# sayands/sgaligner

Measured on AMD Instinct MI355X. Metric: subscan-pairs/sec (fwd+bwd) + node-match Hits@1 vs reference, higher is better.
Workload: dtype f32 (fp32 operands and fp32 accumulation throughout; the anchors x negatives loss sweeps multiply them as three exact bf16 planes, six bf16 MFMAs per product...

## Files before the change

include/sgaligner_hip.h:

```cpp
#ifndef SGALIGNER_HIP_H
#define SGALIGNER_HIP_H
#include <stddef.h>
#include <stdint.h>
#ifdef __cplusplus
extern "C" {
#endif

int sga_version(void);
const char* sga_last_error(void);
int sga_device_cus(void);

int sga_pointnet_fwd(const float* x, const float* w1, const float* b1, const float* w2, const float* b2,
                     const float* w3, const float* b3, float* y, int32_t* argmax, int T, int P, int C3,
                     void* stream);
size_t sga_pointnet_fwd_ws_bytes(int T, int C3);
int sga_pointnet_fwd_ws(const float* x, const float* w1, const float* b1, const float* w2, const float* b2,
                        const float* w3, const float* b3, float* y, int32_t* argmax, int T, int P, int C3,
                        void* workspace, size_t ws_bytes, int mode, void* stream);
size_t sga_pointnet_fwd_bn_ws_bytes(int T, int C3);
int sga_pointnet_fwd_bn(const float* x, const float* w1, const float* b1, const float* w2, const float* b2,
                        const float* w3, const float* b3, float* y, int32_t* argmax, int T, int P, int C3,
                        void* workspace, size_t ws_bytes, void* bn_workspace, size_t bn_ws_bytes, double* bn_sums, int mode, void* stream);
int sga_pointnet_bwd(const float* x, const int32_t* argmax, const float* y, const float* gy, const float* w1,
                     const float* b1, const float* w2, const float* b2, const float* w3, float* gw1, float* gb1,
                     float* gw2, float* gb2, float* gw3, float* gb3, int T, int P, int C3, int mode, void* stream);

int sga_gemm(int transA, int transB, int M, int N, int K, const void* A, long lda, int a_is_f64, const float* B,
             long ldb, float* C, long ldc, const float* bias, int accumulate, void* stream);
int sga_colsum(const float* X, long ld, int M, int N, float* out, int accumulate, void* stream);
int sga_gemm_bnstats(int M, int N, int K, const float* A, long lda, const float* B, long ldb, float* C, long ldc, const float* bias,
                     double* sums, void* stream);
int sga_cast_f64_f32(const double* in, float* out, size_t n, void* stream);

int sga_fusion_fwd(const float* const* embs, int M, const float* weight, float* joint, int T, int D, void* stream);
size_t sga_fusion_bwd_workspace_bytes(int M);
int sga_fusion_bwd(const float* const* embs, int M, const float* weight, const float* gjoint, float* const* gembs,
                   float* gweight, int T, int D, void* workspace, size_t workspace_bytes, void* stream);

int sga_gat_complete_flags(const int64_t* edges, const int32_t* node_off, const int32_t* edge_off, int G, uint8_t* flags, void* stream);
int sga_gat_attn_fwd(const float* H, const float* att_src, const float* att_dst, const float* bias,
                     const int64_t* edges, const int32_t* node_off, const int32_t* edge_off, int G, int nmax,
                     float* out, int32_t* status, const uint8_t* complete, void* stream);
int sga_gat_attn_bwd(const float* H, const float* dO, const float* att_src, const float* att_dst, const int64_t* edges,
                     const int32_t* node_off, const int32_t* edge_off, int G, int nmax, float* dH, float* d_att_src,
                     float* d_att_dst, const uint8_t* complete, void* stream);
int sga_elu_fwd(const float* x, float* y, size_t n, void* stream);
int sga_elu_bwd(const float* x, const float* gy, float* gx, size_t n, void* stream);

int sga_loss_gather(const float* E, int T, int D, const int32_t* idx, int R, float* Z, int Dp, float* nrm, void* stream);
int sga_loss_scatter(const float* dZ, const float* Z, const float* nrm, const int32_t* idx, int R, int D, int Dp,
                     float* dE, void* stream);
int sga_loss_slots(void);
int sga_loss_neg_sums(const float* Z, int Dp, int A, int J1, int J2, float tau0, float tau1, double* sums8, void* stream);
int sga_loss_neg_grad(const float* Z, int Dp, int A, int J1, int J2, float tau0, float tau1, const double* gs8,
                      float* dZ, void* stream);
int sga_loss_neg_sums_shard(const float* Z, int Dp, int A, int J1, int J2, float tau0, float tau1, double* sums8, int a_lo, int a_hi,
                            void* stream);
int sga_loss_neg_grad_shard(const float* Z, int Dp, int A, int J1, int J2, float tau0, float tau1, const double* gs8,
                            float* dZ, int a_lo, int a_hi, void* stream);
int sga_loss_anchor_fwd(const float* const* Z, const int* Dp, int NT, int A, const double* sums, float alpha,
                        float tau_icl, float tau_ial, double* out, int a_lo, int a_hi, void* stream);
int sga_loss_anchor_bwd(const float* const* Z, const int* Dp, int NT, int A, const double* sums, float alpha,
                        float tau_icl, float tau_ial, const float* coef, float* const* M1, double* gs, int a_lo, int a_hi,
                        void* stream);

size_t sga_loss_anchor_f16_ws_bytes(int NT, int A, int ns);
int sga_loss_anchor_fwd_f16(const float* const* Z, const void* const* Zh, const int* Dp, int NT, int A, const double* sums,
                            float alpha, float tau_icl, float tau_ial, double* out, int a_lo, int a_hi, void* ws, size_t ws_bytes,
                            void* stream);
int sga_loss_anchor_bwd_f16(const float* const* Z, const void* const* Zh, const int* Dp, int NT, int A, const double* sums,
                            float alpha, float tau_icl, float tau_ial, const float* coef, float* const* M1,
                            double* gs, int a_lo, int a_hi, void* ws, size_t ws_bytes, void* stream);

int sga_loss_stash_grad(const float* M1, const float* Z, int A, int Dp, float* dZ, int a_lo, int a_hi, void* stream);
int sga_loss_multi_sums(const float* const* Z, int M, int D, const float* beta, int A, int J1, int J2, float tau0, float tau1,
                        double* sums, int a_lo, int a_hi, void* stream);
int sga_loss_multi_grad(const float* const* Z, int M, int D, const float* beta, int A, int J1, int J2, float tau0, float tau1,
                        const double* gs, float* const* dZ, double* gamma, int a_lo, int a_hi, void* stream);
size_t sga_loss_centre_bytes(void);
int sga_loss_centre_tables(const float* Z, int A, int J1, int J2, float* Zc, void* stat_ws, void* stream);
int sga_loss_multi_sums_centred(const float* const* Zc, int M, const float* beta, int A, int J1, int J2, float tau0, float tau1,
                                double* sums, int a_lo, int a_hi, void* stream);
int sga_loss_multi_grad_centred(const float* const* Zc, int M, const float* beta, int A, int J1, int J2, float tau0, float tau1,
                                const double* gs, float* const* dZ, double* gamma, int a_lo, int a_hi, void* stream);
int sga_loss_scatter_tangent_stat(const float* dZ, const float* Z, const float* nrm, const int32_t* idx, int R, int D,
                                  const void* stat_ws, float* dE, void* stream);
int sga_loss_anchor_multi_fwd(const float* const* Z, int M, const float* beta, int A, const double* sums, float alpha,
                              float tau_icl, float tau_ial, double* out, int a_lo, int a_hi, void* stream);
int sga_loss_anchor_multi_bwd(const float* const* Z, int M, const float* beta, int A, const double* sums, float alpha,
                              float tau_icl, float tau_ial, const float* coef, float* const* M1, double* gs, double* gamma,
                              int a_lo, int a_hi, double* out_terms, void* stream);
int sga_loss_anchor_multi_bwd_sym(const float* const* Z, int M, const float* beta, int A, const double* sums, float alpha,
                                  float tau_icl, float tau_ial, const float* coef, float* const* M1, float* const* M2, double* gs,
                                  double* gamma, int a_lo, int a_hi, double* out_terms, void* stream);
int sga_loss_stash_grad_sym(const float* M1, const float* M2, const float* Z, int A, int Dp, float* dZ, int a_lo, int a_hi,
                            void* stream);
int sga_loss_anchor_multi_bwd_symx(const float* const* Z, int M, const float* beta, int A, const double* sums, float alpha,
                                   float tau_icl, float tau_ial, const float* coef, float* const* M1, float* const* M2,
                                   double* gs, double* gamma, int a_lo, int a_hi, int j_lo, int j_hi, int mir, double* out_terms, void* stream);
int sga_loss_stash_grad_symx(const float* M1, const float* M2, const float* Z, int A, int Dp, float* dZ, int a_lo, int a_hi,
                             int j_lo, int j_hi, int mir, void* stream);

int sga_loss_build_joint(const float* const* Z, int M, const float* beta, int rows, float* ZJ, void* stream);
int sga_loss_fold_joint(const float* const* Z, int M, const float* beta, const float* dZJ, int rows, float* const* dZ,
                        double* gamma2, void* stream);
int sga_loss_check_norms(const float* nrm, int n, float* poison, void* stream);

size_t sga_loss_split3_bytes(int A, int J1, int J2);
int sga_loss_split3_tables(const float* Z, int A, int J1, int J2, void* Zb, float* Zc, void* stream);
int sga_loss_multi_sums_bf16x6(const void* const* Zb, int M, const float* beta, int A, int J1, int J2, float tau0, float tau1,
                               double* sums, int a_lo, int a_hi, int lite, void* stream);
int sga_loss_multi_grad_bf16x6(const void* const* Zb, int M, const float* beta, int A, int J1, int J2, float tau0, float tau1,
                               const double* gs, float* const* dZ, double* gamma, int a_lo, int a_hi, void* stream);
int sga_loss_scatter_tangent(const float* dZ, const float* Z, const float* nrm, const int32_t* idx, int A, int J1, int J2, int D,
                             const void* Zb, float* dE, void* stream);
int sga_loss_stash_grad_symx_bf16x6(const float* M1, const float* M2, const void* Zb, int A, int J1, int J2, float* dZ,
                                    int a_lo, int a_hi, int j_lo, int j_hi, int mir, void* stream);

int sga_group_loss_fwd(const float* const* Z, int M, const float* beta, int A, int J1, const int32_t* groups, int G,
                       const int64_t* s_off, int64_t s_total, float alpha, float tau_icl, float tau_ial, float* S,
                       double* sums, double* out, int use_valu, void* stream);
int sga_group_loss_bwd(const float* const* Z, int M, const float* beta, int A, int J1, const int32_t* groups, int G,
                       const int64_t* s_off, int64_t s_total, float alpha, float tau_icl, float tau_ial, float* S,
                       const double* sums, const float* coef, float* const* dZ, double* gamma, int use_valu, void* stream);

size_t sga_simrank_workspace_bytes(int T);
size_t sga_simrank_workspace_bytes_f16(int T, int D);
int sga_simrank(const float* E, int T, int D, const int32_t* pair_off, const int32_t* blk_pair, const int32_t* blk_row, int n_blocks, int B,
                int max_pair_objects, const int32_t* q_idx, const int32_t* q_tgt, int Q, int K, int32_t* rank,
                int32_t* topk_idx, float* topk_sim, int f16, void* workspace, size_t workspace_bytes, void* stream);
int sga_pair_metrics(const int32_t* rank, const int32_t* topk_idx, const float* topk_sim, int K, const int32_t* q_tgt,
                     const int32_t* pair_off, const int32_t* pair_q_off, int B, float* out, void* stream);

int sga_gemm_ex(int transA, int transB, int M, int N, int K, const float* A, long lda, const float* B, long ldb,
                float* C, long ldc, const float* bias, int act, const float* resid, long ldr, void* stream);
int sga_pct_attention(const float* Q, long ldq, const float* V, long ldv, int T, int N, float* stats, float* Xs,
                      long ldx, void* stream);
int sga_pct_attention_bwd(const float* Q, long ldq, const float* V, long ldv, const float* dXs, long ldd, int T, int N,
                          const float* stats, float* work, float* dQ, long ldo, float* dV, long ldw, void* stream);
int sga_segment_max(const float* Y, long ldy, int T, int N, int C, float* G, int32_t* argmax, void* stream);
int sga_segment_max_bwd(const float* dG, const int32_t* argmax, int T, int N, int C, float* dY, long ldd, void* stream);
int sga_pct_head_prep(const float* dG, const float* G, const float* gamma, const float* beta, const float* fin, int T, int C, long R,
                      int training, float slope, float* coef, float* ab, void* stream);
int sga_pct_head_dw(const float* WG, const float* W, const float* ab, const float* cs, const float* coef, const int32_t* amax,
                    const float* cat, long ldc, int T, int N, int C, int K, float* dW, float* Wb, float* a0, void* stream);
int sga_pct_head_scatter(const float* coef, const int32_t* amax, const float* W, int T, int N, int C, int K, float* dcat, long ldd,
                         void* stream);
int sga_segment_max_affine(const float* Y, long ldy, int T, int N, int C, const float* scale, const float* shift, float slope, float* G,
                           int32_t* argmax, void* stream);

int sga_bn_stats(const float* X, long ldx, int R, int C, double* sums, void* stream);
int sga_bn_finalize(const double* sums, int R, int C, const float* gamma, const float* beta, float* running_mean, float* running_var,
                    long long* num_batches_tracked, float momentum, float eps, int training, float* out, void* stream);
int sga_bn_bwd_finalize(const double* sums, int R, int C, float* out, void* stream);
int sga_bn_apply(const float* X, long ldx, int R, int C, const float* scale, const float* shift, int act,
                 const float* resid, long ldr, float* Y, long ldy, void* stream);
int sga_bn_bwd_stats(const float* X, long ldx, const float* dY, long ldd, int R, int C, const float* scale,
                     const float* shift, const float* mean, const float* rstd, int act, double* sums, void* stream);
int sga_bn_bwd_apply(const float* X, long ldx, const float* dY, long ldd, int R, int C, const float* scale,
                     const float* shift, const float* mean, const float* rstd, const float* mean_g,
                     const float* mean_gx, int act, float* dX, long ldo, void* stream);

size_t sga_fps_scratch_floats(int total_points);
int sga_fps(const float* pts, const int32_t* offsets, int n_obj, const int32_t* start, int npoint,
            const int32_t* work_small, int n_small, const int32_t* work_mid, int n_mid,
            const int32_t* work_large, int n_large, int32_t* out_idx, float* scratch, void* stream);

int sga_hull_candidates(const float* pts, const int32_t* offsets, int n_obj, unsigned char* keep, int32_t* n_planes, void* stream);
int sga_hull_max_candidates(void);
int sga_hull_vertices(const double* pts, const int32_t* offsets, int n_obj, unsigned char* is_vertex, int32_t* status, void* stream);

size_t sga_loss_neg_grad_wide_floats(int A, int J1, int J2);
int sga_loss_neg_grad_wide(const float* Z, int Dp, int A, int J1, int J2, float tau0, float tau1, const double* gs8, float* dZ,
                           float* stash, size_t stash_floats, void* stream);

long sga_wide16_ldt(int A, int J1, int J2);
int sga_wide16_prepare(const float* Z, int Dp, int A, int J1, int J2, void* Zh, void* ZhT, void* stream);
int sga_loss_neg_sums_f16(const void* Zh, int Dp, int A, int J1, int J2, float tau0, float tau1, double* sums8, int a_lo, int a_hi, void* stream);
size_t sga_loss_neg_grad_f16_bytes(int A, int J1, int J2);
int sga_loss_neg_grad_f16(const void* Zh, const void* ZhT, int Dp, int A, int J1, int J2, float tau0, float tau1, const double* gs8,
                          float* dZ, void* stash, size_t stash_bytes, int a_lo, int a_hi, void* stream);
size_t sga_loss_stash_grad_f16_bytes(int A, int ns);
int sga_loss_stash_grad_f16(const float* M1, const void* ZhT, int Dp, int A, int J1, int J2, float* dZ, int a_lo, int a_hi,
                            void* ws, size_t ws_bytes, void* stream);

int sga_loss_head_fwd(const void* sums, int sums_f64, const float* lv_ial, const float* lv_icl, int M, double inv_a2,
                      double z_ial, double alpha, double zoom, double* out, void* stream);
int sga_loss_head_bwd(const double* gout, const void* sums, int sums_f64, const float* lv_ial, const float* lv_icl, int M,
                      double inv_a2, double z_ial, double alpha, double zoom, void* dsums, float* dlv_ial, float* dlv_icl,
                      void* stream);

#ifdef __cplusplus
}
#endif
#endif
```

sgaligner_amd/_lib.py:

```python
from __future__ import annotations

import ctypes
import os
from ctypes import c_char_p, c_double, c_float, c_int, c_int64, c_long, c_size_t, c_void_p

_HERE = os.path.dirname(os.path.abspath(__file__))
LIB_PATH = os.environ.get('SGA_LIB_PATH') or os.path.join(_HERE, 'csrc', 'libsga_hip.so')
_lib = None

P = c_void_p
I = c_int
F = c_float

SIGNATURES = {
    'sga_version': (I, []),
    'sga_last_error': (c_char_p, []),
    'sga_device_cus': (I, []),
    'sga_pointnet_fwd': (I, [P, P, P, P, P, P, P, P, P, I, I, I, P]),
    'sga_pointnet_fwd_ws_bytes': (c_size_t, [I, I]),
    'sga_loss_neg_grad_wide_floats': (c_size_t, [I, I, I]),
    'sga_loss_neg_grad_wide': (I, [P, I, I, I, I, c_float, c_float, P, P, P, c_size_t, P]),
    'sga_wide16_ldt': (c_long, [I, I, I]),
    'sga_wide16_prepare': (I, [P, I, I, I, I, P, P, P]),
    'sga_loss_neg_sums_f16': (I, [P, I, I, I, I, c_float, c_float, P, I, I, P]),
    'sga_loss_neg_grad_f16_bytes': (c_size_t, [I, I, I]),
    'sga_loss_neg_grad_f16': (I, [P, P, I, I, I, I, c_float, c_float, P, P, P, c_size_t, I, I, P]),
    'sga_loss_head_fwd': (I, [P, I, P, P, I, c_double, c_double, c_double, c_double, P, P]),
    'sga_loss_head_bwd': (I, [P, P, I, P, P, I, c_double, c_double, c_double, c_double, P, P, P, P]),
    'sga_pointnet_fwd_ws': (I, [P, P, P, P, P, P, P, P, P, I, I, I, P, c_size_t, I, P]),
    'sga_pointnet_fwd_bn_ws_bytes': (c_size_t, [I, I]),
    'sga_pointnet_fwd_bn': (I, [P, P, P, P, P, P, P, P, P, I, I, I, P, c_size_t, P, c_size_t, P, I, P]),
    'sga_pointnet_bwd': (I, [P] * 15 + [I, I, I, I, P]),
    'sga_gat_complete_flags': (I, [P, P, P, I, P, P]),
    'sga_gat_attn_fwd': (I, [P, P, P, P, P, P, P, I, I, P, P, P, P]),
    'sga_gat_attn_bwd': (I, [P, P, P, P, P, P, P, I, I, P, P, P, P, P]),
    'sga_elu_fwd': (I, [P, P, c_size_t, P]),
    'sga_elu_bwd': (I, [P, P, P, c_size_t, P]),
    'sga_simrank_workspace_bytes': (c_size_t, [I]),
    'sga_simrank_workspace_bytes_f16': (c_size_t, [I, I]),
    'sga_simrank': (I, [P, I, I, P, P, P, I, I, I, P, P, I, I, P, P, P, I, P, c_size_t, P]),
    'sga_pair_metrics': (I, [P, P, P, I, P, P, P, I, P, P]),
    'sga_gemm_ex': (I, [I, I, I, I, I, P, c_long, P, c_long, P, c_long, P, I, P, c_long, P]),
    'sga_pct_attention': (I, [P, c_long, P, c_long, I, I, P, P, c_long, P]),
    'sga_pct_attention_bwd': (I, [P, c_long, P, c_long, P, c_long, I, I, P, P, P, c_long, P, c_long, P]),
    'sga_segment_max': (I, [P, c_long, I, I, I, P, P, P]),
    'sga_segment_max_bwd': (I, [P, P, I, I, I, P, c_long, P]),
    'sga_pct_head_prep': (I, [P, P, P, P, P, I, I, c_long, I, c_float, P, P, P]),
    'sga_pct_head_dw': (I, [P, P, P, P, P, P, P, c_long, I, I, I, I, P, P, P, P]),
    'sga_pct_head_scatter': (I, [P, P, P, I, I, I, I, P, c_long, P]),
    'sga_segment_max_affine': (I, [P, c_long, I, I, I, P, P, c_float, P, P, P]),
    'sga_bn_stats': (I, [P, c_long, I, I, P, P]),
    'sga_bn_finalize': (I, [P, I, I, P, P, P, P, P, c_float, c_float, I, P, P]),
    'sga_bn_bwd_finalize': (I, [P, I, I, P, P]),
    'sga_bn_apply': (I, [P, c_long, I, I, P, P, I, P, c_long, P, c_long, P]),
    'sga_bn_bwd_stats': (I, [P, c_long, P, c_long, I, I, P, P, P, P, I, P, P]),
    'sga_bn_bwd_apply': (I, [P, c_long, P, c_long, I, I, P, P, P, P, P, P, I, P, c_long, P]),
    'sga_fps_scratch_floats': (c_size_t, [I]),
    'sga_fps': (I, [P, P, I, P, I, P, I, P, I, P, I, P, P, P]),
    'sga_hull_candidates': (I, [P, P, I, P, P, P]),
    'sga_hull_max_candidates': (I, []),
    'sga_hull_vertices': (I, [P, P, I, P, P, P]),
    'sga_gemm': (I, [I, I, I, I, I, P, c_long, I, P, c_long, P, c_long, P, I, P]),
    'sga_colsum': (I, [P, c_long, I, I, P, I, P]),
    'sga_gemm_bnstats': (I, [I, I, I, P, c_long, P, c_long, P, c_long, P, P, P]),
    'sga_cast_f64_f32': (I, [P, P, c_size_t, P]),
    'sga_loss_gather': (I, [P, I, I, P, I, P, I, P, P]),
    'sga_loss_scatter': (I, [P, P, P, P, I, I, I, P, P]),
    'sga_loss_neg_sums': (I, [P, I, I, I, I, F, F, P, P]),
    'sga_loss_neg_grad': (I, [P, I, I, I, I, F, F, P, P, P]),
    'sga_loss_neg_sums_shard': (I, [P, I, I, I, I, F, F, P, I, I, P]),
    'sga_loss_neg_grad_shard': (I, [P, I, I, I, I, F, F, P, P, I, I, P]),
    'sga_loss_anchor_fwd': (I, [P, P, I, I, P, F, F, F, P, I, I, P]),
    'sga_loss_anchor_bwd': (I, [P, P, I, I, P, F, F, F, P, P, P, I, I, P]),
    'sga_loss_anchor_f16_ws_bytes': (c_size_t, [I, I, I]),
    'sga_loss_anchor_fwd_f16': (I, [P, P, P, I, I, P, F, F, F, P, I, I, P, c_size_t, P]),
    'sga_loss_anchor_bwd_f16': (I, [P, P, P, I, I, P, F, F, F, P, P, P, I, I, P, c_size_t, P]),
    'sga_loss_stash_grad_f16_bytes': (c_size_t, [I, I]),
    'sga_loss_stash_grad_f16': (I, [P, P, I, I, I, I, P, I, I, P, c_size_t, P]),
    'sga_loss_multi_sums': (I, [P, I, I, P, I, I, I, F, F, P, I, I, P]),
    'sga_loss_multi_grad': (I, [P, I, I, P, I, I, I, F, F, P, P, P, I, I, P]),
    'sga_loss_centre_bytes': (c_size_t, []),
    'sga_loss_centre_tables': (I, [P, I, I, I, P, P, P]),
    'sga_loss_multi_sums_centred': (I, [P, I, P, I, I, I, F, F, P, I, I, P]),
    'sga_loss_multi_grad_centred': (I, [P, I, P, I, I, I, F, F, P, P, P, I, I, P]),
    'sga_loss_scatter_tangent_stat': (I, [P, P, P, P, I, I, P, P, P]),
    'sga_loss_build_joint': (I, [P, I, P, I, P, P]),
    'sga_loss_fold_joint': (I, [P, I, P, P, I, P, P, P]),
    'sga_loss_check_norms': (I, [P, I, P, P]),
    'sga_loss_slots': (I, []),
    'sga_loss_anchor_multi_fwd': (I, [P, I, P, I, P, F, F, F, P, I, I, P]),
    'sga_loss_anchor_multi_bwd': (I, [P, I, P, I, P, F, F, F, P, P, P, P, I, I, P, P]),
    'sga_loss_stash_grad': (I, [P, P, I, I, P, I, I, P]),
    'sga_loss_anchor_multi_bwd_sym': (I, [P, I, P, I, P, F, F, F, P, P, P, P, P, I, I, P, P]),
    'sga_loss_stash_grad_sym': (I, [P, P, P, I, I, P, I, I, P]),
    'sga_loss_anchor_multi_bwd_symx': (I, [P, I, P, I, P, F, F, F, P, P, P, P, P, I, I, I, I, I, P, P]),
    'sga_loss_stash_grad_symx': (I, [P, P, P, I, I, P, I, I, I, I, I, P]),
    'sga_loss_split3_bytes': (c_size_t, [I, I, I]),
    'sga_loss_split3_tables': (I, [P, I, I, I, P, P, P]),
    'sga_loss_scatter_tangent': (I, [P, P, P, P, I, I, I, I, P, P, P]),
    'sga_loss_stash_grad_symx_bf16x6': (I, [P, P, P, I, I, I, P, I, I, I, I, I, P]),
    'sga_loss_multi_sums_bf16x6': (I, [P, I, P, I, I, I, F, F, P, I, I, I, P]),
    'sga_loss_multi_grad_bf16x6': (I, [P, I, P, I, I, I, F, F, P, P, P, I, I, P]),
    'sga_group_loss_fwd': (I, [P, I, P, I, I, P, I, P, c_int64, F, F, F, P, P, P, I, P]),
    'sga_group_loss_bwd': (I, [P, I, P, I, I, P, I, P, c_int64, F, F, F, P, P, P, P, P, I, P]),
    'sga_fusion_fwd': (I, [P, I, P, P, I, I, P]),
    'sga_fusion_bwd_workspace_bytes': (c_size_t, [I]),
    'sga_fusion_bwd': (I, [P, I, P, P, P, P, I, I, P, c_size_t, P]),
}


class SgaLibraryError(RuntimeError):
    pass


def lib():
    global _lib
    if _lib is None:
        if not os.path.exists(LIB_PATH):
            raise SgaLibraryError(
                f'HIP library not built: {LIB_PATH} is missing. Run `python -c "import __graft_entry__ as g; g.build()"` '
                f'(or `python -m sgaligner_amd._build`). sgaligner_amd has no CPU fallback.')
        import torch
        try:
            l = ctypes.CDLL(LIB_PATH)
        except OSError as e:
            raise SgaLibraryError(f'cannot load {LIB_PATH}: {e}') from e
        for name, (res, args) in SIGNATURES.items():
            try:
                fn = getattr(l, name)
            except AttributeError as e:
                raise SgaLibraryError(f'{LIB_PATH} does not export {name}; rebuild the library') from e
            fn.restype = res
            fn.argtypes = args
        _lib = l
    return _lib


def check(rc: int, what: str):
    if rc != 0:
        msg = lib().sga_last_error()
        raise RuntimeError(f'{what} failed (code {rc}): {msg.decode() if msg else "?"}')
```

sgaligner_amd/csrc/contrastive.hip:

```cpp
#include "mfma_tiles.h"
#include <type_traits>

#include "loss_math.h"
#include "wide16_api.h"

extern "C" int sga_gemm(int transA, int transB, int M, int N, int K, const void* A, long lda, int a_is_f64, const float* B,
                        long ldb, float* C, long ldc, const float* bias, int accumulate, void* stream);

namespace {

constexpr int CT_THREADS = 256;
constexpr int CT_MAXT = 9;
__global__ void gather_normalize_kernel(const float* __restrict__ E, int D, const int* __restrict__ idx, int R,
                                        float* __restrict__ Z, int Dp, float* __restrict__ nrm) {
    const int lane = threadIdx.x & 63, wpb = blockDim.x >> 6;
    for (int r = blockIdx.x * wpb + (threadIdx.x >> 6); r < R; r += gridDim.x * wpb) {
        const float* x = E + (size_t)idx[r] * D;
        float ss = 0.f;
        for (int d = lane; d < D; d += 64) { const float v = x[d]; ss += v * v; }
        ss = wave_sum(ss);
        const float n = sqrtf(ss);
        const float inv = 1.f / fmaxf(n, 1e-12f);
        float* z = Z + (size_t)r * Dp;
        for (int d = lane; d < Dp; d += 64) z[d] = d < D ? x[d] * inv : 0.f;
        if (lane == 0) nrm[r] = n;
    }
}

__global__ void scatter_normalize_bwd_kernel(const float* __restrict__ dZ, const float* __restrict__ Z,
                                             const float* __restrict__ nrm, const int* __restrict__ idx, int R, int D,
                                             int Dp, float* __restrict__ dE) {
    const int lane = threadIdx.x & 63, wpb = blockDim.x >> 6;
    for (int r = blockIdx.x * wpb + (threadIdx.x >> 6); r < R; r += gridDim.x * wpb) {
        const float* g = dZ + (size_t)r * Dp;
        const float* z = Z + (size_t)r * Dp;
        float dot = 0.f;
        for (int d = lane; d < D; d += 64) dot += g[d] * z[d];
        dot = wave_sum(dot);
        const float n = nrm[r];
        const bool clamped = n < 1e-12f;
        const float inv = 1.f / fmaxf(n, 1e-12f);
        if (clamped) dot = 0.f;
        float* o = dE + (size_t)idx[r] * D;
        for (int d = lane; d < D; d += 64) atomicAdd(o + d, (g[d] - z[d] * dot) * inv);
    }
}

struct SweepSeg { int row0, n, fam; };
struct SweepGroup { int own0, nown, blk0, nseg; SweepSeg seg[2]; int nsplit; };
struct SweepArgs {
    const float* Z; int Dp; int ngroups; SweepGroup grp[4];
    float k0, k1;
    float it0, it1;
    double* sums;
    const double* gs;
    float* dZ;
    int col0;
};

template <int NJT, int NCT, bool GRAD>
__global__ __launch_bounds__(CT_THREADS) void sweep_kernel(SweepArgs a) {
    constexpr int OT = NJT * 32;
    constexpr int GW = NCT * 32;
    extern __shared__ __attribute__((aligned(16))) float lds[];
    float* own_s = lds;
    float* oth_s = lds + 128 * SGA_LDS_STRIDE;

    const int tid = threadIdx.x, lane = tid & 63, wave = tid >> 6, h = lane >> 5;
    int g = 0;
#pragma unroll
    for (int i = 1; i < 4; ++i) if (i < a.ngroups && (int)blockIdx.x >= a.grp[i].blk0) g = i;
    const SweepGroup& grp = a.grp[g];
    const int own0 = grp.own0 + ((int)blockIdx.x - grp.blk0) * 128;
    const int own_end = grp.own0 + grp.nown;
    const int my_i = own0 + wave * 32 + (lane & 31);

    f32x16 gacc[GRAD ? NCT : 1];
    if (GRAD) zero_acc<GRAD ? NCT : 1>(gacc);
    double dsum[2][2] = {{0.0, 0.0}, {0.0, 0.0}};

#pragma unroll
    for (int sg = 0; sg < 2; ++sg) {
        if (sg >= grp.nseg) break;
        const SweepSeg seg = grp.seg[sg];
        float c0 = 0.f, c1 = 0.f;
        if (GRAD) { c0 = (float)(a.gs[seg.fam * 2 + 0] * (double)a.it0); c1 = (float)(a.gs[seg.fam * 2 + 1] * (double)a.it1); }
        const int ntile = (seg.n + OT - 1) / OT;
        for (int jt = blockIdx.y; jt < ntile; jt += gridDim.y) {
            const int j0 = seg.row0 + jt * OT, j_end = seg.row0 + seg.n;
            f32x16 sacc[NJT];
            zero_acc<NJT>(sacc);
            for (int k0 = 0; k0 < a.Dp; k0 += SGA_KC) {
                __syncthreads();
                lds_load_rows<128, CT_THREADS>(own_s, a.Z, a.Dp, own0, own_end, k0, a.Dp, tid);
                lds_load_rows<OT, CT_THREADS>(oth_s, a.Z, a.Dp, j0, j_end, k0, a.Dp, tid);
                __syncthreads();
                mfma_chunk<NJT>(sacc, oth_s, own_s + (wave * 32 + (lane & 31)) * SGA_LDS_STRIDE, lane);
            }
            if (!GRAD) {
                float p0 = 0.f, p1 = 0.f;
                const bool iv = my_i < own_end;
#pragma unroll
                for (int t = 0; t < NJT; ++t)
#pragma unroll
                    for (int r = 0; r < 16; ++r) {
                        const float okf = (iv && (j0 + t * 32 + mfma32_row(r, h) < j_end)) ? 1.f : 0.f;
                        p0 = fmaf(okf, fexp2(sacc[t][r] * a.k0), p0);
                        p1 = fmaf(okf, fexp2(sacc[t][r] * a.k1), p1);
                    }
                dsum[sg][0] += (double)p0;
                dsum[sg][1] += (double)p1;
            } else {
#pragma unroll
                for (int t = 0; t < NJT; ++t)
#pragma unroll
                    for (int r = 0; r < 16; ++r)
                        sacc[t][r] = c0 * fexp2(sacc[t][r] * a.k0) + c1 * fexp2(sacc[t][r] * a.k1);
                __syncthreads();
                for (int e = tid; e < OT * (GW / 4); e += CT_THREADS) {
                    const int r = e / (GW / 4), c = (e % (GW / 4)) * 4;
                    const int gr = j0 + r, gc = a.col0 + c;
                    f32x4 v = {0.f, 0.f, 0.f, 0.f};
                    if (gr < j_end && gc < a.Dp) v = *reinterpret_cast<const f32x4*>(a.Z + (size_t)gr * a.Dp + gc);
                    *reinterpret_cast<f32x4*>(lds + r * GW + c) = v;
                }
                __syncthreads();
#pragma unroll
                for (int t = 0; t < NJT; ++t)
#pragma unroll
                    for (int s = 0; s < 16; ++s) {
                        const float av = sacc[t][s];
                        const float* brow = lds + (t * 32 + mfma32_row(s, h)) * GW + (lane & 31);
#pragma unroll
                        for (int ct = 0; ct < NCT; ++ct)
                            gacc[ct] = __builtin_amdgcn_mfma_f32_32x32x2f32(av, brow[ct * 32], gacc[ct], 0, 0, 0);
                    }
            }
        }
    }
    if (!GRAD) {
#pragma unroll
        for (int sg = 0; sg < 2; ++sg)
#pragma unroll
            for (int tt = 0; tt < 2; ++tt) {
                const double v = wave_sum_d(dsum[sg][tt]);
                if (lane == 0 && sg < grp.nseg && v != 0.0) atomicAdd(a.sums + 8 + my_slot() * 8 + grp.seg[sg].fam * 2 + tt, v);
            }
    } else {
#pragma unroll
        for (int ct = 0; ct < NCT; ++ct) {
            const int d = a.col0 + ct * 32 + (lane & 31);
            if (d < a.Dp) {
#pragma unroll
                for (int r = 0; r < 16; ++r) {
                    const int i = own0 + wave * 32 + mfma32_row(r, h);
                    if (i < own_end) atomicAdd(a.dZ + (size_t)i * a.Dp + d, gacc[ct][r]);
                }
            }
        }
    }
}

struct CoefArgs {
    const float* Z; int Dp; SweepGroup grp[2];
    float k0, k1, it0, it1;
    const double* gs;
    float* stash[2];
    int ld, n1;
};

template <int NJT>
__global__ __launch_bounds__(CT_THREADS) void sweep_coef_kernel(CoefArgs a) {
    constexpr int OT = NJT * 32;
    __shared__ __attribute__((aligned(16))) float own_s[128 * SGA_LDS_STRIDE];
    __shared__ __attribute__((aligned(16))) float oth_s[OT * SGA_LDS_STRIDE];
    const int tid = threadIdx.x, lane = tid & 63, wave = tid >> 6, h = lane >> 5;
    const int g = ((int)blockIdx.x >= a.grp[1].blk0 && a.grp[1].nown > 0) ? 1 : 0;
    const SweepGroup& grp = a.grp[g];
    const int own0 = grp.own0 + ((int)blockIdx.x - grp.blk0) * 128;
    const int own_end = grp.own0 + grp.nown;
    const int my_i = own0 + wave * 32 + (lane & 31);
    float* __restrict__ st = a.stash[g];
#pragma unroll
    for (int sg = 0; sg < 2; ++sg) {
        const SweepSeg seg = grp.seg[sg];
        const float c0 = (float)(a.gs[seg.fam * 2 + 0] * (double)a.it0), c1 = (float)(a.gs[seg.fam * 2 + 1] * (double)a.it1);
        const int ntile = (seg.n + OT - 1) / OT;
        for (int jt = blockIdx.y; jt < ntile; jt += gridDim.y) {
            const int j0 = seg.row0 + jt * OT, j_end = seg.row0 + seg.n;
            f32x16 sacc[NJT];
            zero_acc<NJT>(sacc);
            for (int k0 = 0; k0 < a.Dp; k0 += SGA_KC) {
                __syncthreads();
                lds_load_rows<128, CT_THREADS>(own_s, a.Z, a.Dp, own0, own_end, k0, a.Dp, tid);
                lds_load_rows<OT, CT_THREADS>(oth_s, a.Z, a.Dp, j0, j_end, k0, a.Dp, tid);
                __syncthreads();
                mfma_chunk<NJT>(sacc, oth_s, own_s + (wave * 32 + (lane & 31)) * SGA_LDS_STRIDE, lane);
            }
            if (my_i < own_end) {
#pragma unroll
                for (int t = 0; t < NJT; ++t)
#pragma unroll
                    for (int r = 0; r < 16; ++r) {
                        const int j = j0 + t * 32 + mfma32_row(r, h);
                        if (j < j_end) st[(size_t)(j - a.n1) * a.ld + (my_i - grp.own0)] = c0 * fexp2(sacc[t][r] * a.k0) + c1 * fexp2(sacc[t][r] * a.k1);
                    }
            }
        }
    }
}

template <int NQ, bool GRAD>
__global__ __launch_bounds__(CT_THREADS) void sweep_fast_kernel(SweepArgs a) {
    constexpr int DP = NQ * 8;
    constexpr int STR = DP + 4;
    constexpr int NJT = 4, OT = 128, NCT = 4;
    extern __shared__ __attribute__((aligned(16))) float lds[];

    const int tid = threadIdx.x, lane = tid & 63, wave = tid >> 6, h = lane >> 5;
    int g = 0;
#pragma unroll
    for (int i = 1; i < 4; ++i) if (i < a.ngroups && (int)blockIdx.x >= a.grp[i].blk0) g = i;
    const SweepGroup& grp = a.grp[g];
    const int own0 = grp.own0 + ((int)blockIdx.x - grp.blk0) * 128;
    const int own_end = grp.own0 + grp.nown;
    const int my_i = own0 + wave * 32 + (lane & 31);

    f32x4 own[NQ];
    {
        const float* src = a.Z + (size_t)(my_i < own_end ? my_i : own0) * DP + 4 * h;
        const float msk = my_i < own_end ? 1.f : 0.f;
#pragma unroll
        for (int q = 0; q < NQ; ++q) {
            f32x4 v = *reinterpret_cast<const f32x4*>(src + 8 * q);
            own[q] = v * msk;
        }
    }
    f32x16 gacc[GRAD ? NCT : 1];
    if (GRAD) zero_acc<GRAD ? NCT : 1>(gacc);
    double dsum[2][2] = {{0.0, 0.0}, {0.0, 0.0}};

#pragma unroll
    for (int sg = 0; sg < 2; ++sg) {
        if (sg >= grp.nseg) break;
        const SweepSeg seg = grp.seg[sg];
        float c0 = 0.f, c1 = 0.f;
        if (GRAD) { c0 = (float)(a.gs[seg.fam * 2 + 0] * (double)a.it0); c1 = (float)(a.gs[seg.fam * 2 + 1] * (double)a.it1); }
        const int ntile = (seg.n + OT - 1) / OT;
        for (int jt = blockIdx.y; jt < ntile; jt += gridDim.y) {
            const int j0 = seg.row0 + jt * OT, j_end = seg.row0 + seg.n;
            __syncthreads();
            for (int e = tid; e < OT * (DP / 4); e += CT_THREADS) {
                const int r = e / (DP / 4), c = (e % (DP / 4)) * 4;
                f32x4 v = {0.f, 0.f, 0.f, 0.f};
                if (j0 + r < j_end) v = *reinterpret_cast<const f32x4*>(a.Z + (size_t)(j0 + r) * DP + c);
                *reinterpret_cast<f32x4*>(lds + r * STR + c) = v;
            }
            __syncthreads();
            f32x16 sacc[NJT];
            zero_acc<NJT>(sacc);
            const float* ap = lds + (lane & 31) * STR + 4 * h;
#pragma unroll
            for (int q = 0; q < NQ; ++q) {
#pragma unroll
                for (int t = 0; t < NJT; ++t) {
                    const f32x4 av = *reinterpret_cast<const f32x4*>(ap + t * 32 * STR + 8 * q);
#pragma unroll
                    for (int r = 0; r < 4; ++r) sacc[t] = __builtin_amdgcn_mfma_f32_32x32x2f32(av[r], own[q][r], sacc[t], 0, 0, 0);
                }
            }
            if (!GRAD) {
                float p0 = 0.f, p1 = 0.f;
                const bool iv = my_i < own_end;
#pragma unroll
                for (int t = 0; t < NJT; ++t)
#pragma unroll
                    for (int r = 0; r < 16; ++r) {
                        const float okf = (iv && (j0 + t * 32 + mfma32_row(r, h) < j_end)) ? 1.f : 0.f;
                        p0 = fmaf(okf, fexp2(sacc[t][r] * a.k0), p0);
                        p1 = fmaf(okf, fexp2(sacc[t][r] * a.k1), p1);
                    }
                dsum[sg][0] += (double)p0;
                dsum[sg][1] += (double)p1;
            } else {
#pragma unroll
                for (int t = 0; t < NJT; ++t)
#pragma unroll
                    for (int r = 0; r < 16; ++r)
                        sacc[t][r] = c0 * fexp2(sacc[t][r] * a.k0) + c1 * fexp2(sacc[t][r] * a.k1);
#pragma unroll
                for (int t = 0; t < NJT; ++t)
#pragma unroll
                    for (int s = 0; s < 16; ++s) {
                        const float av = sacc[t][s];
                        const float* brow = lds + (t * 32 + mfma32_row(s, h)) * STR + (lane & 31);
#pragma unroll
                        for (int ct = 0; ct < NCT; ++ct)
                            gacc[ct] = __builtin_amdgcn_mfma_f32_32x32x2f32(av, brow[ct * 32], gacc[ct], 0, 0, 0);
                    }
            }
        }
    }
    if (!GRAD) {
#pragma unroll
        for (int sg = 0; sg < 2; ++sg)
#pragma unroll
// ... 645 lines not shown
                acc[m] = fmaf(gj, a.Z[m][(size_t)r * 104 + d], acc[m]);
                a.dZ[m][(size_t)r * 104 + d] += sb * gj;
            }
        }
#pragma unroll
    for (int m = 0; m < 4; ++m) {
        const float v = wave_sum(acc[m]);
        if (lane == 0 && m < a.M && v != 0.f) atomicAdd(gamma2 + m, (double)v);
    }
}

__global__ void check_norms_kernel(const float* __restrict__ nrm, int n, float* __restrict__ poison) {
    for (int i = blockIdx.x * blockDim.x + threadIdx.x; i < n; i += gridDim.x * blockDim.x)
        if (!(nrm[i] >= 1e-12f)) *poison = __builtin_nanf("");
}

typedef _Float16 ak_f16x8 __attribute__((ext_vector_type(8)));
template <int NROWS, int NTHREADS>
__device__ __forceinline__ void lds_load_rows_h(float* __restrict__ tile, const _Float16* __restrict__ g, int ld, int row0, int nrows, int k0,
                                                int ncols, int tid) {
    unsigned char* t8 = reinterpret_cast<unsigned char*>(tile);
#pragma unroll
    for (int e = tid; e < NROWS * 8; e += NTHREADS) {
        const int r = e >> 3, c = (e & 7) * 8;
        ak_f16x8 v = {0, 0, 0, 0, 0, 0, 0, 0};
        const int gr = row0 + r, gc = k0 + c;
        if (gr < nrows && gc < ncols) v = *reinterpret_cast<const ak_f16x8*>(g + (size_t)gr * ld + gc);
        *reinterpret_cast<ak_f16x8*>(t8 + r * 144 + c * 2) = v;
    }
}
template <int NT>
__device__ __forceinline__ void mfma_chunk_h(f32x16 (&acc)[NT], const float* __restrict__ a_tile, const float* __restrict__ b_row, int lane) {
    const unsigned char* ap = reinterpret_cast<const unsigned char*>(a_tile) + (lane & 31) * 144 + (lane >> 5) * 16;
    const unsigned char* bp = reinterpret_cast<const unsigned char*>(b_row) + (lane >> 5) * 16;
#pragma unroll
    for (int q = 0; q < 4; ++q) {
        const ak_f16x8 b = *reinterpret_cast<const ak_f16x8*>(bp + 32 * q);
#pragma unroll
        for (int t = 0; t < NT; ++t) {
            const ak_f16x8 av = *reinterpret_cast<const ak_f16x8*>(ap + t * 32 * 144 + 32 * q);
            acc[t] = __builtin_amdgcn_mfma_f32_32x32x16_f16(av, b, acc[t], 0, 0, 0);
        }
    }
}

struct AnchorArgs {
    int NT, A, i_lo, i_hi;
    const float* Z[CT_MAXT]; int Dp[CT_MAXT];
    const _Float16* Zh[CT_MAXT];
    const double* sums;
    float alpha, kc, ki, itc, iti;
    double* out;
    const float* coef;
    float* M1[CT_MAXT];
    double* gs;
    const float* SP[CT_MAXT];
    const float* SQ[CT_MAXT];
    long ldp;
};

template <bool BWD, bool PRE = false>
__global__ __launch_bounds__(CT_THREADS) void anchor_kernel(AnchorArgs a) {
    constexpr int NJT = PRE ? 1 : 2, OT = 32 * NJT;
    constexpr int LR = PRE ? 1 : 128, LO = PRE ? 1 : OT;
    __shared__ __attribute__((aligned(16))) float own1[LR * SGA_LDS_STRIDE];
    __shared__ __attribute__((aligned(16))) float own2[LR * SGA_LDS_STRIDE];
    __shared__ __attribute__((aligned(16))) float oth1[LO * SGA_LDS_STRIDE];
    __shared__ __attribute__((aligned(16))) float oth2[LO * SGA_LDS_STRIDE];
    __shared__ float inv_s[CT_MAXT * 8];

    const int tid = threadIdx.x, lane = tid & 63, wave = tid >> 6, h = lane >> 5;
    const int A = a.A, NT = a.NT, M = NT > 1 ? NT - 1 : 0;
    double* const out_s = BWD ? nullptr : a.out + (NT + 2 * M) * (1 + my_slot());
    double* const gs_s = BWD ? a.gs + NT * 8 * (1 + my_slot()) : nullptr;
    for (int e = tid; e < NT * 8; e += CT_THREADS) inv_s[e] = (float)(1.0 / (a.sums[e] + 1e-9));
    const int i0 = a.i_lo + blockIdx.x * 128, j0 = blockIdx.y * OT;
    const int my_i = i0 + wave * 32 + (lane & 31);
    const bool iv = my_i < a.i_hi;
    const int ns = a.i_hi - a.i_lo;

    f32x16 xJ[NJT], gJ[NJT];
    zero_acc<NJT>(xJ);
    zero_acc<NJT>(gJ);

    for (int it = 0; it < NT; ++it) {
        const int k = (NT > 1) ? (it == 0 ? NT - 1 : it - 1) : 0;
        const bool is_joint = NT > 1 && it == 0;
        const float* Z = a.Z[k];
        const int Dp = a.Dp[k];
        f32x16 P[NJT], Q[NJT];
        zero_acc<NJT>(P);
        zero_acc<NJT>(Q);
        const _Float16* Zh = a.Zh[k];
        if constexpr (PRE) {
            __syncthreads();
            const float* sp = a.SP[k] + (iv ? my_i - a.i_lo : 0);
            const float* sq = a.SQ[k] + (iv ? my_i - a.i_lo : 0);
#pragma unroll
            for (int t = 0; t < NJT; ++t)
#pragma unroll
                for (int r = 0; r < 16; ++r) {
                    const int j = min(j0 + t * 32 + mfma32_row(r, h), A - 1);
                    P[t][r] = sp[(size_t)j * a.ldp];
                    Q[t][r] = sq[(size_t)j * a.ldp];
                }
        } else
        if (Zh) {
            for (int k0 = 0; k0 < Dp; k0 += 64) {
                __syncthreads();
                lds_load_rows_h<128, CT_THREADS>(own1, Zh, Dp, i0, A, k0, Dp, tid);
                lds_load_rows_h<128, CT_THREADS>(own2, Zh, Dp, A + i0, 2 * A, k0, Dp, tid);
                lds_load_rows_h<OT, CT_THREADS>(oth1, Zh, Dp, A + j0, 2 * A, k0, Dp, tid);
                lds_load_rows_h<OT, CT_THREADS>(oth2, Zh, Dp, j0, A, k0, Dp, tid);
                __syncthreads();
                const int ro = (wave * 32 + (lane & 31)) * SGA_LDS_STRIDE;
                mfma_chunk_h<NJT>(P, oth1, own1 + ro, lane);
                mfma_chunk_h<NJT>(Q, oth2, own2 + ro, lane);
            }
        } else
        for (int k0 = 0; k0 < Dp; k0 += SGA_KC) {
            __syncthreads();
            lds_load_rows<128, CT_THREADS>(own1, Z, Dp, i0, A, k0, Dp, tid);
            lds_load_rows<128, CT_THREADS>(own2, Z, Dp, A + i0, 2 * A, k0, Dp, tid);
            lds_load_rows<OT, CT_THREADS>(oth1, Z, Dp, A + j0, 2 * A, k0, Dp, tid);
            lds_load_rows<OT, CT_THREADS>(oth2, Z, Dp, j0, A, k0, Dp, tid);
            __syncthreads();
            const int ro = (wave * 32 + (lane & 31)) * SGA_LDS_STRIDE;
            mfma_chunk<NJT>(P, oth1, own1 + ro, lane);
            mfma_chunk<NJT>(Q, oth2, own2 + ro, lane);
        }
        if (is_joint) {
#pragma unroll
            for (int t = 0; t < NJT; ++t) xJ[t] = P[t];
        }
        const float* is = inv_s + k * 8;
        const float a11c = is[0], a12c = is[2], a22c = is[4], a21c = is[6];
        const float a11i = is[1], a12i = is[3], a22i = is[5], a21i = is[7];
        const float* js = inv_s + (NT - 1) * 8;
        const float j11 = js[1], j12 = js[3], j22 = js[5], j21 = js[7];

        if (!BWD) {
            float icl = 0.f, la = 0.f, lb = 0.f;
#pragma unroll
            for (int t = 0; t < NJT; ++t)
#pragma unroll
                for (int r = 0; r < 16; ++r) {
                    const bool ok = iv && (j0 + t * 32 + mfma32_row(r, h) < A);
                    const float x = P[t][r], y = Q[t][r];
                    const float qa = g_val(fexp2(x * a.kc), a11c, a12c);
                    const float qb = g_val(fexp2(y * a.kc), a22c, a21c);
                    const float term = -flog(a.alpha * qa + (1.f - a.alpha) * qb);
                    icl += ok ? term : 0.f;
                    if (M > 0 && !is_joint) {
                        const float dm = fexp2(x * a.ki), dj = fexp2(xJ[t][r] * a.ki);
                        const float qoa = g_val(dm, a11i, a12i), qma = g_val(dj, j11, j12);
                        const float qob = g_val(dm, a22i, a21i), qmb = g_val(dj, j22, j21);
                        const float ta = __expf(qoa) * (qoa - flog(qma));
                        const float tb = __expf(qob) * (qob - flog(qmb));
                        la += ok ? ta : 0.f;
                        lb += ok ? tb : 0.f;
                    }
                    __builtin_amdgcn_sched_barrier(0);
                }
            icl = wave_sum(icl);
            if (lane == 0) atomicAdd(out_s + k, (double)icl);
            if (M > 0 && !is_joint) {
                la = wave_sum(la);
                lb = wave_sum(lb);
                if (lane == 0) { atomicAdd(out_s + NT + k, (double)la); atomicAdd(out_s + NT + M + k, (double)lb); }
            }
        } else {
            const float c = a.coef[k];
            const float ca = (M > 0 && !is_joint) ? a.coef[NT + k] : 0.f;
            const float cb = (M > 0 && !is_joint) ? a.coef[NT + M + k] : 0.f;
            float gs_c[4] = {0.f, 0.f, 0.f, 0.f};
            float gs_i[4] = {0.f, 0.f, 0.f, 0.f};
            float gs_j[4] = {0.f, 0.f, 0.f, 0.f};
#pragma unroll
            for (int t = 0; t < NJT; ++t)
#pragma unroll
                for (int r = 0; r < 16; ++r) {
                    const bool ok = iv && (j0 + t * 32 + mfma32_row(r, h) < A);
                    const float x = P[t][r], y = Q[t][r];
                    const float dx = fexp2(x * a.kc), dy = fexp2(y * a.kc);
                    const GV Ax = g_full(dx, a11c, a12c), Bx = g_full(dx, a22c, a21c);
                    const float qAy = g_val(dy, a11c, a12c), qBy = g_val(dy, a22c, a21c);
                    const float z_ij = a.alpha * Ax.q + (1.f - a.alpha) * qBy;
                    const float z_ji = a.alpha * qAy + (1.f - a.alpha) * Bx.q;
                    const float wA = ok ? -c * a.alpha * frcp(z_ij) : 0.f;
                    const float wB = ok ? -c * (1.f - a.alpha) * frcp(z_ji) : 0.f;
                    float gx = (wA * Ax.dd + wB * Bx.dd) * dx * a.itc;
                    gs_c[0] += wA * Ax.dsa; gs_c[1] += wA * Ax.dsb; gs_c[2] += wB * Bx.dsa; gs_c[3] += wB * Bx.dsb;
                    if (M > 0 && !is_joint) {
                        const float dm = fexp2(x * a.ki), dj = fexp2(xJ[t][r] * a.ki);
                        const GV OA = g_full(dm, a11i, a12i), OB = g_full(dm, a22i, a21i);
                        const GV MA = g_full(dj, j11, j12), MB = g_full(dj, j22, j21);
                        const float eA = ok ? __expf(OA.q) : 0.f, eB = ok ? __expf(OB.q) : 0.f;
                        const float tA = ca * eA * (OA.q - flog(MA.q) + 1.f), uA = -ca * eA * frcp(MA.q);
                        const float tB = cb * eB * (OB.q - flog(MB.q) + 1.f), uB = -cb * eB * frcp(MB.q);
                        gx += (tA * OA.dd + tB * OB.dd) * dm * a.iti;
                        gJ[t][r] += (uA * MA.dd + uB * MB.dd) * dj * a.iti;
                        gs_i[0] += tA * OA.dsa; gs_i[1] += tA * OA.dsb; gs_i[2] += tB * OB.dsa; gs_i[3] += tB * OB.dsb;
                        gs_j[0] += uA * MA.dsa; gs_j[1] += uA * MA.dsb; gs_j[2] += uB * MB.dsa; gs_j[3] += uB * MB.dsb;
                    }
                    P[t][r] = gx;
                    __builtin_amdgcn_sched_barrier(0);
                }
#pragma unroll
            for (int f = 0; f < 4; ++f) {
                const float vc = wave_sum(gs_c[f]);
                if (lane == 0 && vc != 0.f) atomicAdd(gs_s + k * 8 + f * 2 + 0, (double)vc);
                if (M > 0 && !is_joint) {
                    const float vi = wave_sum(gs_i[f]), vj = wave_sum(gs_j[f]);
                    if (lane == 0 && vi != 0.f) atomicAdd(gs_s + k * 8 + f * 2 + 1, (double)vi);
                    if (lane == 0 && vj != 0.f) atomicAdd(gs_s + (NT - 1) * 8 + f * 2 + 1, (double)vj);
                }
            }
            if (is_joint) {
#pragma unroll
                for (int t = 0; t < NJT; ++t) gJ[t] = P[t];
            } else if (iv) {
                float* m1 = a.M1[k];
#pragma unroll
                for (int t = 0; t < NJT; ++t)
#pragma unroll
                    for (int r = 0; r < 16; ++r) {
                        const int j = j0 + t * 32 + mfma32_row(r, h);
                        if (j < A) m1[(size_t)j * ns + (my_i - a.i_lo)] = P[t][r];
                    }
            }
        }
    }
    if (BWD && NT > 1 && iv) {
        float* m1 = a.M1[NT - 1];
#pragma unroll
        for (int t = 0; t < NJT; ++t)
#pragma unroll
            for (int r = 0; r < 16; ++r) {
                const int j = j0 + t * 32 + mfma32_row(r, h);
                if (j < A) m1[(size_t)j * ns + (my_i - a.i_lo)] = gJ[t][r];
            }
    }
}

template <int NCT, bool TRANS>
__global__ __launch_bounds__(256) void stash_gemm_kernel(const float* __restrict__ M1, const float* __restrict__ X,
                                                         float* __restrict__ out, int MR, int KR, int ldm, int ld, int Dp, int k_per_split) {
    const int lane = threadIdx.x & 63, wave = threadIdx.x >> 6, h = lane >> 5, l31 = lane & 31;
    const int m0 = (blockIdx.x * 4 + wave) * 32;
    if (m0 >= MR) return;
    const int kbeg = blockIdx.y * k_per_split, kend = min(KR, kbeg + k_per_split);
    const int m = min(m0 + l31, MR - 1);
    f32x16 acc[NCT];
    zero_acc<NCT>(acc);
    int ncol[NCT];
#pragma unroll
    for (int ct = 0; ct < NCT; ++ct) ncol[ct] = min(ct * 32 + l31, Dp - 1);
    for (int k0 = kbeg; k0 < kend; k0 += 8) {
        float av[4];
        float kmask[4];
#pragma unroll
        for (int r = 0; r < 4; ++r) {
            const int k = k0 + 4 * h + r;
            kmask[r] = k < kend ? 1.f : 0.f;
            const int kc = min(k, KR - 1);
            av[r] = (TRANS ? M1[(size_t)kc * ldm + m] : M1[(size_t)m * ldm + kc]) * kmask[r];
        }
#pragma unroll
        for (int r = 0; r < 4; ++r) {
            const int kc = min(k0 + 4 * h + r, KR - 1);
            const float* xr = X + (size_t)kc * ld;
#pragma unroll
            for (int ct = 0; ct < NCT; ++ct) acc[ct] = __builtin_amdgcn_mfma_f32_32x32x2f32(av[r], xr[ncol[ct]], acc[ct], 0, 0, 0);
        }
    }
#pragma unroll
    for (int ct = 0; ct < NCT; ++ct) {
        const int d = ct * 32 + l31;
        if (d < Dp) {
#pragma unroll
            for (int r = 0; r < 16; ++r) {
                const int row = m0 + mfma32_row(r, h);
                if (row < MR) atomicAdd(out + (size_t)row * ld + d, acc[ct][r]);
            }
        }
    }
}

struct AnchorMultiArgs {
    int M, A, i_lo, i_hi, nsplit;
    const float* Z[4];
    const float* beta;
    const double* sums;
    const float* inv;
    float alpha, kc, ki, itc, iti;
    double* out;
    const float* coef;
    float* M1[4];
    double* gs;
    double* gamma;
    int j_lo;
    float* M2[4];
    int j_hi, mir;
};

template <int M, bool BWD>
__global__ __launch_bounds__(CT_THREADS, M <= 3 ? 2 : 1) void anchor_multi_kernel(AnchorMultiArgs a) {
    constexpr int DP = 104, NQ = 13, NT = M + 1;
    extern __shared__ __attribute__((aligned(16))) float lds[];
    float* inv_s = lds + M * 2 * 32 * DP;
    const int tid = threadIdx.x, lane = tid & 63, wave = tid >> 6, h = lane >> 5, l31 = lane & 31;
    const int A = a.A, ns = a.i_hi - a.i_lo;
    const int ib = blockIdx.x / a.nsplit, split = blockIdx.x % a.nsplit;
    const int i0 = a.i_lo + ib * 32;
    const int my_i = i0 + l31;
    const bool iv = my_i < a.i_hi;

    for (int e = tid; e < M * 2 * 32 * (DP / 4); e += CT_THREADS) {
        const int c = (e % (DP / 4)) * 4, r = (e / (DP / 4)) % 32, side = (e / (DP / 4) / 32) % 2, m = e / (DP / 4) / 64;
        const int row = min(i0 + r, a.i_hi - 1) + side * A;
        *reinterpret_cast<f32x4*>(lds + ((m * 2 + side) * 32 + r) * DP + c) = *reinterpret_cast<const f32x4*>(a.Z[m] + (size_t)row * DP + c);
    }
    for (int e = tid; e < NT * 8; e += CT_THREADS) inv_s[e] = (float)(1.0 / (a.sums[e] + 1e-9));
    __syncthreads();
    float beta[M];
#pragma unroll
    for (int m = 0; m < M; ++m) beta[m] = a.beta[m];

    double acc_d[NT + 2 * M];
#pragma unroll
    for (int e = 0; e < NT + 2 * M; ++e) acc_d[e] = 0.0;

    const int ntile = (A + 31) / 32;
    for (int jt = split * 4 + wave; jt < ntile; jt += a.nsplit * 4) {
        const int j0 = jt * 32;
        float acc_out[NT + 2 * M];
#pragma unroll
        for (int e = 0; e < NT + 2 * M; ++e) acc_out[e] = 0.f;
        const int jrow = min(j0 + l31, A - 1);
        f32x16 P[M], Q[M];
        zero_acc<M>(P);
        zero_acc<M>(Q);
#pragma unroll
        for (int m = 0; m < M; ++m) {
            const float* gp = a.Z[m] + (size_t)(A + jrow) * DP + 4 * h;
            const float* gq = a.Z[m] + (size_t)jrow * DP + 4 * h;
            const float* bp = lds + ((m * 2 + 0) * 32 + l31) * DP + 4 * h;
            const float* bq = lds + ((m * 2 + 1) * 32 + l31) * DP + 4 * h;
            f32x4 apA = *reinterpret_cast<const f32x4*>(gp), aqA = *reinterpret_cast<const f32x4*>(gq), apB = apA, aqB = aqA;
#pragma unroll
            for (int q = 0; q < NQ; ++q) {
                if (q + 1 < NQ) {
                    if (q & 1) { apA = *reinterpret_cast<const f32x4*>(gp + 8 * (q + 1)); aqA = *reinterpret_cast<const f32x4*>(gq + 8 * (q + 1)); }
                    else { apB = *reinterpret_cast<const f32x4*>(gp + 8 * (q + 1)); aqB = *reinterpret_cast<const f32x4*>(gq + 8 * (q + 1)); }
                }
                const f32x4 b1 = *reinterpret_cast<const f32x4*>(bp + 8 * q);
                const f32x4 b2 = *reinterpret_cast<const f32x4*>(bq + 8 * q);
#pragma unroll
                for (int r = 0; r < 4; ++r) {
                    P[m] = __builtin_amdgcn_mfma_f32_32x32x2f32((q & 1) ? apB[r] : apA[r], b1[r], P[m], 0, 0, 0);
                    Q[m] = __builtin_amdgcn_mfma_f32_32x32x2f32((q & 1) ? aqB[r] : aqA[r], b2[r], Q[m], 0, 0, 0);
                }
                __builtin_amdgcn_sched_barrier(0);
            }
        }
        float xs[M][16], ys[M][16];
#pragma unroll
        for (int m = 0; m < M; ++m)
#pragma unroll
            for (int r = 0; r < 16; ++r) { xs[m][r] = P[m][r]; ys[m][r] = Q[m][r]; }
        const float* js = inv_s + M * 8;
#pragma unroll
        for (int r = 0; r < 16; ++r) {
            const int j = j0 + mfma32_row(r, h);
            const bool ok = iv && j < A;
            float xj = 0.f, yj = 0.f;
#pragma unroll
            for (int m = 0; m < M; ++m) { xj = fmaf(beta[m], xs[m][r], xj); yj = fmaf(beta[m], ys[m][r], yj); }
            {
                const float dji = fexp2(xj * a.ki);
                const float qma = g_val(dji, js[1], js[3]), qmb = g_val(dji, js[5], js[7]);
                const float lqma = flog(qma), lqmb = flog(qmb);
#pragma unroll
                for (int k = 0; k < NT; ++k) {
                    const float x = k < M ? xs[k < M ? k : 0][r] : xj, y = k < M ? ys[k < M ? k : 0][r] : yj;
                    const float* is = inv_s + k * 8;
                    const float qa = g_val(fexp2(x * a.kc), is[0], is[2]);
                    const float qb = g_val(fexp2(y * a.kc), is[4], is[6]);
                    const float term = -flog(a.alpha * qa + (1.f - a.alpha) * qb);
                    acc_out[k] += ok ? term : 0.f;
                    if (k < M) {
                        const float dm = fexp2(x * a.ki);
                        const float qoa = g_val(dm, is[1], is[3]), qob = g_val(dm, is[5], is[7]);
                        const float ta = __expf(qoa) * (qoa - lqma), tb = __expf(qob) * (qob - lqmb);
                        acc_out[NT + (k < M ? k : 0)] += ok ? ta : 0.f;
                        acc_out[NT + M + (k < M ? k : 0)] += ok ? tb : 0.f;
                    }
                }
            }
#pragma unroll
            for (int e = 0; e < NT + 2 * M; ++e) asm volatile("" : "+v"(acc_out[e]));
            __builtin_amdgcn_sched_barrier(0);
        }
#pragma unroll
        for (int e = 0; e < NT + 2 * M; ++e) acc_d[e] += (double)acc_out[e];
    }
    const int slot = my_slot();
#pragma unroll
    for (int e = 0; e < NT + 2 * M; ++e) {
        const double v = wave_sum_d(acc_d[e]);
        if (lane == 0 && v != 0.0) atomicAdd(a.out + (NT + 2 * M) * (1 + slot) + e, v);
    }
}

__global__ void inv_sums_kernel(const double* __restrict__ sums, float* __restrict__ inv, int n) {
    const int i = blockIdx.x * blockDim.x + threadIdx.x;
    if (i < n) inv[i] = (float)(1.0 / (sums[i] + 1e-9));
}

template <int M, bool TERMS = false, int RB = (M <= 3 ? 32 : 16), bool SYM = false>
__global__ __launch_bounds__(CT_THREADS, 2) void anchor_multi_bwd16_kernel(AnchorMultiArgs a) {
    static_assert(!SYM || TERMS, "symmetric mode: one-pass build");
    constexpr int DP = 104, NT = M + 1, NSUB = RB / 16, TW = 4 / NSUB;
    extern __shared__ __attribute__((aligned(16))) float lds[];
    const float* __restrict__ inv_s = a.inv;
    auto CF = [&](int e) { return a.coef[e]; };
    const int tid = threadIdx.x, lane = tid & 63, wave = tid >> 6, g = lane >> 4, l15 = lane & 15;
    const int A = a.A, ns = a.i_hi - a.i_lo;
    const int JH = SYM ? a.j_hi : A;
    const int ib = blockIdx.x / a.nsplit, split = blockIdx.x % a.nsplit;
    const int i0 = a.i_lo + ib * RB;
    const int ih = wave % NSUB, tw = wave / NSUB;
    const int my_i = i0 + ih * 16 + l15;
    const bool iv = my_i < a.i_hi;

    for (int e = tid; e < M * 2 * RB * (DP / 4); e += CT_THREADS) {
        const int c = (e % (DP / 4)) * 4, r = (e / (DP / 4)) % RB, side = (e / (DP / 4) / RB) % 2, m = e / (DP / 4) / (2 * RB);
        const int row = min(i0 + r, a.i_hi - 1) + side * A;
        *reinterpret_cast<f32x4*>(lds + ((m * 2 + side) * RB + r) * DP + c) = *reinterpret_cast<const f32x4*>(a.Z[m] + (size_t)row * DP + c);
    }
    __syncthreads();
    float beta[M];
#pragma unroll
    for (int m = 0; m < M; ++m) beta[m] = a.beta[m];

    float acc_gs[NT][8], acc_gam[M];
#pragma unroll
    for (int k = 0; k < NT; ++k)
#pragma unroll
        for (int e = 0; e < 8; ++e) acc_gs[k][e] = 0.f;
#pragma unroll
    for (int m = 0; m < M; ++m) acc_gam[m] = 0.f;
    float acc_out[TERMS ? NT + 2 * M : 1];
#pragma unroll
    for (int e = 0; e < (TERMS ? NT + 2 * M : 1); ++e) acc_out[e] = 0.f;
    int tiles_done = 0;
    const int slot = my_slot();
    auto flush = [&]() {
        if (TERMS) {
#pragma unroll
            for (int e = 0; e < NT + 2 * M; ++e) {
                const float v = wave_sum(acc_out[TERMS ? e : 0]);
                if (lane == 0 && v != 0.f) atomicAdd(a.out + (NT + 2 * M) * (1 + slot) + e, (double)v);
                acc_out[TERMS ? e : 0] = 0.f;
            }
        }
#pragma unroll
        for (int k = 0; k < NT; ++k)
#pragma unroll
            for (int e = 0; e < 8; ++e) {
                const float iv2 = inv_s[k * 8 + e];
                const float v = -iv2 * iv2 * wave_sum(acc_gs[k][e]);
                if (lane == 0 && v != 0.f) atomicAdd(a.gs + NT * 8 * (1 + slot) + k * 8 + e, (double)v);
                acc_gs[k][e] = 0.f;
            }
#pragma unroll
        for (int m = 0; m < M; ++m) {
            const float v = wave_sum(acc_gam[m]);
            if (lane == 0 && v != 0.f) atomicAdd(a.gamma + M * (1 + slot) + m, (double)v);
            acc_gam[m] = 0.f;
        }
    };
    const float* js = inv_s + M * 8;

    const int ntile = (JH + 15) / 16;
#pragma unroll 1
    for (int jt = (a.j_lo >> 4) + split * TW + tw; jt < ntile; jt += a.nsplit * TW) {
        const int j0 = jt * 16;
        const int jrow = min(j0 + l15, A - 1);
        int lofs = 0;
        asm volatile("" : "+v"(lofs));
        f32x4 P[M], Q[M];
        struct JOps { f32x4 p[6], q[6]; float pt[2], qt[2]; };
        auto jload = [&](int m, JOps& o) {
            const float* gp = a.Z[m] + (size_t)(A + jrow) * DP;
            const float* gq = a.Z[m] + (size_t)jrow * DP;
#pragma unroll
            for (int q = 0; q < 6; ++q) {
                o.p[q] = *reinterpret_cast<const f32x4*>(gp + 16 * q + 4 * g);
                o.q[q] = *reinterpret_cast<const f32x4*>(gq + 16 * q + 4 * g);
            }
#pragma unroll
            for (int t = 0; t < 2; ++t) { o.pt[t] = gp[96 + 4 * t + g]; o.qt[t] = gq[96 + 4 * t + g]; }
        };
        constexpr bool JDB = true;
        JOps jb[JDB ? 2 : 1];
        jload(0, jb[0]);
#pragma unroll
        for (int m = 0; m < M; ++m) {
            if (JDB) { if (m + 1 < M) jload(m + 1, jb[JDB ? (m + 1) & 1 : 0]); }
            else if (m > 0) jload(m, jb[0]);
            __builtin_amdgcn_sched_barrier(0);
            P[m] = f32x4{0.f, 0.f, 0.f, 0.f};
            Q[m] = P[m];
            const JOps& o = jb[JDB ? m & 1 : 0];
            const float* bp = lds + lofs + ((m * 2 + 0) * RB + ih * 16 + l15) * DP;
            const float* bq = lds + lofs + ((m * 2 + 1) * RB + ih * 16 + l15) * DP;
#pragma unroll
            for (int q = 0; q < 6; ++q) {
                const f32x4 b1 = *reinterpret_cast<const f32x4*>(bp + 16 * q + 4 * g);
                const f32x4 b2 = *reinterpret_cast<const f32x4*>(bq + 16 * q + 4 * g);
#pragma unroll
                for (int r = 0; r < 4; ++r) {
                    P[m] = __builtin_amdgcn_mfma_f32_16x16x4f32(o.p[q][r], b1[r], P[m], 0, 0, 0);
                    Q[m] = __builtin_amdgcn_mfma_f32_16x16x4f32(o.q[q][r], b2[r], Q[m], 0, 0, 0);
                }
            }
#pragma unroll
            for (int t = 0; t < 2; ++t) {
                const int kk = 96 + 4 * t + g;
                P[m] = __builtin_amdgcn_mfma_f32_16x16x4f32(o.pt[t], bp[kk], P[m], 0, 0, 0);
                Q[m] = __builtin_amdgcn_mfma_f32_16x16x4f32(o.qt[t], bq[kk], Q[m], 0, 0, 0);
            }
            __builtin_amdgcn_sched_barrier(0);
        }
        const float cJ = CF(M);
        auto epilogue = [&](auto masked_c) {
        constexpr bool MASKED = decltype(masked_c)::value;
#pragma unroll
        for (int r = 0; r < 4; ++r) {
            const int j = j0 + 4 * g + r;
            const bool ok = !MASKED || (iv && (j < JH));
            const float okf = (!MASKED || ok) ? 1.f : 0.f;
            float xj = 0.f, yj = 0.f;
#pragma unroll
            for (int m = 0; m < M; ++m) { xj = fmaf(beta[m], P[m][r], xj); yj = fmaf(beta[m], Q[m][r], yj); }
            float gJ, EA = 0.f, EB = 0.f;
            {
                const float dx = fexp2(xj * a.kc), dy = fexp2(yj * a.kc);
                const GP Ax = g_parts(dx, js[0], js[2]), Bx = g_parts(dx, js[4], js[6]);
                const float qAy = g_val(dy, js[0], js[2]), qBy = g_val(dy, js[4], js[6]);
                const float denA = a.alpha * Ax.q + (1.f - a.alpha) * qBy;
                const float wA = okf * (-cJ * a.alpha) * frcp(denA) * dx;
                const float wB = okf * (-cJ * (1.f - a.alpha)) * frcp(a.alpha * qAy + (1.f - a.alpha) * Bx.q) * dx;
                if (TERMS) acc_out[TERMS ? M : 0] = fmaf(okf, -flog(denA), acc_out[TERMS ? M : 0]);
                gJ = fmaf(wA, Ax.dd, wB * Bx.dd) * a.itc;
                acc_gs[M][0] = fmaf(wA, Ax.p, acc_gs[M][0]); acc_gs[M][2] = fmaf(wA, Ax.r, acc_gs[M][2]);
                acc_gs[M][4] = fmaf(wB, Bx.p, acc_gs[M][4]); acc_gs[M][6] = fmaf(wB, Bx.r, acc_gs[M][6]);
            }
            const float dji = fexp2(xj * a.ki);
            const GP MA = g_parts(dji, js[1], js[3]), MB = g_parts(dji, js[5], js[7]);
            const float lqma = flog(MA.q), lqmb = flog(MB.q);
            float gx[M];
#pragma unroll
            for (int m = 0; m < M; ++m) {
                const float* is = inv_s + m * 8;
                const float c = CF(m), ca = CF(NT + m), cb = CF(NT + M + m);
                const float x = P[m][r], y = Q[m][r];
                const float dx = fexp2(x * a.kc), dy = fexp2(y * a.kc);
                const GP Ax = g_parts(dx, is[0], is[2]), Bx = g_parts(dx, is[4], is[6]);
                const float qAy = g_val(dy, is[0], is[2]), qBy = g_val(dy, is[4], is[6]);
                const float denA = a.alpha * Ax.q + (1.f - a.alpha) * qBy;
                const float wA = okf * (-c * a.alpha) * frcp(denA) * dx;
                const float wB = okf * (-c * (1.f - a.alpha)) * frcp(a.alpha * qAy + (1.f - a.alpha) * Bx.q) * dx;
                if (TERMS) acc_out[TERMS ? m : 0] = fmaf(okf, -flog(denA), acc_out[TERMS ? m : 0]);
                float gxm = fmaf(wA, Ax.dd, wB * Bx.dd) * a.itc;
                acc_gs[m][0] = fmaf(wA, Ax.p, acc_gs[m][0]); acc_gs[m][2] = fmaf(wA, Ax.r, acc_gs[m][2]);
                acc_gs[m][4] = fmaf(wB, Bx.p, acc_gs[m][4]); acc_gs[m][6] = fmaf(wB, Bx.r, acc_gs[m][6]);
                const float dm = fexp2(x * a.ki);
                const GP OA = g_parts(dm, is[1], is[3]), OB = g_parts(dm, is[5], is[7]);
                const float xA = okf * __expf(OA.q), xB = okf * __expf(OB.q);
                const float eA = ca * xA, eB = cb * xB;
                if (TERMS) {
                    acc_out[TERMS ? NT + m : 0] = fmaf(xA, OA.q - lqma, acc_out[TERMS ? NT + m : 0]);
                    acc_out[TERMS ? NT + M + m : 0] = fmaf(xB, OB.q - lqmb, acc_out[TERMS ? NT + M + m : 0]);
                }
                const float tA = eA * (OA.q - lqma + 1.f) * dm, tB = eB * (OB.q - lqmb + 1.f) * dm;
                gxm = fmaf(fmaf(tA, OA.dd, tB * OB.dd), a.iti, gxm);
                acc_gs[m][1] = fmaf(tA, OA.p, acc_gs[m][1]); acc_gs[m][3] = fmaf(tA, OA.r, acc_gs[m][3]);
                acc_gs[m][5] = fmaf(tB, OB.p, acc_gs[m][5]); acc_gs[m][7] = fmaf(tB, OB.r, acc_gs[m][7]);
                EA += eA; EB += eB;
                gx[m] = gxm;
            }
            {
                const float uA = -EA * frcp(MA.q) * dji, uB = -EB * frcp(MB.q) * dji;
                gJ = fmaf(fmaf(uA, MA.dd, uB * MB.dd), a.iti, gJ);
                acc_gs[M][1] = fmaf(uA, MA.p, acc_gs[M][1]); acc_gs[M][3] = fmaf(uA, MA.r, acc_gs[M][3]);
                acc_gs[M][5] = fmaf(uB, MB.p, acc_gs[M][5]); acc_gs[M][7] = fmaf(uB, MB.r, acc_gs[M][7]);
            }
#pragma unroll
            for (int m = 0; m < M; ++m) {
                acc_gam[m] = fmaf(gJ, P[m][r], acc_gam[m]);
#ifdef SGA_DBG_AA_NOSTORE
                acc_gam[m] += fmaf(beta[m], gJ, gx[m]);
#else
                if (ok) a.M1[m][(size_t)(j - a.j_lo) * ns + (my_i - a.i_lo)] = fmaf(beta[m], gJ, gx[m]);
#endif
            }
#pragma unroll
            for (int k = 0; k < NT; ++k)
#pragma unroll
                for (int e = 0; e < 8; ++e) asm volatile("" : "+v"(acc_gs[k][e]));
#pragma unroll
            for (int m = 0; m < M; ++m) asm volatile("" : "+v"(acc_gam[m]));
            if (TERMS) {
#pragma unroll
                for (int e = 0; e < NT + 2 * M; ++e) asm volatile("" : "+v"(acc_out[TERMS ? e : 0]));
            }
            __builtin_amdgcn_sched_barrier(0);
        }
        };
        auto epilogue_sym = [&](auto) {
#pragma unroll
        for (int r = 0; r < 4; ++r) {
            const int j = j0 + 4 * g + r;
            const bool ok = iv && (j < JH);
            const float okf = ok ? 1.f : 0.f;
            float xj = 0.f, yj = 0.f;
#pragma unroll
            for (int m = 0; m < M; ++m) { xj = fmaf(beta[m], P[m][r], xj); yj = fmaf(beta[m], Q[m][r], yj); }
            float gci[NT][2];
#pragma unroll
            for (int k = 0; k < NT; ++k) {
                const float* is = inv_s + k * 8;
                const float x = k < M ? P[k < M ? k : 0][r] : xj, y = k < M ? Q[k < M ? k : 0][r] : yj;
                const float c = CF(k);
                const float dx = fexp2(x * a.kc), dy = fexp2(y * a.kc);
                const GP Ax = g_parts(dx, is[0], is[2]), Bx = g_parts(dx, is[4], is[6]);
                const GP Ay = g_parts(dy, is[0], is[2]), By = g_parts(dy, is[4], is[6]);
                const float den1 = a.alpha * Ax.q + (1.f - a.alpha) * By.q;
                const float den2 = a.alpha * Ay.q + (1.f - a.alpha) * Bx.q;
                const float r1 = okf * -c * frcp(den1), r2 = okf * -c * frcp(den2);
                const float wAx = a.alpha * r1 * dx, wBx = (1.f - a.alpha) * r2 * dx;
                const float wAy = a.alpha * r2 * dy, wBy = (1.f - a.alpha) * r1 * dy;
                acc_out[TERMS ? k : 0] = fmaf(okf, -(flog(den1) + flog(den2)), acc_out[TERMS ? k : 0]);
                gci[k][0] = fmaf(wAx, Ax.dd, wBx * Bx.dd) * a.itc;
                gci[k][1] = fmaf(wAy, Ay.dd, wBy * By.dd) * a.itc;
                acc_gs[k][0] = fmaf(wAx, Ax.p, fmaf(wAy, Ay.p, acc_gs[k][0])); acc_gs[k][2] = fmaf(wAx, Ax.r, fmaf(wAy, Ay.r, acc_gs[k][2]));
                acc_gs[k][4] = fmaf(wBx, Bx.p, fmaf(wBy, By.p, acc_gs[k][4])); acc_gs[k][6] = fmaf(wBx, Bx.r, fmaf(wBy, By.r, acc_gs[k][6]));
#pragma unroll
                for (int e = 0; e < 8; e += 2) asm volatile("" : "+v"(acc_gs[k][e]));
                asm volatile("" : "+v"(acc_out[TERMS ? k : 0]));
                __builtin_amdgcn_sched_barrier(0);
            }
#pragma unroll
            for (int dir = 0; dir < 2; ++dir) {
                const float vj = dir ? yj : xj;
                const float dji = fexp2(vj * a.ki);
                const GP MA = g_parts(dji, js[1], js[3]), MB = g_parts(dji, js[5], js[7]);
                const float lqma = flog(MA.q), lqmb = flog(MB.q);
                float gx[M], EA = 0.f, EB = 0.f;
#pragma unroll
                for (int m = 0; m < M; ++m) {
                    const float* is = inv_s + m * 8;
                    const float ca = CF(NT + m), cb = CF(NT + M + m);
                    const float v = dir ? Q[m][r] : P[m][r];
                    const float dm = fexp2(v * a.ki);
                    const GP OA = g_parts(dm, is[1], is[3]), OB = g_parts(dm, is[5], is[7]);
                    const float xA = okf * __expf(OA.q), xB = okf * __expf(OB.q);
                    const float eA = ca * xA, eB = cb * xB;
                    acc_out[TERMS ? NT + m : 0] = fmaf(xA, OA.q - lqma, acc_out[TERMS ? NT + m : 0]);
                    acc_out[TERMS ? NT + M + m : 0] = fmaf(xB, OB.q - lqmb, acc_out[TERMS ? NT + M + m : 0]);
                    const float tA = eA * (OA.q - lqma + 1.f) * dm, tB = eB * (OB.q - lqmb + 1.f) * dm;
                    gx[m] = fmaf(fmaf(tA, OA.dd, tB * OB.dd), a.iti, gci[m][dir]);
                    acc_gs[m][1] = fmaf(tA, OA.p, acc_gs[m][1]); acc_gs[m][3] = fmaf(tA, OA.r, acc_gs[m][3]);
                    acc_gs[m][5] = fmaf(tB, OB.p, acc_gs[m][5]); acc_gs[m][7] = fmaf(tB, OB.r, acc_gs[m][7]);
                    EA += eA; EB += eB;
                }
                const float uA = -EA * frcp(MA.q) * dji, uB = -EB * frcp(MB.q) * dji;
                const float gJ = fmaf(fmaf(uA, MA.dd, uB * MB.dd), a.iti, gci[M][dir]);
                acc_gs[M][1] = fmaf(uA, MA.p, acc_gs[M][1]); acc_gs[M][3] = fmaf(uA, MA.r, acc_gs[M][3]);
                acc_gs[M][5] = fmaf(uB, MB.p, acc_gs[M][5]); acc_gs[M][7] = fmaf(uB, MB.r, acc_gs[M][7]);
                float* const* dst = dir ? a.M2 : a.M1;
                const size_t off = (size_t)(j - (dir ? a.mir : a.j_lo)) * ns + (my_i - a.i_lo);
#pragma unroll
                for (int m = 0; m < M; ++m) {
                    acc_gam[m] = fmaf(gJ, dir ? Q[m][r] : P[m][r], acc_gam[m]);
                    if (ok) dst[m][off] = fmaf(beta[m], gJ, gx[m]);
                }
#pragma unroll
                for (int k = 0; k < NT; ++k)
#pragma unroll
                    for (int e = 1; e < 8; e += 2) asm volatile("" : "+v"(acc_gs[k][e]));
#pragma unroll
                for (int m = 0; m < M; ++m) asm volatile("" : "+v"(acc_gam[m]));
#pragma unroll
                for (int e = NT; e < NT + 2 * M; ++e) asm volatile("" : "+v"(acc_out[TERMS ? e : 0]));
                __builtin_amdgcn_sched_barrier(0);
            }
        }
        };
#ifdef SGA_DBG_AA_NOEPI
#pragma unroll
        for (int m = 0; m < M; ++m)
#pragma unroll
            for (int r = 0; r < 4; ++r) acc_gam[m] += P[m][r] * Q[m][r];
#else
        if constexpr (SYM) {
            if (j0 >= a.mir) epilogue_sym(0); else epilogue(std::true_type{});
        } else {
            if (j0 + 16 <= A && i0 + RB <= a.i_hi) epilogue(std::false_type{}); else epilogue(std::true_type{});
        }
#endif
        if ((++tiles_done & (SYM ? 15 : 31)) == 0) flush();
    }
    flush();
}

int rows_grid(int R) {
    int g = (R + 3) / 4;
    const int cap = sga_num_cus() * 8;
    return g > cap ? cap : (g < 1 ? 1 : g);
}

}

extern "C" int sga_loss_gather(const float* E, int T, int D, const int32_t* idx, int R, float* Z, int Dp, float* nrm,
                               void* stream) {
    (void)T;
    SGA_CHECK_ARG(D >= 1 && Dp >= D && Dp % 8 == 0 && R >= 0, "sga_loss_gather: bad argument (Dp must be a multiple of 8 >= D)");
    if (R == 0) return SGA_OK;
    SGA_CHECK_ARG(E && idx && Z && nrm, "sga_loss_gather: null pointer");
    hipLaunchKernelGGL(gather_normalize_kernel, dim3(rows_grid(R)), dim3(256), 0, static_cast<hipStream_t>(stream), E, D, idx, R, Z, Dp, nrm);
    SGA_CHECK_LAUNCH("sga_loss_gather");
    return SGA_OK;
}

extern "C" int sga_loss_scatter(const float* dZ, const float* Z, const float* nrm, const int32_t* idx, int R, int D,
                                int Dp, float* dE, void* stream) {
    SGA_CHECK_ARG(D >= 1 && Dp >= D && R >= 0, "sga_loss_scatter: bad argument");
    if (R == 0) return SGA_OK;
    SGA_CHECK_ARG(dZ && Z && nrm && idx && dE, "sga_loss_scatter: null pointer");
    hipLaunchKernelGGL(scatter_normalize_bwd_kernel, dim3(rows_grid(R)), dim3(256), 0, static_cast<hipStream_t>(stream), dZ, Z, nrm, idx, R, D, Dp, dE);
    SGA_CHECK_LAUNCH("sga_loss_scatter");
    return SGA_OK;
}

static void fill_groups(SweepArgs& a, int A, int J1, int J2, bool grad, int a_lo, int a_hi) {
    const int x1 = 0, x2 = A, n1 = 2 * A, n2 = 2 * A + J1, ns = a_hi - a_lo;
    int blk = 0, g = 0;
    auto add = [&](int own0, int nown, SweepSeg s0, SweepSeg s1) {
        if (nown <= 0) return;
        SweepGroup& G = a.grp[g++];
        G.own0 = own0; G.nown = nown; G.blk0 = blk; G.nseg = 2; G.seg[0] = s0; G.seg[1] = s1; G.nsplit = 1;
        blk += (nown + 127) / 128;
    };
    add(x1 + a_lo, ns, SweepSeg{n1, J1, 0}, SweepSeg{n2, J2, 1});
    add(x2 + a_lo, ns, SweepSeg{n2, J2, 2}, SweepSeg{n1, J1, 3});
    if (grad) {
        add(n1, J1, SweepSeg{x1 + a_lo, ns, 0}, SweepSeg{x2 + a_lo, ns, 3});
        add(n2, J2, SweepSeg{x1 + a_lo, ns, 1}, SweepSeg{x2 + a_lo, ns, 2});
    }
    a.ngroups = g;
}

static int total_blocks(const SweepArgs& a) {
    int n = 0;
    for (int g = 0; g < a.ngroups; ++g) n += (a.grp[g].nown + 127) / 128;
    return n;
}

extern "C" int sga_loss_neg_sums(const float* Z, int Dp, int A, int J1, int J2, float tau0, float tau1, double* sums8,
                                 void* stream) {
    return sga_loss_neg_sums_shard(Z, Dp, A, J1, J2, tau0, tau1, sums8, 0, A, stream);
}

extern "C" int sga_loss_neg_sums_shard(const float* Z, int Dp, int A, int J1, int J2, float tau0, float tau1, double* sums8,
                                       int a_lo, int a_hi, void* stream) {
    SGA_CHECK_ARG(Z && sums8 && Dp % 8 == 0 && A >= 0 && J1 >= 0 && J2 >= 0 && tau0 > 0 && tau1 > 0, "sga_loss_neg_sums: bad argument");
    SGA_CHECK_ARG(a_lo >= 0 && a_lo <= a_hi && a_hi <= A, "sga_loss_neg_sums: anchor shard [%d,%d) outside [0,%d]", a_lo, a_hi, A);
    hipStream_t s = static_cast<hipStream_t>(stream);
    if (int rc = zero_slots(sums8, 8, s, "sga_loss_neg_sums")) return rc;
    if (A == 0 || a_hi == a_lo || (J1 == 0 && J2 == 0)) return SGA_OK;
    SweepArgs a{};
    a.Z = Z; a.Dp = Dp; a.k0 = LOG2E / tau0; a.k1 = LOG2E / tau1; a.it0 = 1.f / tau0; a.it1 = 1.f / tau1;
    a.sums = sums8; a.gs = nullptr; a.dZ = nullptr; a.col0 = 0;
    fill_groups(a, A, J1, J2, false, a_lo, a_hi);
    const int nblk = total_blocks(a);
    const int jt = ((J1 > J2 ? J1 : J2) + 127) / 128;
    int gy = (8 * sga_num_cus() + nblk - 1) / nblk;
    if (gy > jt) gy = jt;
    if (gy < 1) gy = 1;
    if (Dp == 104) launch_sweep_fast<13, false>(a, nblk, gy, s);
    else if (Dp == 128) launch_sweep_fast<16, false>(a, nblk, gy, s);
    else launch_sweep<4, 1, false>(a, nblk, gy, s);
    fold_slots(sums8, 8, s);
    SGA_CHECK_LAUNCH("sga_loss_neg_sums");
    return SGA_OK;
}

extern "C" int sga_loss_neg_grad(const float* Z, int Dp, int A, int J1, int J2, float tau0, float tau1,
                                 const double* gs8, float* dZ, void* stream) {
    return sga_loss_neg_grad_shard(Z, Dp, A, J1, J2, tau0, tau1, gs8, dZ, 0, A, stream);
}

extern "C" int sga_loss_neg_grad_shard(const float* Z, int Dp, int A, int J1, int J2, float tau0, float tau1,
                                       const double* gs8, float* dZ, int a_lo, int a_hi, void* stream) {
    SGA_CHECK_ARG(Z && gs8 && dZ && Dp % 8 == 0 && A >= 0 && J1 >= 0 && J2 >= 0, "sga_loss_neg_grad: bad argument");
    SGA_CHECK_ARG(a_lo >= 0 && a_lo <= a_hi && a_hi <= A, "sga_loss_neg_grad: anchor shard [%d,%d) outside [0,%d]", a_lo, a_hi, A);
    hipStream_t s = static_cast<hipStream_t>(stream);
    if (A == 0 || a_hi == a_lo || (J1 == 0 && J2 == 0)) return SGA_OK;
    SweepArgs a{};
    a.Z = Z; a.Dp = Dp; a.k0 = LOG2E / tau0; a.k1 = LOG2E / tau1; a.it0 = 1.f / tau0; a.it1 = 1.f / tau1;
    a.sums = nullptr; a.gs = gs8; a.dZ = dZ;
    fill_groups(a, A, J1, J2, true, a_lo, a_hi);
    const int nblk = total_blocks(a);
    int mx = A > J1 ? A : J1;
    if (J2 > mx) mx = J2;
    int gy = (6 * sga_num_cus() + nblk - 1) / nblk;
    if (Dp <= 128) {
        const int jt = (mx + 127) / 128;
        if (gy > jt) gy = jt;
        if (gy < 1) gy = 1;
        a.col0 = 0;
        if (Dp == 104) launch_sweep_fast<13, true>(a, nblk, gy, s);
        else if (Dp == 128) launch_sweep_fast<16, true>(a, nblk, gy, s);
        else launch_sweep<4, 4, true>(a, nblk, gy, s);
    } else {
        const int jt = (mx + 63) / 64;
        if (gy > jt) gy = jt;
        if (gy < 1) gy = 1;
        for (int col0 = 0; col0 < Dp; col0 += 320) {
            a.col0 = col0;
            launch_sweep<2, 10, true>(a, nblk, gy, s);
        }
    }
    SGA_CHECK_LAUNCH("sga_loss_neg_grad");
    return SGA_OK;
}

extern "C" size_t sga_loss_neg_grad_wide_floats(int A, int J1, int J2) {
    return (size_t)2 * (size_t)(J1 + J2) * (size_t)((A + 31) / 32 * 32);
}

extern "C" int sga_loss_neg_grad_wide(const float* Z, int Dp, int A, int J1, int J2, float tau0, float tau1, const double* gs8,
                                      float* dZ, float* stash, size_t stash_floats, void* stream) {
    SGA_CHECK_ARG(Z && gs8 && dZ && stash && Dp % 8 == 0 && A >= 0 && J1 >= 0 && J2 >= 0, "sga_loss_neg_grad_wide: bad argument");
    hipStream_t s = static_cast<hipStream_t>(stream);
    const int J = J1 + J2;
    if (A == 0 || J == 0) return SGA_OK;
    size_t rows = stash_floats / ((size_t)2 * J);
    if (rows >= (size_t)A) rows = A; else rows = rows / 32 * 32;
    SGA_CHECK_ARG(rows >= 32 || rows == (size_t)A, "sga_loss_neg_grad_wide: workspace holds fewer than 32 anchor rows (%zu floats for J = %d)", stash_floats, J);
    const int n1 = 2 * A, n2 = 2 * A + J1;
    for (int lo = 0; lo < A; lo += (int)rows) {
        const int hi = lo + (int)rows < A ? lo + (int)rows : A, ns = hi - lo;
        CoefArgs a{};
        a.Z = Z; a.Dp = Dp; a.k0 = LOG2E / tau0; a.k1 = LOG2E / tau1; a.it0 = 1.f / tau0; a.it1 = 1.f / tau1; a.gs = gs8;
        a.ld = ns; a.n1 = n1;
        a.stash[0] = stash; a.stash[1] = stash + (size_t)J * ns;
        const int nb = (ns + 127) / 128;
        a.grp[0] = SweepGroup{lo, ns, 0, 2, {SweepSeg{n1, J1, 0}, SweepSeg{n2, J2, 1}}, 1};
        a.grp[1] = SweepGroup{A + lo, ns, nb, 2, {SweepSeg{n2, J2, 2}, SweepSeg{n1, J1, 3}}, 1};
        const int mx = J1 > J2 ? J1 : J2;
        int gy = (6 * sga_num_cus() + 2 * nb - 1) / (2 * nb);
        const int jt = (mx + 63) / 64;
        if (gy > jt) gy = jt;
        if (gy < 1) gy = 1;
        hipLaunchKernelGGL(sweep_coef_kernel<2>, dim3(2 * nb, gy), dim3(CT_THREADS), 0, s, a);
        SGA_CHECK_LAUNCH("sga_loss_neg_grad_wide");
        for (int g = 0; g < 2; ++g) {
            const float* C = a.stash[g];
            const size_t own_row = (size_t)(g == 0 ? lo : A + lo);
            int rc = sga_gemm(1, 0, ns, Dp, J, C, ns, 0, Z + (size_t)n1 * Dp, Dp, dZ + own_row * Dp, Dp, nullptr, 1, stream);
            if (rc) return rc;
            rc = sga_gemm(0, 0, J, Dp, ns, C, ns, 0, Z + own_row * Dp, Dp, dZ + (size_t)n1 * Dp, Dp, nullptr, 1, stream);
            if (rc) return rc;
        }
    }
    return SGA_OK;
}

static int fill_anchor(AnchorArgs& a, const float* const* Z, const int* Dp, int NT, int A, const double* sums,
                       float alpha, float tau_icl, float tau_ial, int a_lo, int a_hi) {
    if (NT < 1 || NT > CT_MAXT) { sga_set_error("sga_loss_anchor: NT=%d outside [1,%d]", NT, CT_MAXT); return SGA_ERR_ARG; }
    if (a_lo < 0 || a_hi > A || a_lo > a_hi) { sga_set_error("sga_loss_anchor: anchor shard [%d,%d) outside [0,%d]", a_lo, a_hi, A); return SGA_ERR_ARG; }
    a.NT = NT; a.A = A; a.sums = sums; a.alpha = alpha; a.i_lo = a_lo; a.i_hi = a_hi;
    a.kc = LOG2E / tau_icl; a.ki = LOG2E / tau_ial; a.itc = 1.f / tau_icl; a.iti = 1.f / tau_ial;
    for (int k = 0; k < NT; ++k) {
        if (!Z[k] || Dp[k] % 8) { sga_set_error("sga_loss_anchor: table %d null or Dp %% 8 != 0", k); return SGA_ERR_ARG; }
        a.Z[k] = Z[k]; a.Dp[k] = Dp[k];
    }
    return SGA_OK;
}

extern "C" int sga_loss_anchor_fwd(const float* const* Z, const int* Dp, int NT, int A, const double* sums,
                                   float alpha, float tau_icl, float tau_ial, double* out, int a_lo, int a_hi, void* stream) {
    return sga_loss_anchor_fwd_f16(Z, nullptr, Dp, NT, A, sums, alpha, tau_icl, tau_ial, out, a_lo, a_hi, nullptr, 0, stream);
}

static size_t anchor_ws_ldp(int ns) { return (size_t)(ns + 3) / 4 * 4; }
extern "C" size_t sga_loss_anchor_f16_ws_bytes(int NT, int A, int ns) {
    if (NT < 1 || A < 1 || ns < 1) return 256;
    return (size_t)NT * 2 * A * anchor_ws_ldp(ns) * sizeof(float) + 256;
}
static int anchor_pre_blocks(AnchorArgs& a, const void* const* Zh, void* ws, size_t ws_bytes, hipStream_t s, bool& pre) {
    pre = false;
    if (!ws) return SGA_OK;
    const int ns = a.i_hi - a.i_lo, A = a.A;
    if (ws_bytes < sga_loss_anchor_f16_ws_bytes(a.NT, A, ns)) {
        sga_set_error("sga_loss_anchor (f16): workspace of %zu bytes, %zu needed", ws_bytes, sga_loss_anchor_f16_ws_bytes(a.NT, A, ns));
        return SGA_ERR_WORKSPACE;
    }
    const size_t ldp = anchor_ws_ldp(ns);
    float* w = static_cast<float*>(ws);
    SgaW16Store e[8];
    int n = 0;
    for (int k = 0; k < a.NT; ++k) {
        const _Float16* zh = Zh ? static_cast<const _Float16*>(Zh[k]) : nullptr;
        const long dp = a.Dp[k];
        float* sp = w + (size_t)(2 * k) * A * ldp;
        float* sq = w + (size_t)(2 * k + 1) * A * ldp;
        a.SP[k] = sp; a.SQ[k] = sq;
        if (zh) {
            e[n++] = SgaW16Store{zh + (size_t)A * dp, dp, A, zh + (size_t)a.i_lo * dp, dp, ns, (int)dp, sp, (long)ldp};
            e[n++] = SgaW16Store{zh, dp, A, zh + (size_t)(A + a.i_lo) * dp, dp, ns, (int)dp, sq, (long)ldp};
        } else {
            const float* z = a.Z[k];
            if (int rc = sga_gemm(0, 1, A, ns, (int)dp, z + (size_t)A * dp, dp, 0, z + (size_t)a.i_lo * dp, dp, sp, (long)ldp, nullptr, 0, s)) return rc;
            if (int rc = sga_gemm(0, 1, A, ns, (int)dp, z, dp, 0, z + (size_t)(A + a.i_lo) * dp, dp, sq, (long)ldp, nullptr, 0, s)) return rc;
        }
        if (n == 8 || (k == a.NT - 1 && n > 0)) {
            if (int rc = sga_wide16_store_batch(e, n, s)) return rc;
            n = 0;
        }
    }
    a.ldp = (long)ldp;
    pre = true;
    return SGA_OK;
}

extern "C" int sga_loss_anchor_fwd_f16(const float* const* Z, const void* const* Zh, const int* Dp, int NT, int A, const double* sums,
                                       float alpha, float tau_icl, float tau_ial, double* out, int a_lo, int a_hi, void* ws, size_t ws_bytes,
                                       void* stream) {
    SGA_CHECK_ARG(Z && Dp && sums && out && A >= 0, "sga_loss_anchor_fwd: bad argument");
    hipStream_t s = static_cast<hipStream_t>(stream);
    const int M = NT > 1 ? NT - 1 : 0;
    if (int rc0 = zero_slots(out, NT + 2 * M, s, "sga_loss_anchor_fwd")) return rc0;
    if (A == 0 || a_hi <= a_lo) return SGA_OK;
    AnchorArgs a{};
    int rc = fill_anchor(a, Z, Dp, NT, A, sums, alpha, tau_icl, tau_ial, a_lo, a_hi);
    if (rc) return rc;
    a.out = out;
    for (int k = 0; k < NT; ++k) a.Zh[k] = Zh ? static_cast<const _Float16*>(Zh[k]) : nullptr;
    bool pre = false;
    if (int rcp = anchor_pre_blocks(a, Zh, ws, ws_bytes, s, pre)) return rcp;
    if (pre) hipLaunchKernelGGL((anchor_kernel<false, true>), dim3((a_hi - a_lo + 127) / 128, (A + 31) / 32), dim3(CT_THREADS), 0, s, a);
    else hipLaunchKernelGGL(anchor_kernel<false>, dim3((a_hi - a_lo + 127) / 128, (A + 63) / 64), dim3(CT_THREADS), 0, s, a);
    fold_slots(out, NT + 2 * M, s);
    SGA_CHECK_LAUNCH("sga_loss_anchor_fwd");
    return SGA_OK;
}

extern "C" int sga_loss_anchor_bwd(const float* const* Z, const int* Dp, int NT, int A, const double* sums,
                                   float alpha, float tau_icl, float tau_ial, const float* coef, float* const* M1,
                                   double* gs, int a_lo, int a_hi, void* stream) {
    return sga_loss_anchor_bwd_f16(Z, nullptr, Dp, NT, A, sums, alpha, tau_icl, tau_ial, coef, M1, gs, a_lo, a_hi, nullptr, 0, stream);
}

extern "C" int sga_loss_anchor_bwd_f16(const float* const* Z, const void* const* Zh, const int* Dp, int NT, int A, const double* sums,
                                       float alpha, float tau_icl, float tau_ial, const float* coef, float* const* M1,
                                       double* gs, int a_lo, int a_hi, void* ws, size_t ws_bytes, void* stream) {
    SGA_CHECK_ARG(Z && Dp && sums && coef && M1 && gs && A >= 0, "sga_loss_anchor_bwd: bad argument");
    hipStream_t s = static_cast<hipStream_t>(stream);
    if (int rc0 = zero_slots(gs, NT * 8, s, "sga_loss_anchor_bwd")) return rc0;
    if (A == 0 || a_hi <= a_lo) return SGA_OK;
    AnchorArgs a{};
    int rc = fill_anchor(a, Z, Dp, NT, A, sums, alpha, tau_icl, tau_ial, a_lo, a_hi);
    if (rc) return rc;
    a.coef = coef; a.gs = gs;
    for (int k = 0; k < NT; ++k) { SGA_CHECK_ARG(M1[k], "sga_loss_anchor_bwd: null stash %d", k); a.M1[k] = M1[k]; }
    for (int k = 0; k < NT; ++k) a.Zh[k] = Zh ? static_cast<const _Float16*>(Zh[k]) : nullptr;
    bool pre = false;
    if (int rcp = anchor_pre_blocks(a, Zh, ws, ws_bytes, s, pre)) return rcp;
    if (pre) hipLaunchKernelGGL((anchor_kernel<true, true>), dim3((a_hi - a_lo + 127) / 128, (A + 31) / 32), dim3(CT_THREADS), 0, s, a);
    else hipLaunchKernelGGL(anchor_kernel<true>, dim3((a_hi - a_lo + 127) / 128, (A + 63) / 64), dim3(CT_THREADS), 0, s, a);
    fold_slots(gs, NT * 8, s);
    SGA_CHECK_LAUNCH("sga_loss_anchor_bwd");
    return SGA_OK;
}

static int fill_multi(MultiArgs& a, const float* const* Z, int M, int D, const float* beta, int A, int J1, int J2, float tau0,
                      float tau1, bool grad, int a_lo, int a_hi) {
    if (D < 1 || D > 104) { sga_set_error("sga_loss_multi: D=%d outside [1,104] (the fused sweeps take Dp = 104 tables)", D); return SGA_ERR_ARG; }
    a.ktail = D > 100 ? 2 : (D > 96 ? 1 : 0);
    if (a_lo < 0 || a_hi > A || a_lo > a_hi) { sga_set_error("sga_loss_multi: anchor shard [%d,%d) outside [0,%d]", a_lo, a_hi, A); return SGA_ERR_ARG; }
    if (M < 2 || M > 4) { sga_set_error("sga_loss_multi: M=%d outside [2,4]", M); return SGA_ERR_ARG; }
    a.M = M;
    for (int m = 0; m < M; ++m) { if (!Z[m]) { sga_set_error("sga_loss_multi: null table"); return SGA_ERR_ARG; } a.Z[m] = Z[m]; }
    a.beta = beta; a.k0 = LOG2E / tau0; a.k1 = LOG2E / tau1; a.it0 = 1.f / tau0; a.it1 = 1.f / tau1;
    SweepArgs tmp{};
    fill_groups(tmp, A, J1, J2, grad, a_lo, a_hi);
    a.ngroups = tmp.ngroups;
    for (int g = 0; g < 4; ++g) a.grp[g] = tmp.grp[g];
    return SGA_OK;
}
static int plan_multi(MultiArgs& a, int target_steps, int own_rows = 128) {
    int nwg = 0;
    for (int g = 0; g < a.ngroups; ++g) {
        SweepGroup& G = a.grp[g];
        int steps = 0;
        for (int sg = 0; sg < G.nseg; ++sg) steps += (G.seg[sg].n + 31) / 32;
        int ns = (steps + target_steps - 1) / target_steps;
        if (ns < 1) ns = 1;
        G.nsplit = ns;
        G.blk0 = nwg;
        nwg += ((((G.nown + own_rows - 1) / own_rows) * ns + 7) / 8) * 8;
    }
    return nwg;
}

static int multi_sums_impl(const float* const* Z, int M, int D, bool centred, const float* beta, int A, int J1, int J2, float tau0,
                           float tau1, double* sums, int a_lo, int a_hi, void* stream) {
    SGA_CHECK_ARG(Z && beta && sums && A >= 0 && J1 >= 0 && J2 >= 0, "sga_loss_multi_sums: bad argument");
    hipStream_t s = static_cast<hipStream_t>(stream);
    if (int rc0 = zero_slots(sums, (M + 1) * 8, s, "sga_loss_multi_sums")) return rc0;
    if (A == 0 || a_hi <= a_lo || (J1 == 0 && J2 == 0)) return SGA_OK;
    MultiArgs a{};
    int rc = fill_multi(a, Z, M, D, beta, A, J1, J2, tau0, tau1, false, a_lo, a_hi);
    if (rc) return rc;
    a.swap_tail = centred ? 1 : 0;
    a.sums = sums;
    const int nwg = plan_multi(a, 160, S16_OWN);
    if (M == 2) launch_sweep16<2, false>(a, nwg, s);
    else if (M == 3) launch_sweep16<3, false>(a, nwg, s);
    else launch_sweep16x2<false>(a, nwg, s);
    fold_slots(sums, (M + 1) * 8, s);
    SGA_CHECK_LAUNCH("sga_loss_multi_sums");
    return SGA_OK;
}
extern "C" int sga_loss_multi_sums(const float* const* Z, int M, int D, const float* beta, int A, int J1, int J2, float tau0,
                                   float tau1, double* sums, int a_lo, int a_hi, void* stream) {
    return multi_sums_impl(Z, M, D, false, beta, A, J1, J2, tau0, tau1, sums, a_lo, a_hi, stream);
}
extern "C" int sga_loss_multi_sums_centred(const float* const* Zc, int M, const float* beta, int A, int J1, int J2, float tau0,
                                           float tau1, double* sums, int a_lo, int a_hi, void* stream) {
    return multi_sums_impl(Zc, M, 102, true, beta, A, J1, J2, tau0, tau1, sums, a_lo, a_hi, stream);
}

static int multi_grad_impl(const float* const* Z, int M, int D, bool centred, const float* beta, int A, int J1, int J2, float tau0,
                           float tau1, const double* gs, float* const* dZ, double* gamma, int a_lo, int a_hi,
                           void* stream) {
    SGA_CHECK_ARG(Z && beta && gs && dZ && gamma && A >= 0 && J1 >= 0 && J2 >= 0, "sga_loss_multi_grad: bad argument");
    hipStream_t s = static_cast<hipStream_t>(stream);
    if (int rcz = zero_slots(gamma, M > 0 ? M : 1, s, "sga_loss_multi_grad")) return rcz;
    if (A == 0 || a_hi <= a_lo || (J1 == 0 && J2 == 0)) return SGA_OK;
    MultiArgs a{};
    int rc = fill_multi(a, Z, M, D, beta, A, J1, J2, tau0, tau1, true, a_lo, a_hi);
    if (rc) return rc;
    a.swap_tail = centred ? 1 : 0;
    a.gs = gs; a.gamma = gamma;
    for (int m = 0; m < M; ++m) { SGA_CHECK_ARG(dZ[m], "sga_loss_multi_grad: null dZ"); a.dZ[m] = dZ[m]; }
    const int nwg = plan_multi(a, 160, S16_OWN);
    if (M == 2) launch_sweep16<2, true>(a, nwg, s);
    else if (M == 3) launch_sweep16<3, true>(a, nwg, s);
    else launch_sweep16x2<true>(a, nwg, s);
    fold_slots(gamma, M, s);
    SGA_CHECK_LAUNCH("sga_loss_multi_grad");
    return SGA_OK;
}
extern "C" int sga_loss_multi_grad(const float* const* Z, int M, int D, const float* beta, int A, int J1, int J2, float tau0,
                                   float tau1, const double* gs, float* const* dZ, double* gamma, int a_lo, int a_hi,
                                   void* stream) {
    return multi_grad_impl(Z, M, D, false, beta, A, J1, J2, tau0, tau1, gs, dZ, gamma, a_lo, a_hi, stream);
}
extern "C" int sga_loss_multi_grad_centred(const float* const* Zc, int M, const float* beta, int A, int J1, int J2, float tau0,
                                           float tau1, const double* gs, float* const* dZ, double* gamma, int a_lo, int a_hi,
                                           void* stream) {
    return multi_grad_impl(Zc, M, 102, true, beta, A, J1, J2, tau0, tau1, gs, dZ, gamma, a_lo, a_hi, stream);
}

extern "C" int sga_loss_build_joint(const float* const* Z, int M, const float* beta, int rows, float* ZJ, void* stream) {
    SGA_CHECK_ARG(Z && beta && ZJ && M >= 2 && M <= 4 && rows >= 0, "sga_loss_build_joint: bad argument");
    if (rows == 0) return SGA_OK;
    MultiArgs a{};
    a.M = M; a.beta = beta;
    for (int m = 0; m < M; ++m) a.Z[m] = Z[m];
    hipLaunchKernelGGL(build_joint_kernel, dim3(rows_grid(rows)), dim3(256), 0, static_cast<hipStream_t>(stream), a, ZJ, rows);
    SGA_CHECK_LAUNCH("sga_loss_build_joint");
    return SGA_OK;
}

extern "C" int sga_loss_fold_joint(const float* const* Z, int M, const float* beta, const float* dZJ, int rows,
                                   float* const* dZ, double* gamma2, void* stream) {
    SGA_CHECK_ARG(Z && beta && dZJ && dZ && gamma2 && M >= 2 && M <= 4 && rows >= 0, "sga_loss_fold_joint: bad argument");
    if (rows == 0) return SGA_OK;
    MultiArgs a{};
    a.M = M; a.beta = beta;
    for (int m = 0; m < M; ++m) { a.Z[m] = Z[m]; a.dZ[m] = dZ[m]; }
    hipLaunchKernelGGL(fold_joint_kernel, dim3(rows_grid(rows)), dim3(256), 0, static_cast<hipStream_t>(stream), a, dZJ, rows, gamma2);
    SGA_CHECK_LAUNCH("sga_loss_fold_joint");
    return SGA_OK;
}

extern "C" int sga_loss_check_norms(const float* nrm, int n, float* poison, void* stream) {
    SGA_CHECK_ARG(nrm && poison && n >= 0, "sga_loss_check_norms: bad argument");
    if (n == 0) return SGA_OK;
    hipLaunchKernelGGL(check_norms_kernel, dim3(64), dim3(256), 0, static_cast<hipStream_t>(stream), nrm, n, poison);
    SGA_CHECK_LAUNCH("sga_loss_check_norms");
    return SGA_OK;
}

extern "C" int sga_loss_slots(void) { return SGA_SLOTS; }

static void launch_stash(bool trans, int nct10, const float* M1, const float* X, float* out, int MR, int KR, int ldm, int ld,
                         int w, hipStream_t s) {
    const int gx = (MR + 127) / 128;
    int splits = (6 * sga_num_cus() + gx - 1) / gx;
    int kper = ((KR + splits - 1) / splits + 7) / 8 * 8;
    if (kper < 64) kper = 64;
    splits = (KR + kper - 1) / kper;
    dim3 grid(gx, splits), blk(256);
    if (trans) {
        if (nct10) hipLaunchKernelGGL((stash_gemm_kernel<10, true>), grid, blk, 0, s, M1, X, out, MR, KR, ldm, ld, w, kper);
        else hipLaunchKernelGGL((stash_gemm_kernel<4, true>), grid, blk, 0, s, M1, X, out, MR, KR, ldm, ld, w, kper);
    } else {
        if (nct10) hipLaunchKernelGGL((stash_gemm_kernel<10, false>), grid, blk, 0, s, M1, X, out, MR, KR, ldm, ld, w, kper);
        else hipLaunchKernelGGL((stash_gemm_kernel<4, false>), grid, blk, 0, s, M1, X, out, MR, KR, ldm, ld, w, kper);
    }
}

extern "C" int sga_loss_stash_grad(const float* M1, const float* Z, int A, int Dp, float* dZ, int a_lo, int a_hi, void* stream) {
    SGA_CHECK_ARG(M1 && Z && dZ && A >= 0 && Dp >= 8 && Dp % 8 == 0 && a_lo >= 0 && a_hi <= A && a_lo <= a_hi, "sga_loss_stash_grad: bad argument");
    const int ns = a_hi - a_lo;
    if (A == 0 || ns == 0) return SGA_OK;
    hipStream_t s = static_cast<hipStream_t>(stream);
    const float* X1 = Z + (size_t)a_lo * Dp;
    const float* X2 = Z + (size_t)A * Dp;
    if (ns % 4 == 0 && Dp % 4 == 0 && reinterpret_cast<uintptr_t>(M1) % 16 == 0 && reinterpret_cast<uintptr_t>(Z) % 16 == 0 &&
        reinterpret_cast<uintptr_t>(dZ) % 16 == 0) {
        int rc = sga_gemm(1, 0, ns, Dp, A, M1, ns, 0, X2, Dp, dZ + (size_t)a_lo * Dp, Dp, nullptr, 1, stream);
        if (rc) return rc;
        return sga_gemm(0, 0, A, Dp, ns, M1, ns, 0, X1, Dp, dZ + (size_t)A * Dp, Dp, nullptr, 1, stream);
    }
    for (int c0 = 0; c0 < Dp; c0 += 320) {
        const int w = Dp - c0 < 320 ? Dp - c0 : 320;
        launch_stash(true, w > 128, M1, X2 + c0, dZ + (size_t)a_lo * Dp + c0, ns, A, ns, Dp, w, s);
        launch_stash(false, w > 128, M1, X1 + c0, dZ + (size_t)A * Dp + c0, A, ns, ns, Dp, w, s);
    }
    SGA_CHECK_LAUNCH("sga_loss_stash_grad");
    return SGA_OK;
}

static int fill_anchor_multi(AnchorMultiArgs& a, const float* const* Z, int M, const float* beta, int A, const double* sums,
                             float alpha, float tau_icl, float tau_ial, int a_lo, int a_hi) {
    if (M < 2 || M > 4) { sga_set_error("sga_loss_anchor_multi: M=%d not in {2,3,4} (use the per-table kernels)", M); return SGA_ERR_ARG; }
    if (a_lo < 0 || a_hi > A || a_lo > a_hi) { sga_set_error("sga_loss_anchor_multi: anchor shard [%d,%d) outside [0,%d]", a_lo, a_hi, A); return SGA_ERR_ARG; }
    a.M = M; a.A = A; a.i_lo = a_lo; a.i_hi = a_hi; a.beta = beta; a.sums = sums; a.alpha = alpha;
    a.kc = LOG2E / tau_icl; a.ki = LOG2E / tau_ial; a.itc = 1.f / tau_icl; a.iti = 1.f / tau_ial;
    for (int m = 0; m < M; ++m) { if (!Z[m]) { sga_set_error("sga_loss_anchor_multi: null table"); return SGA_ERR_ARG; } a.Z[m] = Z[m]; }
    const int nib = (a_hi - a_lo + 31) / 32, ntile = (A + 31) / 32;
    int ns = (4 * sga_num_cus() + nib - 1) / (nib > 0 ? nib : 1);
    if (ns > (ntile + 3) / 4) ns = (ntile + 3) / 4;
    if (ns < 1) ns = 1;
    a.nsplit = ns;
    return SGA_OK;
}

template <int M, bool BWD>
static void launch_anchor_multi(const AnchorMultiArgs& a, hipStream_t s) {
    const size_t lds = (size_t)(M * 2 * 32 * 104 + (M + 1) * 8) * sizeof(float);
    auto k = anchor_multi_kernel<M, BWD>;
    hipFuncSetAttribute(reinterpret_cast<const void*>(k), hipFuncAttributeMaxDynamicSharedMemorySize, (int)lds);
    const int nib = (a.i_hi - a.i_lo + 31) / 32;
    hipLaunchKernelGGL(k, dim3(nib * a.nsplit), dim3(CT_THREADS), lds, s, a);
}

extern "C" int sga_loss_anchor_multi_fwd(const float* const* Z, int M, const float* beta, int A, const double* sums,
                                         float alpha, float tau_icl, float tau_ial, double* out, int a_lo, int a_hi,
                                         void* stream) {
    SGA_CHECK_ARG(Z && beta && sums && out && A >= 0, "sga_loss_anchor_multi_fwd: bad argument");
    hipStream_t s = static_cast<hipStream_t>(stream);
    const int n = (M + 1) + 2 * M;
    if (int rc0 = zero_slots(out, n, s, "sga_loss_anchor_multi_fwd")) return rc0;
    if (A == 0 || a_hi <= a_lo) return SGA_OK;
    AnchorMultiArgs a{};
    int rc = fill_anchor_multi(a, Z, M, beta, A, sums, alpha, tau_icl, tau_ial, a_lo, a_hi);
    if (rc) return rc;
    a.out = out;
    if (M == 2) launch_anchor_multi<2, false>(a, s); else if (M == 3) launch_anchor_multi<3, false>(a, s); else launch_anchor_multi<4, false>(a, s);
    fold_slots(out, n, s);
    SGA_CHECK_LAUNCH("sga_loss_anchor_multi_fwd");
    return SGA_OK;
}

extern "C" int sga_loss_anchor_multi_bwd(const float* const* Z, int M, const float* beta, int A, const double* sums,
                                         float alpha, float tau_icl, float tau_ial, const float* coef, float* const* M1,
                                         double* gs, double* gamma, int a_lo, int a_hi, double* out_terms, void* stream) {
    SGA_CHECK_ARG(Z && beta && sums && coef && M1 && gs && gamma && A >= 0, "sga_loss_anchor_multi_bwd: bad argument");
    hipStream_t s = static_cast<hipStream_t>(stream);
    if (int rc0 = zero_slots(gs, (M + 1) * 8, s, "sga_loss_anchor_multi_bwd")) return rc0;
    if (int rc1 = zero_slots(gamma, M, s, "sga_loss_anchor_multi_bwd")) return rc1;
    if (out_terms) { if (int rc2 = zero_slots(out_terms, (M + 1) + 2 * M, s, "sga_loss_anchor_multi_bwd")) return rc2; }
    if (A == 0 || a_hi <= a_lo) return SGA_OK;
    AnchorMultiArgs a{};
    int rc = fill_anchor_multi(a, Z, M, beta, A, sums, alpha, tau_icl, tau_ial, a_lo, a_hi);
    if (rc) return rc;
    a.coef = coef; a.gs = gs; a.gamma = gamma;
    float* inv = reinterpret_cast<float*>(gs + (size_t)(1 + SGA_SLOTS) * (M + 1) * 8);
    hipLaunchKernelGGL(inv_sums_kernel, dim3(1), dim3(64), 0, s, sums, inv, (M + 1) * 8);
    a.inv = inv;
    for (int m = 0; m < M; ++m) { SGA_CHECK_ARG(M1[m], "sga_loss_anchor_multi_bwd: null stash"); a.M1[m] = M1[m]; }
    {
        const int RB = M <= 3 ? 32 : 16, TW = M <= 3 ? 2 : 4;
        const size_t lds = (size_t)(M * 2 * RB * 104 + (M + 1) * 8) * sizeof(float);
        const int nib = (a.i_hi - a.i_lo + RB - 1) / RB, ntile16 = (A + 15) / 16;
        int nsp = (6 * sga_num_cus() + nib - 1) / (nib > 0 ? nib : 1);
        if (nsp > (ntile16 + TW - 1) / TW) nsp = (ntile16 + TW - 1) / TW;
        if (nsp < 1) nsp = 1;
        a.nsplit = nsp;
        a.out = out_terms;
        auto go = [&](auto k) {
            hipFuncSetAttribute(reinterpret_cast<const void*>(k), hipFuncAttributeMaxDynamicSharedMemorySize, (int)lds);
            hipLaunchKernelGGL(k, dim3(nib * nsp), dim3(CT_THREADS), lds, s, a);
        };
        if (out_terms) { if (M == 2) go(anchor_multi_bwd16_kernel<2, true>); else if (M == 3) go(anchor_multi_bwd16_kernel<3, true>); else go(anchor_multi_bwd16_kernel<4, true>); }
        else { if (M == 2) go(anchor_multi_bwd16_kernel<2, false>); else if (M == 3) go(anchor_multi_bwd16_kernel<3, false>); else go(anchor_multi_bwd16_kernel<4, false>); }
    }
    if (out_terms) fold_slots(out_terms, (M + 1) + 2 * M, s);
    fold_slots(gs, (M + 1) * 8, s);
    fold_slots(gamma, M, s);
    SGA_CHECK_LAUNCH("sga_loss_anchor_multi_bwd");
    return SGA_OK;
}

static int symx_impl(const float* const* Z, int M, const float* beta, int A, const double* sums, float alpha,
                     float tau_icl, float tau_ial, const float* coef, float* const* M1, float* const* M2,
                     double* gs, double* gamma, int a_lo, int a_hi, int j_lo, int j_hi, int mir, double* out_terms,
                     void* stream);

extern "C" int sga_loss_anchor_multi_bwd_symx(const float* const* Z, int M, const float* beta, int A, const double* sums, float alpha,
                                              float tau_icl, float tau_ial, const float* coef, float* const* M1, float* const* M2,
                                              double* gs, double* gamma, int a_lo, int a_hi, int j_lo, int j_hi, int mir, double* out_terms,
                                              void* stream) {
    return symx_impl(Z, M, beta, A, sums, alpha, tau_icl, tau_ial, coef, M1, M2, gs, gamma, a_lo, a_hi, j_lo, j_hi, mir, out_terms, stream);
}

static int symx_impl(const float* const* Z, int M, const float* beta, int A, const double* sums, float alpha,
                     float tau_icl, float tau_ial, const float* coef, float* const* M1, float* const* M2,
                     double* gs, double* gamma, int a_lo, int a_hi, int j_lo, int j_hi, int mir, double* out_terms,
                     void* stream) {
    SGA_CHECK_ARG(Z && beta && sums && coef && M1 && M2 && gs && gamma && out_terms && A >= 0, "sga_loss_anchor_multi_bwd_symx: bad argument");
    SGA_CHECK_ARG(M >= 2 && M <= 4, "sga_loss_anchor_multi_bwd_symx: M=%d (2, 3 or 4)", M);
    SGA_CHECK_ARG(a_lo % 32 == 0 && (a_hi % 32 == 0 || a_hi == A), "sga_loss_anchor_multi_bwd_symx: block [%d,%d) not on 32-row boundaries", a_lo, a_hi);
    SGA_CHECK_ARG(j_lo >= 0 && j_lo % 16 == 0 && j_hi <= A && j_lo <= j_hi && (j_hi % 16 == 0 || j_hi == A) && mir >= j_lo && (mir % 16 == 0 || mir >= j_hi),
                  "sga_loss_anchor_multi_bwd_symx: columns [%d,%d) / mirror start %d not on 16-column boundaries", j_lo, j_hi, mir);
    SGA_CHECK_ARG(mir <= j_lo || (j_lo >= a_lo && (mir < j_hi ? mir : j_hi) <= a_hi), "sga_loss_anchor_multi_bwd_symx: ordered columns [%d,%d) outside the block's square [%d,%d)",
                  j_lo, mir, a_lo, a_hi);
    hipStream_t s = static_cast<hipStream_t>(stream);
    if (int rc0 = zero_slots(gs, (M + 1) * 8, s, "sga_loss_anchor_multi_bwd_symx")) return rc0;
    if (int rc1 = zero_slots(gamma, M, s, "sga_loss_anchor_multi_bwd_symx")) return rc1;
    if (int rc2 = zero_slots(out_terms, (M + 1) + 2 * M, s, "sga_loss_anchor_multi_bwd_symx")) return rc2;
    if (A == 0 || a_hi <= a_lo || j_hi <= j_lo) return SGA_OK;
    AnchorMultiArgs a{};
    int rc = fill_anchor_multi(a, Z, M, beta, A, sums, alpha, tau_icl, tau_ial, a_lo, a_hi);
    if (rc) return rc;
    a.coef = coef; a.gs = gs; a.gamma = gamma; a.out = out_terms; a.j_lo = j_lo; a.j_hi = j_hi; a.mir = mir;
    float* inv = reinterpret_cast<float*>(gs + (size_t)(1 + SGA_SLOTS) * (M + 1) * 8);
    hipLaunchKernelGGL(inv_sums_kernel, dim3(1), dim3(64), 0, s, sums, inv, (M + 1) * 8);
    a.inv = inv;
    for (int m = 0; m < M; ++m) {
        SGA_CHECK_ARG(M1[m] && (M2[m] || mir >= j_hi), "sga_loss_anchor_multi_bwd_symx: null stash");
        a.M1[m] = M1[m]; a.M2[m] = M2[m];
    }
    const int RB = M <= 3 ? 32 : 16, TW = M <= 3 ? 2 : 4;
    const size_t lds = (size_t)(M * 2 * RB * 104 + (M + 1) * 8) * sizeof(float);
    const int nib = (a_hi - a_lo + RB - 1) / RB, ntile16 = (j_hi - j_lo + 15) / 16;
    int nsp = (6 * sga_num_cus() + nib - 1) / nib;
    if (nsp > (ntile16 + TW - 1) / TW) nsp = (ntile16 + TW - 1) / TW;
    if (nsp < 1) nsp = 1;
    a.nsplit = nsp;
    auto go = [&](auto k) {
        hipFuncSetAttribute(reinterpret_cast<const void*>(k), hipFuncAttributeMaxDynamicSharedMemorySize, (int)lds);
        hipLaunchKernelGGL(k, dim3(nib * nsp), dim3(CT_THREADS), lds, s, a);
    };
    if (M == 2) go(anchor_multi_bwd16_kernel<2, true, 32, true>);
    else if (M == 3) go(anchor_multi_bwd16_kernel<3, true, 32, true>);
    else go(anchor_multi_bwd16_kernel<4, true, 16, true>);
    fold_slots(out_terms, (M + 1) + 2 * M, s);
    fold_slots(gs, (M + 1) * 8, s);
    fold_slots(gamma, M, s);
    SGA_CHECK_LAUNCH("sga_loss_anchor_multi_bwd_symx");
    return SGA_OK;
}

extern "C" int sga_loss_anchor_multi_bwd_sym(const float* const* Z, int M, const float* beta, int A, const double* sums, float alpha,
                                             float tau_icl, float tau_ial, const float* coef, float* const* M1, float* const* M2,
                                             double* gs, double* gamma, int a_lo, int a_hi, double* out_terms, void* stream) {
    return sga_loss_anchor_multi_bwd_symx(Z, M, beta, A, sums, alpha, tau_icl, tau_ial, coef, M1, M2, gs, gamma, a_lo, a_hi, a_lo, A, a_hi, out_terms, stream);
}

extern "C" int sga_loss_stash_grad_symx(const float* M1, const float* M2, const float* Z, int A, int Dp, float* dZ, int a_lo, int a_hi,
                                        int j_lo, int j_hi, int mir, void* stream) {
    SGA_CHECK_ARG(M1 && Z && dZ && A >= 0 && Dp >= 8 && Dp % 8 == 0 && a_lo >= 0 && a_hi <= A && a_lo <= a_hi && j_lo >= 0 && j_lo <= j_hi && j_hi <= A &&
                  mir >= j_lo && (M2 || mir >= j_hi), "sga_loss_stash_grad_symx: bad argument");
    const int ns = a_hi - a_lo, c1 = j_hi - j_lo, c2 = mir < j_hi ? j_hi - mir : 0;
    if (A == 0 || ns == 0 || c1 == 0) return SGA_OK;
    const float* X1 = Z;
    const float* X2 = Z + (size_t)A * Dp;
    float* d1 = dZ;
    float* d2 = dZ + (size_t)A * Dp;
    int rc = sga_gemm(1, 0, ns, Dp, c1, M1, ns, 0, X2 + (size_t)j_lo * Dp, Dp, d1 + (size_t)a_lo * Dp, Dp, nullptr, 1, stream);
    if (!rc) rc = sga_gemm(0, 0, c1, Dp, ns, M1, ns, 0, X1 + (size_t)a_lo * Dp, Dp, d2 + (size_t)j_lo * Dp, Dp, nullptr, 1, stream);
    if (!rc && c2 > 0) rc = sga_gemm(0, 0, c2, Dp, ns, M2, ns, 0, X2 + (size_t)a_lo * Dp, Dp, d1 + (size_t)mir * Dp, Dp, nullptr, 1, stream);
    if (!rc && c2 > 0) rc = sga_gemm(1, 0, ns, Dp, c2, M2, ns, 0, X1 + (size_t)mir * Dp, Dp, d2 + (size_t)a_lo * Dp, Dp, nullptr, 1, stream);
    return rc;
}

extern "C" int sga_loss_stash_grad_sym(const float* M1, const float* M2, const float* Z, int A, int Dp, float* dZ, int a_lo, int a_hi,
                                       void* stream) {
    return sga_loss_stash_grad_symx(M1, M2, Z, A, Dp, dZ, a_lo, a_hi, a_lo, A, a_hi, stream);
}
```

sgaligner_amd/csrc/sweep3.hip:

```cpp
#include <stdlib.h>
#include <type_traits>

#include "loss_math.h"

namespace {

typedef __bf16 bf16x8 __attribute__((ext_vector_type(8)));
typedef __bf16 bf16x2 __attribute__((ext_vector_type(2)));
typedef float f32x2 __attribute__((ext_vector_type(2)));
typedef unsigned int u32x4 __attribute__((ext_vector_type(4)));
typedef unsigned int u32x2 __attribute__((ext_vector_type(2)));
typedef short s16x4 __attribute__((ext_vector_type(4)));

constexpr int S3_DP = 104;
constexpr int S3_PLANE = 3 * 2 * 1024;
constexpr int S3_TAIL = 3 * S3_PLANE;
constexpr int S3_BLOCK = S3_TAIL + 2048;
constexpr int S3_NCH = S3_BLOCK / 1024;
constexpr int S3_ROWSLOTS = 3 * 12 + 4;

__device__ __forceinline__ void split3_pair(float v0, float v1, unsigned& h, unsigned& m, unsigned& l) {
    const bf16x2 H = __builtin_convertvector(f32x2{v0, v1}, bf16x2);
    const unsigned hu = __builtin_bit_cast(unsigned, H);
#ifdef S3_SPLIT_DOT2
    unsigned c0 = 0x0000BF80u, c1 = 0xBF800000u;
    asm("" : "+s"(c0), "+s"(c1));
    const bf16x2 n0 = __builtin_bit_cast(bf16x2, c0), n1 = __builtin_bit_cast(bf16x2, c1);
    const float r0 = __builtin_amdgcn_fdot2_f32_bf16(H, n0, v0, false);
    const float r1 = __builtin_amdgcn_fdot2_f32_bf16(H, n1, v1, false);
#else
    const float r0 = v0 - __builtin_bit_cast(float, hu << 16);
    const float r1 = v1 - __builtin_bit_cast(float, hu & 0xffff0000u);
#endif
    const bf16x2 Mi = __builtin_convertvector(f32x2{r0, r1}, bf16x2);
    const unsigned mu = __builtin_bit_cast(unsigned, Mi);
#ifdef S3_SPLIT_DOT2
    const float s0 = __builtin_amdgcn_fdot2_f32_bf16(Mi, n0, r0, false);
    const float s1 = __builtin_amdgcn_fdot2_f32_bf16(Mi, n1, r1, false);
#else
    const float s0 = r0 - __builtin_bit_cast(float, mu << 16);
    const float s1 = r1 - __builtin_bit_cast(float, mu & 0xffff0000u);
#endif
    const bf16x2 Lo = __builtin_convertvector(f32x2{s0, s1}, bf16x2);
    h = hu; m = mu; l = __builtin_bit_cast(unsigned, Lo);
}
__device__ __forceinline__ f32x4 mfma_b(u32x4 a, u32x4 b, f32x4 c) {
    return __builtin_amdgcn_mfma_f32_16x16x32_bf16(__builtin_bit_cast(bf16x8, a), __builtin_bit_cast(bf16x8, b), c, 0, 0, 0);
}
__device__ __forceinline__ u32x2 tr_read16(const unsigned char* p) {
    return __builtin_bit_cast(u32x2, __builtin_amdgcn_ds_read_tr16_b64_v4i16((__attribute__((address_space(3))) s16x4*)(p)));
}
__device__ __forceinline__ unsigned long long sreg64(unsigned long long v) {
    const unsigned lo = __builtin_amdgcn_readfirstlane((unsigned)v), hi = __builtin_amdgcn_readfirstlane((unsigned)(v >> 32));
    return ((unsigned long long)hi << 32) | lo;
}
template <int X, int END, int NR, bool VALU_ALL> __device__ __forceinline__ void sgb_seq() {
    if constexpr (X < END) {
        __builtin_amdgcn_sched_group_barrier(0x008, 1, 0);
        if constexpr (X < NR) __builtin_amdgcn_sched_group_barrier(0x100, 1, 0);
        if constexpr (VALU_ALL || X < 2) __builtin_amdgcn_sched_group_barrier(0x002, 2, 0);
        sgb_seq<X + 1, END, NR, VALU_ALL>();
    }
}
__host__ __device__ constexpr int s3_slot(int g, int i) { return 16 * g + (i ^ (12 * (g & 1))); }

struct TLayout { int nbA, nb1, nb2; };
__host__ __device__ inline TLayout make_tlayout(int A, int J1, int J2) { return TLayout{(A + 31) / 32, (J1 + 31) / 32, (J2 + 31) / 32}; }

constexpr int S3_STAT_BYTES = 2048;
constexpr int S3_DREAL = 100;

constexpr int S3_CS_BLOCKS = 256;
__global__ __launch_bounds__(128) void split3_colsum_kernel(const float* __restrict__ Z, int R, double* __restrict__ part) {
    const int c = threadIdx.x;
    const int per = (R + gridDim.x - 1) / gridDim.x, r0 = blockIdx.x * per, r1 = min(R, r0 + per);
    if (c >= S3_DP) return;
    double acc = 0.0;
    for (int r = r0; r < r1; ++r) acc += (double)Z[(size_t)r * S3_DP + c];
    part[(size_t)blockIdx.x * S3_DP + c] = acc;
}
__global__ __launch_bounds__(128) void split3_stats_kernel(const double* __restrict__ part, int nblocks, int R, float* __restrict__ stat) {
    __shared__ double sq[128];
    const int c = threadIdx.x;
    double cs = 0.0;
    if (c < S3_DP) for (int b = 0; b < nblocks; ++b) cs += part[(size_t)b * S3_DP + c];
    float zb = (c < S3_DREAL && R > 0) ? (float)(cs / (double)R) : 0.f;
    sq[c] = (double)zb * (double)zb;
    __syncthreads();
    __shared__ double tot;
    if (c == 0) {
        double t = 0.0;
        for (int i = 0; i < 128; ++i) t += sq[i];
        tot = t;
    }
    __syncthreads();
    const bool centre = tot >= 0.25;
    if (!centre) zb = 0.f;
    if (c < S3_DP) stat[c] = zb;
    if (c == 0) { stat[S3_DP] = centre ? (float)(0.5 * tot) : 0.f; stat[S3_DP + 1] = centre ? 1.f : 0.f; }
}

__global__ __launch_bounds__(256) void split3_tables_kernel(const float* __restrict__ Z, int A, int J1, int J2, unsigned char* __restrict__ Zb,
                                                            const float* __restrict__ stat, float* __restrict__ Zc) {
    __shared__ float tile[32 * S3_DP];
    __shared__ float zbar[S3_DP];
    const TLayout L = make_tlayout(A, J1, J2);
    int b = blockIdx.x, old0, len;
    if (b < L.nbA) { old0 = 0; len = A; }
    else if (b < 2 * L.nbA) { b -= L.nbA; old0 = A; len = A; }
    else if (b < 2 * L.nbA + L.nb1) { b -= 2 * L.nbA; old0 = 2 * A; len = J1; }
    else { b -= 2 * L.nbA + L.nb1; old0 = 2 * A + J1; len = J2; }
    const int nvalid = min(32, len - 32 * b);
    const float* src = Z + (size_t)(old0 + 32 * b) * S3_DP;
    if (threadIdx.x < S3_DP) zbar[threadIdx.x] = stat[threadIdx.x];
    __syncthreads();
    for (int e = threadIdx.x; e < 32 * S3_DP; e += 256) {
        const int r = e / S3_DP, c = e - r * S3_DP;
        tile[e] = (r < nvalid && c < S3_DREAL) ? src[e] - zbar[c] : 0.f;
        if (Zc && old0 < 2 * A && r < nvalid) Zc[(size_t)(old0 + 32 * b) * S3_DP + e] = c == S3_DREAL + 1 ? 1.f : tile[e];
    }
    __syncthreads();
    if (threadIdx.x < 32) {
        const int r = threadIdx.x;
        if (r < nvalid) {
            double a = 0.0;
            for (int c = 0; c < S3_DREAL; ++c) a += (double)zbar[c] * (double)tile[r * S3_DP + c];
            tile[r * S3_DP + S3_DREAL] = (float)(a + (double)stat[S3_DP]);
            tile[r * S3_DP + S3_DREAL + 1] = 1.f;
        }
    }
    __syncthreads();
    unsigned* out = reinterpret_cast<unsigned*>(Zb + (size_t)blockIdx.x * S3_BLOCK);
    for (int e = threadIdx.x; e < 3 * 2 * 64 * 4; e += 256) {
        const int p = e & 3, st = (e >> 2) & 63, jh = (e >> 8) & 1, q = e >> 9;
        const int g = st >> 4, i = (st & 15) ^ (12 * (g & 1));
        const int row = 8 * (i >> 2) + 4 * jh + (i & 3), col = 32 * q + 8 * g + 2 * p;
        unsigned h, m, l;
        split3_pair(tile[row * S3_DP + col], tile[row * S3_DP + col + 1], h, m, l);
        out[e] = h; out[S3_PLANE / 4 + e] = m; out[2 * S3_PLANE / 4 + e] = l;
    }
    for (int e = threadIdx.x; e < 2 * 64 * 4; e += 256) {
        const int p = e & 3, st = (e >> 2) & 63, jh = (e >> 8) & 1;
        const int g = st >> 4, i = (st & 15) ^ (12 * (g & 1));
        const int row = 8 * (i >> 2) + 4 * jh + (i & 3), col = 96 + 2 * p;
        unsigned h, m, l;
        split3_pair(tile[row * S3_DP + col], tile[row * S3_DP + col + 1], h, m, l);
        out[S3_TAIL / 4 + e] = g < 2 ? h : (g == 2 ? m : l);
    }
}


__global__ __launch_bounds__(256) void centre_tables_kernel(const float* __restrict__ Z, int R, const float* __restrict__ stat, float* __restrict__ Zc) {
    const int lane = threadIdx.x & 63, wpb = blockDim.x >> 6;
    for (int r = blockIdx.x * wpb + (threadIdx.x >> 6); r < R; r += gridDim.x * wpb) {
        const float* z = Z + (size_t)r * S3_DP;
        float* o = Zc + (size_t)r * S3_DP;
        double acc = 0.0;
        float v[2];
#pragma unroll
        for (int t = 0; t < 2; ++t) {
            const int d = lane + 64 * t;
            const float zb = d < S3_DREAL ? stat[d] : 0.f;
            v[t] = d < S3_DREAL ? z[d] - zb : 0.f;
            acc += (double)zb * (double)v[t];
        }
        acc = wave_sum_d(acc);
        o[lane] = v[0];
        const int d1 = lane + 64;
        if (d1 < S3_DP) o[d1] = d1 < S3_DREAL ? v[1] : (d1 == S3_DREAL ? (float)(acc + (double)stat[S3_DP]) : (d1 == S3_DREAL + 1 ? 1.f : 0.f));
    }
}

#ifdef S3_DBG_TIMING
__device__ unsigned long long g_s3_dbg[16];
#define S3_T(i) { const unsigned long long t_ = __builtin_readcyclecounter(); tacc[i] += t_ - tprev; tprev = t_; }
#else
#define S3_T(i)
#endif
struct TSeg { int blk0, jt_lo, jt_hi, old0, lo, hi, fam; };
struct TGroup { int own0, nown, own_old0, own_blk0, blk0, nsplit, nseg; TSeg seg[2]; };
struct TArgs {
    int M; const unsigned char* Zb[4]; int perm[4]; int ngroups; TGroup grp[4];
    float k0, k1, it0, it1, ka;
    const float* beta;
    double* sums;
    const double* gs;
    float* dZ[4];
    double* gamma;
};

template <int M, bool GRAD, int WV, int MG = M, bool GAM = true, bool LITE = false, bool FOLD = false>
__global__ __launch_bounds__(WV * 64, WV == 8 ? 2 : 1) void sweep3_kernel(TArgs a) {
    static_assert(!LITE || !GRAD, "LITE: the forward sums only");
    static_assert(!FOLD || (GRAD && WV == 4), "FOLD: the one-wave-per-SIMD gradient sweep only");
    constexpr int NCT = 7;
    constexpr int WAVES = WV, THREADS = WAVES * 64;
    constexpr int OWN = WV * 16;
    constexpr int NCH = LITE ? S3_NCH - S3_PLANE / 1024 : S3_NCH;
    constexpr int KMAX = (NCH + WAVES - 1) / WAVES;
    constexpr int BUF = M * S3_BLOCK;
    constexpr bool PIPE = WV == 4;
#ifndef S3_OWN_IN_S
#define S3_OWN_IN_S 1
#endif
    constexpr bool OWN_IN_S = GRAD && PIPE && S3_OWN_IN_S;
#ifndef S3_SPREAD
#define S3_SPREAD 1
#endif
    constexpr bool SPREAD = OWN_IN_S && S3_SPREAD && !FOLD;
    extern __shared__ __attribute__((aligned(16))) unsigned char lds3[];

    const int tid = threadIdx.x, lane = tid & 63, wave = tid >> 6, g4 = lane >> 4, l15 = lane & 15;
    int g = 0;
#pragma unroll
    for (int i = 1; i < 4; ++i) if (i < a.ngroups && (int)blockIdx.x >= a.grp[i].blk0) g = i;
    const TGroup& grp = a.grp[g];
    const int wg_in_grp = (int)blockIdx.x - grp.blk0;
    const int nsplit = grp.nsplit, n_ob = (grp.nown + OWN - 1) / OWN, n_units = n_ob * nsplit;
    const int unit = (wg_in_grp & 7) * ((n_units + 7) >> 3) + (wg_in_grp >> 3);
    if ((wg_in_grp >> 3) >= ((n_units + 7) >> 3) || unit >= n_units) return;
    const int split = unit / n_ob;
    const int own0 = grp.own0 + (unit - split * n_ob) * OWN;
    const int own_end = grp.own0 + grp.nown;
    const int wrow0 = own0 + wave * 16;
#ifdef S3_DBG_TIMING
    unsigned long long tacc[8] = {0, 0, 0, 0, 0, 0, 0, 0}, tprev = __builtin_readcyclecounter();
#endif

    u32x4 opl[M][3][3], otl[M][2];
    float beta[M];
    const bool iv = wrow0 + l15 < own_end;
    {
        const int my_i = wrow0 + l15;
        const int rel = (iv ? my_i : own0) - grp.own_old0;
        const int o = rel & 31, oi = 4 * (o >> 3) + (o & 3), ojh = (o >> 2) & 1;
        const size_t off = (size_t)(grp.own_blk0 + (rel >> 5)) * S3_BLOCK;
#pragma unroll
        for (int m = 0; m < M; ++m) {
            const unsigned char* base = a.Zb[m] + off;
#pragma unroll
            for (int p = 0; p < 3; ++p)
#pragma unroll
                for (int q = 0; q < 3; ++q) {
                    const int so = ((q * 2 + ojh) * 64 + s3_slot(g4, oi)) * 16;
                    opl[m][p][q] = iv ? *reinterpret_cast<const u32x4*>(base + p * S3_PLANE + so) : u32x4{0, 0, 0, 0};
                }
            u32x4 th = iv ? *reinterpret_cast<const u32x4*>(base + S3_TAIL + (ojh * 64 + s3_slot(0, oi)) * 16) : u32x4{0, 0, 0, 0};
            u32x4 tm = iv ? *reinterpret_cast<const u32x4*>(base + S3_TAIL + (ojh * 64 + s3_slot(2, oi)) * 16) : u32x4{0, 0, 0, 0};
            u32x4 tl = iv ? *reinterpret_cast<const u32x4*>(base + S3_TAIL + (ojh * 64 + s3_slot(3, oi)) * 16) : u32x4{0, 0, 0, 0};
            const float ksc = a.k1;
            auto rescale = [&](u32x4& ph, u32x4& pm, u32x4& pl) {
#pragma unroll
                for (int d = 0; d < 4; ++d) {
                    const float x0 = (__builtin_bit_cast(float, ph[d] << 16) + __builtin_bit_cast(float, pm[d] << 16)) + __builtin_bit_cast(float, pl[d] << 16);
                    const float x1 = (__builtin_bit_cast(float, ph[d] & 0xffff0000u) + __builtin_bit_cast(float, pm[d] & 0xffff0000u)) + __builtin_bit_cast(float, pl[d] & 0xffff0000u);
                    unsigned nh, nm, nl;
                    split3_pair(x0 * ksc, x1 * ksc, nh, nm, nl);
                    ph[d] = nh; pm[d] = nm; pl[d] = nl;
                }
            };
#pragma unroll
            for (int q = 0; q < 3; ++q) rescale(opl[m][0][q], opl[m][1][q], opl[m][2][q]);
            rescale(th, tm, tl);
            otl[m][0] = g4 == 1 ? tm : th;
            otl[m][1] = g4 == 0 ? tl : (g4 == 2 ? tm : u32x4{0, 0, 0, 0});
#pragma unroll
            for (int t = 0; t < 2; ++t)
                otl[m][t][2] = (otl[m][t][2] >> 16) | (otl[m][t][2] << 16);
        }
    }
#pragma unroll
    for (int m = 0; m < M; ++m) beta[m] = a.beta[a.perm[m]];

    constexpr int NSM = GRAD ? (FOLD ? 1 : MG) : 1;
    f32x4 gacc[GRAD ? MG : 1][NCT], gsm[NSM][NCT];
#pragma unroll
    for (int m = 0; m < (GRAD ? MG : 1); ++m)
#pragma unroll
        for (int ct = 0; ct < NCT; ++ct) gacc[m][ct] = f32x4{0.f, 0.f, 0.f, 0.f};
#pragma unroll
    for (int m = 0; m < NSM; ++m)
#pragma unroll
        for (int ct = 0; ct < NCT; ++ct) gsm[m][ct] = f32x4{0.f, 0.f, 0.f, 0.f};
    float gam[M];
#pragma unroll
    for (int m = 0; m < M; ++m) gam[m] = 0.f;

    const int wave_u = __builtin_amdgcn_readfirstlane(wave);
    unsigned l16 = threadIdx.x;
    asm volatile("" : "+v"(l16));
    l16 = (l16 & 63u) * 16u;
    unsigned long long tb[M];
    auto set_tile = [&](int blk) {
#pragma unroll
        for (int m = 0; m < M; ++m) tb[m] = sreg64(reinterpret_cast<unsigned long long>(a.Zb[m]) + (unsigned long long)blk * S3_BLOCK);
    };
    auto issue_slots = [&](unsigned char* buf, int f_lo, int f_hi) {
#ifdef S3_DBG_NODMA
        return;
#endif
#pragma unroll
        for (int f = f_lo; f < f_hi; ++f) {
            if (f >= M * KMAX) break;
            const int m = f / KMAX, k = f % KMAX;
            const int rot = (wave_u + m) & (WAVES - 1);
            int c = rot + k * WAVES;
            if ((k + 1) * WAVES > NCH) c = c >= NCH ? c - WAVES : c;
            if (LITE) c = c >= 2 * (S3_PLANE / 1024) ? c + S3_PLANE / 1024 : c;
            __builtin_amdgcn_global_load_lds((const __attribute__((address_space(1))) void*)(reinterpret_cast<const unsigned char*>(tb[m] + (unsigned)(c * 1024)) + l16),
                                             (__attribute__((address_space(3))) void*)(buf + m * S3_BLOCK + c * 1024), 16, 0, 0);
        }
    };
    auto issue = [&](int blk, unsigned char* buf) { set_tile(blk); issue_slots(buf, 0, M * KMAX); };

    const int aoff = s3_slot(g4, l15) * 16;
    const int tr_io = 4 * g4 + (l15 >> 2), tr_cs = l15 & 3;
    const int tr_main = s3_slot(tr_cs >> 1, tr_io) * 16 + (tr_cs & 1) * 8;
    const int tr_tail = S3_TAIL + tr_io * 16 + (tr_cs & 1) * 8;
    const int tr_tail_l = S3_TAIL + (48 + (tr_io ^ 12)) * 16 + (tr_cs & 1) * 8;

#pragma unroll 1
    for (int sg = 0; sg < 2; ++sg) {
        if (sg >= grp.nseg) break;
        const TSeg seg = grp.seg[sg];
        float c0[M + 1], c1[M + 1];
#pragma unroll
        for (int m = 0; m <= M; ++m) {
            const int mo = m < M ? a.perm[m] : M;
            c0[m] = GRAD ? (float)(a.gs[mo * 8 + seg.fam * 2 + 0] * (double)a.it0) : 0.f;
            c1[m] = GRAD ? (float)(a.gs[mo * 8 + seg.fam * 2 + 1] * (double)a.it1) : 0.f;
        }
        const float ka = a.ka;
        double dsum[M + 1][2];
#pragma unroll
        for (int m = 0; m <= M; ++m) { dsum[m][0] = 0.0; dsum[m][1] = 0.0; }
        float pl0[LITE ? M + 1 : 1], pl1[LITE ? M + 1 : 1];
#pragma unroll
        for (int m = 0; m < (LITE ? M + 1 : 1); ++m) { pl0[m] = 0.f; pl1[m] = 0.f; }

        __syncthreads();
        if (seg.jt_lo + split < seg.jt_hi) issue(seg.blk0 + seg.jt_lo + split, lds3);
        int it = 0;
#pragma unroll 1
        for (int jt = seg.jt_lo + split; jt < seg.jt_hi; jt += nsplit, ++it) {
            unsigned char* buf = lds3 + (it & 1) * BUF;
            const int j0 = seg.old0 + 32 * jt;
            S3_T(5)
            __syncthreads();
            S3_T(0)
            const int next_blk = seg.blk0 + (jt + nsplit < seg.jt_hi ? jt + nsplit : jt);
            unsigned char* next_buf = lds3 + ((it + 1) & 1) * BUF;
            set_tile(next_blk);
            S3_T(1)
            if (GRAD) {
                const int vlo = max(seg.lo - j0, 0), vhi = min(seg.hi - j0, 32);
                if (vlo > 0 || vhi < 32) {
                    for (int x = tid; x < M * 32 * S3_ROWSLOTS; x += THREADS) {
                        const int pc = x % S3_ROWSLOTS, w = (x / S3_ROWSLOTS) % 32, m = x / (S3_ROWSLOTS * 32);
                        if (w >= vlo && w < vhi) continue;
                        const int wjh = (w >> 2) & 1, wi = 4 * (w >> 3) + (w & 3);
                        unsigned char* base = buf + m * S3_BLOCK;
                        if (pc < 36) {
                            const int pl = pc / 12, q = (pc % 12) >> 2, gq = pc & 3;
                            *reinterpret_cast<u32x4*>(base + pl * S3_PLANE + ((q * 2 + wjh) * 64 + s3_slot(gq, wi)) * 16) = u32x4{0, 0, 0, 0};
                        } else {
                            const int gq = pc - 36;
                            *reinterpret_cast<u32x4*>(base + S3_TAIL + (wjh * 64 + s3_slot(gq, wi)) * 16) = u32x4{0, 0, 0, 0};
// ... 768 lines not shown
```

sgaligner_amd/loss_ops.py:

```python
from __future__ import annotations

import ctypes as _ct

import numpy as _np
import torch

from . import _lib
from . import ops as _o
from .ops import (_SmallCache, _ev_start, _ev_stop, _fingerprint, _h2d, _p, _ptr_array, _req, _stream, get_mfma_mode, DEFERRED_CHECKS, IndexSets,
                  _POINTNET_MODE, _stash_bytes, cast_f32, colsum, gemm)

def _anchor_chunks(a_lo, a_hi, A, n_tables):
    ns = a_hi - a_lo
    if ns <= 0 or A <= 0:
        return []
    rows = max(32, (_stash_bytes() // (4 * A * max(1, n_tables))) // 32 * 32)
    return [(c, min(c + rows, a_hi)) for c in range(a_lo, a_hi, rows)]


def _sym_chunks(A, n_tables):
    return [(lo, hi) for lo, hi, _, _, _ in _sym_jobs([0, A], 0, n_tables)]


def _sym_jobs(cuts, rank, n_tables):
# ... 180 lines not shown
                if _o.KERNEL_EVENTS is not None:
                    ev16 = (torch.cuda.Event(enable_timing=True), torch.cuda.Event(enable_timing=True))
                    ev16[0].record()
                _lib.check(L.sga_loss_neg_grad_f16(_p(zhs[k]), _p(zts[k]), dp, A, s.J1, s.J2, TAU_ICL, TAU_IAL, gs[k].data_ptr(), _p(dz),
                                                   _p(stash), have, a_lo, a_hi, st), 'sga_loss_neg_grad_f16')
                if ev16 is not None:
                    ev16[1].record()
                    _o.KERNEL_EVENTS.setdefault('wide16_grad', []).append(ev16 + ((A, s.J1, s.J2, dp),))
                del stash
            elif dp > 128 and _o.WIDE_STASH and a_lo == 0 and a_hi == A:
                need = int(L.sga_loss_neg_grad_wide_floats(A, s.J1, s.J2))
                have = max(min(need, _stash_bytes() // 4), 2 * (s.J1 + s.J2) * min(A, 32))
                stash = torch.empty((have,), device=dev, dtype=torch.float32)
                _lib.check(L.sga_loss_neg_grad_wide(_p(z), dp, A, s.J1, s.J2, TAU_ICL, TAU_IAL, gs[k].data_ptr(), _p(dz), _p(stash), have, st),
                           'sga_loss_neg_grad_wide')
                del stash
            else:
                _lib.check(L.sga_loss_neg_grad_shard(_p(z), dp, A, s.J1, s.J2, TAU_ICL, TAU_IAL, gs[k].data_ptr(), _p(dz), a_lo, a_hi, st),
                           'sga_loss_neg_grad')
            if ev is not None:
                ev[1].record()
                _o.KERNEL_EVENTS.setdefault('sweep_kernel<4,4,grad>', []).append(ev + ((A, s.J1, s.J2, dp),))
            t, d = ctx.shapes[k]
            de = torch.zeros((t, d), device=dev, dtype=torch.float32)
            _lib.check(L.sga_loss_scatter(_p(dz), _p(z), _p(nrms[k]), _p(s.idx), s.R, d, dp, _p(de), st), 'sga_loss_scatter')
            grads.append(de)
            dzs[k] = None
        return (None, None, None, None, *grads)


def contrastive_terms(tables, data_dict, alpha=ALPHA, shard=None, reduce=None):
    s = IndexSets.of(data_dict, tables[0].device, int(tables[0].shape[0]))
    return ContrastiveTermsFn.apply(s, alpha, shard, reduce, *tables), s


class LossHeadFn(torch.autograd.Function):

    @staticmethod
    def forward(ctx, sums, lv_ial, lv_icl, n_anchors, z_ial, alpha_ial, zoom):
        M = int(lv_ial.numel())
        if sums.dtype not in (torch.float32, torch.float64) or sums.numel() != 3 * M + 1 or lv_icl.numel() != M:
            raise RuntimeError('sgaligner_amd: LossHeadFn takes the 3M+1 loss terms (float32/float64) and two [M] log_vars vectors')
        sums = sums.contiguous()
        la, lc = _req(lv_ial.detach(), 'log_vars (ial)'), _req(lv_icl.detach(), 'log_vars (icl)')
        out = torch.empty((4,), device=sums.device, dtype=torch.float64)
        inv_aa = 1.0 / float(n_anchors * n_anchors) if n_anchors else float('nan')
        ctx.consts = (M, inv_aa, float(z_ial), float(alpha_ial), float(zoom))
        ctx.f64 = int(sums.dtype == torch.float64)
        _lib.check(_lib.lib().sga_loss_head_fwd(_p(sums), ctx.f64, _p(la), _p(lc), *ctx.consts, _p(out), _stream()), 'sga_loss_head_fwd')
        ctx.save_for_backward(sums, la, lc)
        return out

    @staticmethod
    def coef_hint(lv_ial, lv_icl, n_anchors, z_ial, alpha_ial, zoom):
        M = int(lv_ial.numel())
        la, lc = _req(lv_ial.detach(), 'log_vars (ial)'), _req(lv_icl.detach(), 'log_vars (icl)')
        dev = la.device
        key = (str(dev), M)
        cst = LossHeadFn._hint_const.get(key)
        if cst is None:
            cst = LossHeadFn._hint_const[key] = (torch.tensor([1.0, 0.0, 0.0, 0.0], device=dev, dtype=torch.float64),
                                                 torch.zeros((3 * M + 1,), device=dev, dtype=torch.float32))
        inv_aa = 1.0 / float(n_anchors * n_anchors) if n_anchors else float('nan')
        d = torch.empty((3 * M + 1,), device=dev, dtype=torch.float32)
        junk = torch.empty((2, M), device=dev, dtype=torch.float32)
        _lib.check(_lib.lib().sga_loss_head_bwd(_p(cst[0]), _p(cst[1]), 0, _p(la), _p(lc), M, inv_aa, float(z_ial), float(alpha_ial), float(zoom),
                                                _p(d), _p(junk[0]), _p(junk[1]), _stream()), 'sga_loss_head_bwd')
        return d

    _hint_const = {}

    @staticmethod
    def backward(ctx, gout):
        sums, la, lc = ctx.saved_tensors
        M = ctx.consts[0]
        gout = gout.to(torch.float64).contiguous()
        dsums = torch.empty_like(sums)
        dla, dlc = torch.empty_like(la), torch.empty_like(lc)
        _lib.check(_lib.lib().sga_loss_head_bwd(_p(gout), _p(sums), ctx.f64, _p(la), _p(lc), *ctx.consts, _p(dsums), _p(dla), _p(dlc),
                                                _stream()), 'sga_loss_head_bwd')
        return dsums, dla, dlc, None, None, None, None


class LossGroups:

    def __init__(self, data_dict, b, device):
        ca = _np.asarray(data_dict['e1i_count']).reshape(-1).astype(_np.int64)
        c1 = _np.asarray(data_dict['e1j_count']).reshape(-1).astype(_np.int64)
        c2 = _np.asarray(data_dict['e2j_count']).reshape(-1).astype(_np.int64)
        if not (len(ca) == len(c1) == len(c2)):
            raise RuntimeError('sgaligner_amd: e1i_count / e1j_count / e2j_count disagree')
        if int(b) < 1:
            raise RuntimeError(f'sgaligner_amd: loss_group must be a positive number of pairs (got {b})')
        B = len(ca)
        cuts = list(range(0, B, int(b))) + [B]
        oa, o1, o2 = (_np.concatenate([[0], _np.cumsum(c)]) for c in (ca, c1, c2))
        g = _np.zeros((len(cuts) - 1, 8), dtype=_np.int32)
        for k, (lo, hi) in enumerate(zip(cuts[:-1], cuts[1:])):
            g[k, :6] = (oa[lo], oa[hi] - oa[lo], o1[lo], o1[hi] - o1[lo], o2[lo], o2[hi] - o2[lo])
        size = 2 * g[:, 1].astype(_np.int64) * (g[:, 1].astype(_np.int64) + g[:, 3] + g[:, 5])
        soff = _np.concatenate([[0], _np.cumsum(size)]).astype(_np.int64)
        self.G, self.b = int(g.shape[0]), int(b)
        self.host = g
        self.s_total = int(soff[-1])
        self.groups = torch.from_numpy(g).to(device)
        self.soff = torch.from_numpy(soff).to(device)
        self.na = torch.from_numpy(g[:, 1].astype(_np.float32)).to(device)
        self.totals = (int(oa[-1]), int(o1[-1]), int(o2[-1]))

    _cache = _SmallCache()

    @staticmethod
    def of(data_dict, b, device):
        device = torch.device(device)
        key = _fingerprint([_np.asarray(data_dict[k]) for k in ('e1i_count', 'e1j_count', 'e2j_count')], (str(device), int(b)))
        return LossGroups._cache.get(key, lambda: LossGroups(data_dict, b, device))


class GroupedContrastiveFn(torch.autograd.Function):

    @staticmethod
    def forward(ctx, index_sets, groups, alpha, beta, *tables):
        L = _lib.lib()
        M = len(tables)
        nt = M + 1 if M > 1 else 1
        no = nt + (2 * M if M > 1 else 0)
        tables = [_req(t.contiguous(), f'table[{i}]') for i, t in enumerate(tables)]
        dev = tables[0].device
        s, gr = index_sets, groups
        if (s.A, s.J1, s.J2) != gr.totals:
            raise RuntimeError('sgaligner_amd: per-pair counts (e1i_count/e1j_count/e2j_count) do not add up to the index sets')
        st = _stream()
        dp = 104
        T = tables[0].shape[0]
        zs, nrms = [], []
        poison = torch.zeros((1,), device=dev, dtype=torch.float32)
        for e in tables:
            d = e.shape[1]
            if d > dp:
                raise RuntimeError('sgaligner_amd: loss_group needs emb_dim <= 104')
            z = torch.empty((max(s.R, 1), dp), device=dev, dtype=torch.float32)
            nrm = torch.empty((max(s.R, 1),), device=dev, dtype=torch.float32)
            _lib.check(L.sga_loss_gather(_p(e), T, d, _p(s.idx), s.R, _p(z), dp, _p(nrm), st), 'sga_loss_gather')
            _lib.check(L.sga_loss_check_norms(_p(nrm), s.R, _p(poison), st), 'sga_loss_check_norms')
            zs.append(z); nrms.append(nrm)
        if beta is not None:
            beta = _req(beta.contiguous(), 'beta')
        S = torch.empty((M * max(gr.s_total, 1),), device=dev, dtype=torch.float32)
        sums = torch.empty((max(gr.G, 1), nt, 8), device=dev, dtype=torch.float64)
        out = torch.zeros((max(gr.G, 1), no), device=dev, dtype=torch.float64)
        _lib.check(L.sga_group_loss_fwd(_ptr_array(zs), M, _p(beta), s.A, s.J1, _p(gr.groups), gr.G, _p(gr.soff), gr.s_total,
                                        float(alpha), TAU_ICL, TAU_IAL, _p(S), _p(sums), _p(out), int(_o.GROUP_LOSS_VALU), st), 'sga_group_loss_fwd')
        ctx.s, ctx.gr, ctx.alpha, ctx.M = s, gr, float(alpha), M
        ctx.shapes = [tuple(t.shape) for t in tables]
        ctx.has_beta = beta is not None
        ctx.save_for_backward(S, sums, *( [beta] if beta is not None else []), *zs, *nrms)
        return out[:gr.G].float() + poison

    @staticmethod
    def backward(ctx, gout):
        L = _lib.lib()
        s, gr, M = ctx.s, ctx.gr, ctx.M
        saved = list(ctx.saved_tensors)
        S, sums = saved[0], saved[1]
        beta = saved[2] if ctx.has_beta else None
        rest = saved[3:] if ctx.has_beta else saved[2:]
        zs, nrms = rest[:M], rest[M:]
        dev = S.device
        st = _stream()
        dp = 104
        coef = gout.contiguous().float()
        C = S.clone()
        dzs = [torch.zeros((max(s.R, 1), dp), device=dev, dtype=torch.float32) for _ in range(M)]
        gamma = torch.zeros((max(gr.G, 1), M), device=dev, dtype=torch.float64)
        _lib.check(L.sga_group_loss_bwd(_ptr_array(zs), M, _p(beta), s.A, s.J1, _p(gr.groups), gr.G, _p(gr.soff), gr.s_total,
                                        ctx.alpha, TAU_ICL, TAU_IAL, _p(C), _p(sums), _p(coef), _ptr_array(dzs), _p(gamma), int(_o.GROUP_LOSS_VALU), st),
                   'sga_group_loss_bwd')
        grads = []
        for k in range(M):
            t, d = ctx.shapes[k]
            de = torch.zeros((t, d), device=dev, dtype=torch.float32)
            _lib.check(L.sga_loss_scatter(_p(dzs[k]), _p(zs[k]), _p(nrms[k]), _p(s.idx), s.R, d, dp, _p(de), st), 'sga_loss_scatter')
            grads.append(de)
        gbeta = gamma[:gr.G].sum(0).float() if ctx.has_beta else None
        return (None, None, None, gbeta, *grads)


def grouped_contrastive_terms(tables, fusion_weight, data_dict, b, alpha=ALPHA):
    dev = tables[0].device
    s = IndexSets.of(data_dict, dev, int(tables[0].shape[0]))
    gr = LossGroups.of(data_dict, b, dev)
    beta = None
    if len(tables) > 1:
        w = torch.softmax(fusion_weight.reshape(-1), dim=0)
        beta = (w * w) / (w * w).sum()
    return GroupedContrastiveFn.apply(s, gr, alpha, beta, *tables), gr


def group_data_dicts(data_dict, b):
    ca, c1, c2 = (_np.asarray(data_dict[k]).reshape(-1) for k in ('e1i_count', 'e1j_count', 'e2j_count'))
    oa, o1, o2 = (_np.concatenate([[0], _np.cumsum(c)]) for c in (ca, c1, c2))
    B = len(ca)
    out = []
    for lo in range(0, B, int(b)):
        hi = min(B, lo + int(b))
        out.append({'e1i': _np.asarray(data_dict['e1i'])[oa[lo]:oa[hi]], 'e2i': _np.asarray(data_dict['e2i'])[oa[lo]:oa[hi]],
                    'e1j': _np.asarray(data_dict['e1j'])[o1[lo]:o1[hi]], 'e2j': _np.asarray(data_dict['e2j'])[o2[lo]:o2[hi]]})
    return out


def _sums_lite(ns, J1, J2):
    if _o.BF16X6_SUMS_LITE is not None:
        return bool(_o.BF16X6_SUMS_LITE)
    return ns * min(J1, J2) >= _o.BF16X6_SUMS_LITE_MIN_TERMS


def _allreduce_sum(t, group_reduce):
    if group_reduce is not None:
        group_reduce(t)
    return t


class FusedContrastiveFn(torch.autograd.Function):

    @staticmethod
    def forward(ctx, index_sets, alpha, shard, reduce, coef_hint, beta, *tables):
        L = _lib.lib()
        M = len(tables)
        nt = M + 1
        tables = [_req(t.contiguous(), f'table[{i}]') for i, t in enumerate(tables)]
        beta = _req(beta.contiguous(), 'beta')
        dev = tables[0].device
        s = index_sets
        a_lo, a_hi = (0, s.A) if shard is None else (int(shard[0]), int(shard[1]))
        T = tables[0].shape[0]
        st = _stream()
        dp = 104
        zs, nrms = [], []
        poison = torch.zeros((1,), device=dev, dtype=torch.float32)
        for k, e in enumerate(tables):
            d = e.shape[1]
            if d > dp:
                raise RuntimeError('sgaligner_amd: the fused loss path needs emb_dim <= 104')
            z = torch.empty((s.R + 32, dp), device=dev, dtype=torch.float32)
            z[s.R:].zero_()
            nrm = torch.empty((s.R,), device=dev, dtype=torch.float32)
            _lib.check(L.sga_loss_gather(_p(e), T, d, _p(s.idx), s.R, _p(z), dp, _p(nrm), st), 'sga_loss_gather')
            _lib.check(L.sga_loss_check_norms(_p(nrm), s.R, _p(poison), st), 'sga_loss_check_norms')
            zs.append(z); nrms.append(nrm)
        zarr = _ptr_array(zs)
        slots = 1 + L.sga_loss_slots()
        sums = torch.empty((slots, nt, 8), device=dev, dtype=torch.float64)
        dmax = max(e.shape[1] for e in tables)
        zbs, zcs = [], []
        split3 = centred32 = False
        if M in (2, 3, 4) and dmax <= 100 and _o.FUSED_ANCHOR_BWD and get_mfma_mode() in ('bf16x6', 'f16'):
            split3 = True
            nb = L.sga_loss_split3_bytes(s.A, s.J1, s.J2)
            for z in zs:
                zb = torch.empty((nb,), device=dev, dtype=torch.uint8)
                zc = torch.empty((2 * s.A + 32, dp), device=dev, dtype=torch.float32)
                zc[2 * s.A:].zero_()
                _lib.check(L.sga_loss_split3_tables(_p(z), s.A, s.J1, s.J2, _p(zb), _p(zc), st), 'sga_loss_split3_tables')
                zbs.append(zb); zcs.append(zc)
            ev = None
            if _o.KERNEL_EVENTS is not None:
                ev = (torch.cuda.Event(enable_timing=True), torch.cuda.Event(enable_timing=True))
                ev[0].record()
            lite = _sums_lite(a_hi - a_lo, s.J1, s.J2)
            _lib.check(L.sga_loss_multi_sums_bf16x6(_ptr_array(zbs), M, _p(beta), s.A, s.J1, s.J2, TAU_ICL, TAU_IAL, _p(sums),
                                                    a_lo, a_hi, 1 if lite else 0, st), 'sga_loss_multi_sums_bf16x6')
            if ev is not None:
                ev[1].record()
                _o.KERNEL_EVENTS.setdefault('loss_multi_sums_bf16x6', []).append(ev + ((a_hi - a_lo, s.A, s.J1, s.J2, M, bool(lite)),))
        elif M in (2, 3, 4) and dmax <= 100 and _o.FUSED_ANCHOR_BWD and _o.CENTRED_F32:
            centred32 = True
            nst = int(L.sga_loss_centre_bytes())
            for z in zs:
                zc = torch.empty((s.R + 32, dp), device=dev, dtype=torch.float32)
                zc[s.R:].zero_()
                stw = torch.empty((nst,), device=dev, dtype=torch.uint8)
                _lib.check(L.sga_loss_centre_tables(_p(z), s.A, s.J1, s.J2, _p(zc), _p(stw), st), 'sga_loss_centre_tables')
                zbs.append(stw); zcs.append(zc)
            ev = None
            if _o.KERNEL_EVENTS is not None:
                ev = (torch.cuda.Event(enable_timing=True), torch.cuda.Event(enable_timing=True))
                ev[0].record()
            _lib.check(L.sga_loss_multi_sums_centred(_ptr_array(zcs), M, _p(beta), s.A, s.J1, s.J2, TAU_ICL, TAU_IAL, _p(sums), a_lo, a_hi, st),
                       'sga_loss_multi_sums_centred')
            if ev is not None:
                ev[1].record()
                _o.KERNEL_EVENTS.setdefault('loss_multi_sums', []).append(ev + ((a_hi - a_lo, s.A, s.J1, s.J2, M),))
        else:
            ev = None
            if _o.KERNEL_EVENTS is not None:
                ev = (torch.cuda.Event(enable_timing=True), torch.cuda.Event(enable_timing=True))
                ev[0].record()
            _lib.check(L.sga_loss_multi_sums(zarr, M, dmax, _p(beta), s.A, s.J1, s.J2, TAU_ICL, TAU_IAL, _p(sums), a_lo, a_hi, st),
                       'sga_loss_multi_sums')
            if ev is not None:
                ev[1].record()
                _o.KERNEL_EVENTS.setdefault('loss_multi_sums', []).append(ev + ((a_hi - a_lo, s.A, s.J1, s.J2, M),))
        sums = _allreduce_sum(sums[0].contiguous(), reduce)
        zj = torch.empty((2 * s.A, M * dp), device=dev, dtype=torch.float32)
        _lib.check(L.sga_loss_build_joint(zarr, M, _p(beta), 2 * s.A, _p(zj), st), 'sga_loss_build_joint')
        out = torch.empty((slots * (nt + 2 * M),), device=dev, dtype=torch.float64)
        dps = [dp] * M + [M * dp]
        onepass = coef_hint is not None and M <= 4 and _o.FUSED_ANCHOR_BWD and _o.FUSED_AA_ONEPASS and s.A >= _o.ONEPASS_MIN_ANCHORS
        extra = []
        if onepass:
            coef = _req(coef_hint.contiguous(), 'coef_hint')
            n_terms = nt + 2 * M
            dz_all = torch.zeros((M, s.R, dp), device=dev, dtype=torch.float32)
            zz = torch.zeros((n_terms + nt * 8 + M,), device=dev, dtype=torch.float64)
            out_acc, gs_aa, gam_aa = zz[:n_terms], zz[n_terms:n_terms + nt * 8].view(nt, 8), zz[n_terms + nt * 8:]
            cuts, crank = (shard[2], shard[3]) if (shard is not None and len(shard) >= 4) else (([0, s.A], 0) if (a_lo == 0 and a_hi == s.A) else (None, 0))
            sym = _o.AA_SYMMETRIC and M <= _o.AA_SYMMETRIC_MAX_M and cuts is not None and all(c % 32 == 0 for c in cuts[:-1]) and cuts[-1] == s.A \
                and cuts[crank] == a_lo and cuts[crank + 1] == a_hi
            jobs = _sym_jobs(list(cuts), crank, M) if sym else []
            chunks = jobs if sym else _anchor_chunks(a_lo, a_hi, s.A, M)
            if sym and len(cuts) == 2 and len(jobs) < 2:
                sym, chunks = False, _anchor_chunks(a_lo, a_hi, s.A, M)
            if chunks:
                gsc = torch.empty((slots + 1, nt, 8), device=dev, dtype=torch.float64)
                gam2 = torch.empty((slots, M), device=dev, dtype=torch.float64)
            if chunks and sym:
                fl = max(((jh - jl) + max(0, jh - mir)) * (hi - lo) for lo, hi, jl, jh, mir in chunks)
                buf = [torch.empty((fl,), device=dev, dtype=torch.float32) for _ in range(M)]
                for lo, hi, jl, jh, mir in chunks:
                    n1 = (jh - jl) * (hi - lo)
                    m1 = [b[:n1] for b in buf]
                    m2 = [b[n1:] for b in buf]
                    has2 = mir < jh
                    _lib.check(L.sga_loss_anchor_multi_bwd_symx(zarr, M, _p(beta), s.A, _p(sums), float(alpha), TAU_ICL, TAU_IAL, _p(coef),
                                     _ptr_array(m1), _ptr_array(m2) if has2 else (_ct.c_void_p * M)(), _p(gsc), _p(gam2),
                                     lo, hi, jl, jh, mir, _p(out), st), 'sga_loss_anchor_multi_bwd_symx')
                    out_acc += out[:n_terms]
                    gs_aa += gsc[0]
                    gam_aa += gam2[0]
                    for k in range(M):
                        if split3 and _o.BF16X6_STASH:
                            _lib.check(L.sga_loss_stash_grad_symx_bf16x6(_p(m1[k]), _p(m2[k]) if has2 else None, _p(zbs[k]), s.A, s.J1, s.J2,
                                                                         _p(dz_all[k]), lo, hi, jl, jh, mir, st), 'sga_loss_stash_grad_symx_bf16x6')
                        else:
                            _lib.check(L.sga_loss_stash_grad_symx(_p(m1[k]), _p(m2[k]) if has2 else None, _p(zcs[k] if (split3 or centred32) else zs[k]), s.A, dp,
                                                                  _p(dz_all[k]), lo, hi, jl, jh, mir, st), 'sga_loss_stash_grad_symx')
                del buf, m1, m2
            elif chunks:
                cmax = max(hi - lo for lo, hi in chunks)
                m1 = [torch.empty((s.A * cmax,), device=dev, dtype=torch.float32) for _ in range(M)]
                for lo, hi in chunks:
                    _lib.check(L.sga_loss_anchor_multi_bwd(zarr, M, _p(beta), s.A, _p(sums), float(alpha), TAU_ICL, TAU_IAL, _p(coef),
                                                           _ptr_array(m1), _p(gsc), _p(gam2), lo, hi, _p(out), st), 'sga_loss_anchor_multi_bwd')
                    out_acc += out[:n_terms]
                    gs_aa += gsc[0]
                    gam_aa += gam2[0]
                    for k in range(M):
                        if split3 and _o.BF16X6_STASH:
                            _lib.check(L.sga_loss_stash_grad_symx_bf16x6(_p(m1[k]), None, _p(zbs[k]), s.A, s.J1, s.J2, _p(dz_all[k]), lo, hi, 0, s.A, s.A, st),
                                       'sga_loss_stash_grad_symx_bf16x6')
                        else:
                            _lib.check(L.sga_loss_stash_grad(_p(m1[k]), _p(zcs[k] if (split3 or centred32) else zs[k]), s.A, dp, _p(dz_all[k]), lo, hi, st), 'sga_loss_stash_grad')
                del m1
            out = _allreduce_sum(out_acc.clone(), reduce)
            extra = [dz_all, gs_aa.clone(), gam_aa.clone(), coef]
        else:
            if M <= 4 and _o.FUSED_ANCHOR_FWD:
                _lib.check(L.sga_loss_anchor_multi_fwd(zarr, M, _p(beta), s.A, _p(sums), float(alpha), TAU_ICL, TAU_IAL, _p(out),
                                                       a_lo, a_hi, st), 'sga_loss_anchor_multi_fwd')
            else:
                _lib.check(L.sga_loss_anchor_fwd(_ptr_array(zs + [zj]), (_ct.c_int * nt)(*dps), nt, s.A, _p(sums), float(alpha),
                                                 TAU_ICL, TAU_IAL, _p(out), a_lo, a_hi, st), 'sga_loss_anchor_fwd')
            out = _allreduce_sum(out[:nt + 2 * M].contiguous(), reduce)
        ctx.s, ctx.alpha, ctx.M, ctx.shard, ctx.reduce = s, float(alpha), M, (a_lo, a_hi), reduce
        ctx.shapes = [tuple(t.shape) for t in tables]
        ctx.n_zb = len(zbs)
        ctx.split3 = split3
        ctx.centred32 = centred32
        ctx.onepass = onepass
        ctx.n_zc = len(zcs)
        ctx.save_for_backward(sums, beta, zj, *zs, *nrms, *zbs, *zcs, *extra)
        return out.float() + poison

    @staticmethod
    def backward(ctx, gout):
        L = _lib.lib()
        s, M = ctx.s, ctx.M
        a_lo, a_hi = ctx.shard
        ns = a_hi - a_lo
        nt = M + 1
        sums, beta, zj, *rest = ctx.saved_tensors
        onepass_saved = None
        if ctx.onepass:
            rest, onepass_saved = rest[:-4], rest[-4:]
        zs, nrms, zbs = rest[:M], rest[M:2 * M], rest[2 * M:2 * M + ctx.n_zb]
        zcs = rest[2 * M + ctx.n_zb:]
        dev = sums.device
        st = _stream()
        dp = 104
        A = s.A
        coef = gout.contiguous().float()
        slots = 1 + L.sga_loss_slots()
        gam_neg = torch.empty((slots, M), device=dev, dtype=torch.float64)
        if onepass_saved is not None:
            dz_aa, gs_aa, gam_aa, hint = onepass_saved
            hh = torch.dot(hint, hint)
            u = torch.dot(coef, hint) / hh
            mismatch = (coef - u * hint).abs().max() > 1e-4 * hh.sqrt()
            u = torch.where(mismatch, torch.full_like(u, float('nan')), u)
            if _o.VALIDATE:
                bad = mismatch.to(torch.int32).reshape(1)
                DEFERRED_CHECKS.submit_fn(bad, lambda v: None if v[0] == 0 else (
                    'sgaligner_amd: the gradient that reached the loss terms is not a multiple of the one OverallLoss announced at forward time '
                    "(backward through something other than loss_dict['loss'] up to a factor); set sgaligner_amd.ops.FUSED_AA_ONEPASS = False"))
            dz_all = dz_aa * u.float()
            dzs = [dz_all[k] for k in range(M)]
            gs = _allreduce_sum(gs_aa * u, ctx.reduce)
            gam_anc = gam_aa * u
            chunks = []
        else:
            dz_all = torch.zeros((M, s.R, dp), device=dev, dtype=torch.float32)
            dzs = [dz_all[k] for k in range(M)]
            gam_anc = torch.zeros((M,), device=dev, dtype=torch.float64)
        fused = M <= 4 and _o.FUSED_ANCHOR_BWD
        ntab = M if fused else nt
        if onepass_saved is None:
            chunks = _anchor_chunks(a_lo, a_hi, A, ntab)
            zz = torch.zeros((nt * 8 + M,), device=dev, dtype=torch.float64)
            gs = zz[:nt * 8].view(nt, 8)
        if onepass_saved is not None:
            pass
        elif fused:
            gsc = torch.empty((slots + 1, nt, 8), device=dev, dtype=torch.float64)
            gam2 = torch.empty((slots, M), device=dev, dtype=torch.float64)
            gam_acc = zz[nt * 8:]
        else:
            gsc = torch.empty((slots, nt, 8), device=dev, dtype=torch.float64)
            dps = [dp] * M + [M * dp]
            dzj = torch.zeros((2 * A, M * dp), device=dev, dtype=torch.float32) if chunks else None
        if chunks:
            cmax = max(hi - lo for lo, hi in chunks)
            m1 = [torch.empty((A * cmax,), device=dev, dtype=torch.float32) for _ in range(ntab)]
        for lo, hi in chunks:
            if fused:
                _lib.check(L.sga_loss_anchor_multi_bwd(_ptr_array(zs), M, _p(beta), A, _p(sums), ctx.alpha, TAU_ICL, TAU_IAL, _p(coef),
                                                       _ptr_array(m1), _p(gsc), _p(gam2), lo, hi, None, st), 'sga_loss_anchor_multi_bwd')
                gam_acc += gam2[0]
            else:
                _lib.check(L.sga_loss_anchor_bwd(_ptr_array(list(zs) + [zj]), (_ct.c_int * nt)(*dps), nt, A, _p(sums), ctx.alpha,
                                                 TAU_ICL, TAU_IAL, _p(coef), _ptr_array(m1), _p(gsc), lo, hi, st), 'sga_loss_anchor_bwd')
                _lib.check(L.sga_loss_stash_grad(_p(m1[M]), _p(zj), A, M * dp, _p(dzj), lo, hi, st), 'sga_loss_stash_grad')
            gs += gsc[0]
            for k in range(M):
                if ctx.split3 and _o.BF16X6_STASH:
                    _lib.check(L.sga_loss_stash_grad_symx_bf16x6(_p(m1[k]), None, _p(zbs[k]), A, s.J1, s.J2, _p(dzs[k]), lo, hi, 0, A, A, st),
                               'sga_loss_stash_grad_symx_bf16x6')
                else:
                    _lib.check(L.sga_loss_stash_grad(_p(m1[k]), _p(zcs[k] if (ctx.split3 or ctx.centred32) else zs[k]), A, dp, _p(dzs[k]), lo, hi, st), 'sga_loss_stash_grad')
        if chunks:
            del m1
            if fused:
                gam_anc = gam_acc
            else:
                gam_sq = torch.zeros((M,), device=dev, dtype=torch.float64)
                _lib.check(L.sga_loss_fold_joint(_ptr_array(zs), M, _p(beta), _p(dzj), 2 * A, _ptr_array(dzs), _p(gam_sq), st),
                           'sga_loss_fold_joint')
                gam_anc = gam_sq / (2.0 * torch.sqrt(beta.double()))
                del dzj
        if onepass_saved is None:
            gs = _allreduce_sum(gs, ctx.reduce)
        ev = None
        if _o.KERNEL_EVENTS is not None:
            ev = (torch.cuda.Event(enable_timing=True), torch.cuda.Event(enable_timing=True))
            ev[0].record()
        if ctx.n_zb and ctx.split3:
            _lib.check(L.sga_loss_multi_grad_bf16x6(_ptr_array(zbs), M, _p(beta), A, s.J1, s.J2, TAU_ICL, TAU_IAL, _p(gs), _ptr_array(dzs),
                                                    _p(gam_neg), a_lo, a_hi, st), 'sga_loss_multi_grad_bf16x6')
        elif ctx.centred32:
            _lib.check(L.sga_loss_multi_grad_centred(_ptr_array(zcs), M, _p(beta), A, s.J1, s.J2, TAU_ICL, TAU_IAL, _p(gs), _ptr_array(dzs),
                                                     _p(gam_neg), a_lo, a_hi, st), 'sga_loss_multi_grad_centred')
        else:
            _lib.check(L.sga_loss_multi_grad(_ptr_array(zs), M, max(d for _, d in ctx.shapes), _p(beta), A, s.J1, s.J2, TAU_ICL, TAU_IAL, _p(gs), _ptr_array(dzs),
                                             _p(gam_neg), a_lo, a_hi, st), 'sga_loss_multi_grad')
        if ev is not None:
            ev[1].record()
            _o.KERNEL_EVENTS.setdefault('loss_multi_grad_bf16x6' if ctx.split3 else 'loss_multi_grad', []).append(ev + ((ns, A, s.J1, s.J2, M),))
        grads = []
        same = all(sh == ctx.shapes[0] for sh in ctx.shapes)
        de_all = torch.zeros((M,) + tuple(ctx.shapes[0]), device=dev, dtype=torch.float32) if same else None
        for k in range(M):
            t, d = ctx.shapes[k]
            de = de_all[k] if same else torch.zeros((t, d), device=dev, dtype=torch.float32)
            if ctx.n_zb and ctx.split3:
                _lib.check(L.sga_loss_scatter_tangent(_p(dzs[k]), _p(zs[k]), _p(nrms[k]), _p(s.idx), A, s.J1, s.J2, d, _p(zbs[k]), _p(de), st),
                           'sga_loss_scatter_tangent')
            elif ctx.centred32:
                _lib.check(L.sga_loss_scatter_tangent_stat(_p(dzs[k]), _p(zs[k]), _p(nrms[k]), _p(s.idx), s.R, d, _p(zbs[k]), _p(de), st),
                           'sga_loss_scatter_tangent_stat')
            else:
                _lib.check(L.sga_loss_scatter(_p(dzs[k]), _p(zs[k]), _p(nrms[k]), _p(s.idx), s.R, d, dp, _p(de), st), 'sga_loss_scatter')
            grads.append(de)
        gbeta = (gam_neg[0] + gam_anc).float()
        return (None, None, None, None, None, gbeta, *grads)


def fused_contrastive_terms(tables, fusion_weight, data_dict, alpha=ALPHA, shard=None, reduce=None, coef_hint=None):
    s = IndexSets.of(data_dict, tables[0].device, int(tables[0].shape[0]))
    w = torch.softmax(fusion_weight.reshape(-1), dim=0)
    beta = (w * w) / (w * w).sum()
    if coef_hint is not None and not (torch.is_grad_enabled() and (beta.requires_grad or any(t.requires_grad for t in tables))):
        coef_hint = None
    return FusedContrastiveFn.apply(s, alpha, shard, reduce, coef_hint, beta, *tables), s
```

Measured before the change: 968.2.

## Run anchor-anchor backward on precomputed bf16x6 split planes with bf16 MFMAs

Adds a planes variant of the anchor-multi backward kernel that reads the pre-split three-plane bf16 tables (the same swizzled layout used by the negative sweeps). It multiplies them with six bf16 16x16x32 MFMAs per product instead of the fp32 path, and uses 32-column tiles with a larger workgroup. The Python loss op switches both the forward-time symmetric build and the backward fused path to it when split3 with bf16x6 mode is enabled. The aim is to speed up the anchor×anchor similarity GEMMs using higher-throughput bf16 matrix cores while keeping near-fp32 accuracy. The trade-offs are more MFMAs per product, a workgroup limited to one block per CU, and the layout constants moving into a shared header.

Result: no change. 977.2, median of 6 (+0.9%).

```diff
diff --git a/include/sgaligner_hip.h b/include/sgaligner_hip.h
--- a/include/sgaligner_hip.h
+++ b/include/sgaligner_hip.h
@@ -100,6 +100,13 @@
                                    double* gs, double* gamma, int a_lo, int a_hi, int j_lo, int j_hi, int mir, double* out_terms, void* stream);
 int sga_loss_stash_grad_symx(const float* M1, const float* M2, const float* Z, int A, int Dp, float* dZ, int a_lo, int a_hi,
                              int j_lo, int j_hi, int mir, void* stream);
+int sga_loss_anchor_multi_bwd_bf16x6(const void* const* Zb, int M, const float* beta, int A, const double* sums, float alpha,
+                                     float tau_icl, float tau_ial, const float* coef, float* const* M1, double* gs, double* gamma,
+                                     int a_lo, int a_hi, double* out_terms, void* stream);
+int sga_loss_anchor_multi_bwd_symx_bf16x6(const void* const* Zb, int M, const float* beta, int A, const double* sums, float alpha,
+                                          float tau_icl, float tau_ial, const float* coef, float* const* M1, float* const* M2,
+                                          double* gs, double* gamma, int a_lo, int a_hi, int j_lo, int j_hi, int mir, double* out_terms,
+                                          void* stream);
 
 int sga_loss_build_joint(const float* const* Z, int M, const float* beta, int rows, float* ZJ, void* stream);
 int sga_loss_fold_joint(const float* const* Z, int M, const float* beta, const float* dZJ, int rows, float* const* dZ,
diff --git a/sgaligner_amd/_lib.py b/sgaligner_amd/_lib.py
--- a/sgaligner_amd/_lib.py
+++ b/sgaligner_amd/_lib.py
@@ -94,6 +94,8 @@
     'sga_loss_anchor_multi_bwd_sym': (I, [P, I, P, I, P, F, F, F, P, P, P, P, P, I, I, P, P]),
     'sga_loss_stash_grad_sym': (I, [P, P, P, I, I, P, I, I, P]),
     'sga_loss_anchor_multi_bwd_symx': (I, [P, I, P, I, P, F, F, F, P, P, P, P, P, I, I, I, I, I, P, P]),
+    'sga_loss_anchor_multi_bwd_bf16x6': (I, [P, I, P, I, P, F, F, F, P, P, P, P, I, I, P, P]),
+    'sga_loss_anchor_multi_bwd_symx_bf16x6': (I, [P, I, P, I, P, F, F, F, P, P, P, P, P, I, I, I, I, I, P, P]),
     'sga_loss_stash_grad_symx': (I, [P, P, P, I, I, P, I, I, I, I, I, P]),
     'sga_loss_split3_bytes': (c_size_t, [I, I, I]),
     'sga_loss_split3_tables': (I, [P, I, I, I, P, P, P]),
diff --git a/sgaligner_amd/csrc/contrastive.hip b/sgaligner_amd/csrc/contrastive.hip
--- a/sgaligner_amd/csrc/contrastive.hip
+++ b/sgaligner_amd/csrc/contrastive.hip
@@ -2,6 +2,7 @@
 #include <type_traits>
 
 #include "loss_math.h"
+#include "split3_layout.h"
 #include "wide16_api.h"
 
 extern "C" int sga_gemm(int transA, int transB, int M, int N, int K, const void* A, long lda, int a_is_f64, const float* B,
@@ -1253,6 +1254,8 @@
     int j_lo;
     float* M2[4];
     int j_hi, mir;
+    const unsigned char* Zb[4];
+    int nbA;
 };
 
 template <int M, bool BWD>
@@ -1369,10 +1372,18 @@
     if (i < n) inv[i] = (float)(1.0 / (sums[i] + 1e-9));
 }
 
-template <int M, bool TERMS = false, int RB = (M <= 3 ? 32 : 16), bool SYM = false>
-__global__ __launch_bounds__(CT_THREADS, 2) void anchor_multi_bwd16_kernel(AnchorMultiArgs a) {
+typedef unsigned int aa_u32x4 __attribute__((ext_vector_type(4)));
+typedef __bf16 aa_bf16x8 __attribute__((ext_vector_type(8)));
+__device__ __forceinline__ f32x4 aa_mfma3(aa_u32x4 a, aa_u32x4 b, f32x4 c) {
+    return __builtin_amdgcn_mfma_f32_16x16x32_bf16(__builtin_bit_cast(aa_bf16x8, a), __builtin_bit_cast(aa_bf16x8, b), c, 0, 0, 0);
+}
+template <int M> constexpr int aa_planes_threads() { return M <= 3 ? 2 * CT_THREADS : CT_THREADS; }
+template <int M, bool TERMS = false, int RB = (M <= 3 ? 32 : 16), bool SYM = false, bool PL = false>
+__global__ __launch_bounds__(PL ? aa_planes_threads<M>() : CT_THREADS, PL ? 1 : 2) void anchor_multi_bwd16_kernel(AnchorMultiArgs a) {
     static_assert(!SYM || TERMS, "symmetric mode: one-pass build");
-    constexpr int DP = 104, NT = M + 1, NSUB = RB / 16, TW = 4 / NSUB;
+    static_assert(!PL || RB == 32, "three planes: whole 32-row blocks");
+    constexpr int THREADS = PL ? aa_planes_threads<M>() : CT_THREADS;
+    constexpr int DP = 104, NT = M + 1, NSUB = RB / 16, TW = THREADS / 64 / NSUB;
     extern __shared__ __attribute__((aligned(16))) float lds[];
     const float* __restrict__ inv_s = a.inv;
     auto CF = [&](int e) { return a.coef[e]; };
@@ -1382,13 +1393,36 @@
     const int ib = blockIdx.x / a.nsplit, split = blockIdx.x % a.nsplit;
     const int i0 = a.i_lo + ib * RB;
     const int ih = wave % NSUB, tw = wave / NSUB;
-    const int my_i = i0 + ih * 16 + l15;
+    const int my_i = i0 + (PL ? 8 * (l15 >> 2) + 4 * ih + (l15 & 3) : ih * 16 + l15);
     const bool iv = my_i < a.i_hi;
 
-    for (int e = tid; e < M * 2 * RB * (DP / 4); e += CT_THREADS) {
-        const int c = (e % (DP / 4)) * 4, r = (e / (DP / 4)) % RB, side = (e / (DP / 4) / RB) % 2, m = e / (DP / 4) / (2 * RB);
-        const int row = min(i0 + r, a.i_hi - 1) + side * A;
-        *reinterpret_cast<f32x4*>(lds + ((m * 2 + side) * RB + r) * DP + c) = *reinterpret_cast<const f32x4*>(a.Z[m] + (size_t)row * DP + c);
+    if constexpr (PL) {
+        unsigned char* lb = reinterpret_cast<unsigned char*>(lds);
+        for (int e = tid; e < M * 2 * 32 * S3_ROWSLOTS; e += THREADS) {
+            const int k = e % S3_ROWSLOTS, r = (e / S3_ROWSLOTS) % 32, side = (e / S3_ROWSLOTS / 32) % 2, m = e / (S3_ROWSLOTS * 64);
+            const int row = min(i0 + r, a.i_hi - 1), o = row & 31;
+            const int si = 4 * (o >> 3) + (o & 3), sh = (o >> 2) & 1, di = 4 * (r >> 3) + (r & 3), dh = (r >> 2) & 1;
+            const unsigned char* src = a.Zb[m] + (size_t)(side * a.nbA + (row >> 5)) * S3_BLOCK;
+            aa_u32x4 v;
+            int doff;
+            if (k < 36) {
+                const int p = k / 12, q = (k >> 2) % 3, gg = k & 3;
+                v = *reinterpret_cast<const aa_u32x4*>(src + p * S3_PLANE + ((q * 2 + sh) * 64 + s3_slot(gg, si)) * 16);
+                doff = p * S3_PLANE + ((q * 2 + dh) * 64 + s3_slot(gg, di)) * 16;
+            } else {
+                const int gg = k - 36;
+                v = gg == 3 ? aa_u32x4{0, 0, 0, 0} : *reinterpret_cast<const aa_u32x4*>(src + S3_TAIL + (sh * 64 + s3_slot(gg ? gg + 1 : 0, si)) * 16);
+                v[2] = (v[2] >> 16) | (v[2] << 16);
+                doff = S3_TAIL + (dh * 64 + s3_slot(gg, di)) * 16;
+            }
+            *reinterpret_cast<aa_u32x4*>(lb + (m * 2 + side) * S3_BLOCK + doff) = v;
+        }
+    } else {
+        for (int e = tid; e < M * 2 * RB * (DP / 4); e += THREADS) {
+            const int c = (e % (DP / 4)) * 4, r = (e / (DP / 4)) % RB, side = (e / (DP / 4) / RB) % 2, m = e / (DP / 4) / (2 * RB);
+            const int row = min(i0 + r, a.i_hi - 1) + side * A;
+            *reinterpret_cast<f32x4*>(lds + ((m * 2 + side) * RB + r) * DP + c) = *reinterpret_cast<const f32x4*>(a.Z[m] + (size_t)row * DP + c);
+        }
     }
     __syncthreads();
     float beta[M];
@@ -1434,14 +1468,53 @@
     };
     const float* js = inv_s + M * 8;
 
-    const int ntile = (JH + 15) / 16;
+    const int ntile = PL ? 2 * ((JH + 31) / 32) : (JH + 15) / 16;
 #pragma unroll 1
     for (int jt = (a.j_lo >> 4) + split * TW + tw; jt < ntile; jt += a.nsplit * TW) {
-        const int j0 = jt * 16;
+        const int j0 = PL ? 32 * (jt >> 1) : jt * 16, jspan = PL ? 32 : 16;
+        const int jc0 = PL ? j0 + 4 * (jt & 1) + 8 * g : j0 + 4 * g;
         const int jrow = min(j0 + l15, A - 1);
         int lofs = 0;
         asm volatile("" : "+v"(lofs));
         f32x4 P[M], Q[M];
+        if constexpr (PL) {
+            const unsigned char* lb = reinterpret_cast<const unsigned char*>(lds) + lofs;
+            const int jb = jt >> 1, jh = jt & 1, ls = 16 * s3_slot(g, l15);
+            const int lt0 = S3_TAIL + ih * 1024 + 16 * s3_slot(g == 1 ? 1 : 0, l15);
+            const int lt1 = S3_TAIL + ih * 1024 + 16 * s3_slot(g == 0 ? 2 : (g == 2 ? 1 : 3), l15);
+            struct JPl { aa_u32x4 pl[3][3], t; };
+            auto jload = [&](int hs, JPl& o) {
+                const unsigned char* src = a.Zb[hs >> 1] + (size_t)(((hs & 1) ? 0 : a.nbA) + jb) * S3_BLOCK + ls;
+#pragma unroll
+                for (int p = 0; p < 3; ++p)
+#pragma unroll
+                    for (int q = 0; q < 3; ++q) o.pl[p][q] = *reinterpret_cast<const aa_u32x4*>(src + p * S3_PLANE + (q * 2 + jh) * 1024);
+                o.t = *reinterpret_cast<const aa_u32x4*>(src + S3_TAIL + jh * 1024);
+            };
+            JPl jr[2];
+            jload(0, jr[0]);
+#pragma unroll
+            for (int hs = 0; hs < 2 * M; ++hs) {
+                if (hs + 1 < 2 * M) jload(hs + 1, jr[(hs + 1) & 1]);
+                __builtin_amdgcn_sched_barrier(0);
+                const JPl& o = jr[hs & 1];
+                const unsigned char* ob = lb + ((hs >> 1) * 2 + (hs & 1)) * S3_BLOCK;
+                aa_u32x4 w[3][3];
+#pragma unroll
+                for (int p = 0; p < 3; ++p)
+#pragma unroll
+                    for (int q = 0; q < 3; ++q) w[p][q] = *reinterpret_cast<const aa_u32x4*>(ob + p * S3_PLANE + (q * 2 + ih) * 1024 + ls);
+                f32x4 acc = aa_mfma3(o.t, *reinterpret_cast<const aa_u32x4*>(ob + lt0), f32x4{0.f, 0.f, 0.f, 0.f});
+                acc = aa_mfma3(o.t, *reinterpret_cast<const aa_u32x4*>(ob + lt1), acc);
+                constexpr int JP[6] = {2, 1, 1, 0, 0, 0}, WP[6] = {0, 1, 0, 2, 1, 0};
+#pragma unroll
+                for (int x = 0; x < 6; ++x)
+#pragma unroll
+                    for (int q = 0; q < 3; ++q) acc = aa_mfma3(o.pl[JP[x]][q], w[WP[x]][q], acc);
+                if (hs & 1) Q[hs >> 1] = acc; else P[hs >> 1] = acc;
+                __builtin_amdgcn_sched_barrier(0);
+            }
+        } else {
         struct JOps { f32x4 p[6], q[6]; float pt[2], qt[2]; };
         auto jload = [&](int m, JOps& o) {
             const float* gp = a.Z[m] + (size_t)(A + jrow) * DP;
@@ -1485,12 +1558,13 @@
             }
             __builtin_amdgcn_sched_barrier(0);
         }
+        }
         const float cJ = CF(M);
         auto epilogue = [&](auto masked_c) {
         constexpr bool MASKED = decltype(masked_c)::value;
 #pragma unroll
         for (int r = 0; r < 4; ++r) {
-            const int j = j0 + 4 * g + r;
+            const int j = jc0 + r;
             const bool ok = !MASKED || (iv && (j < JH));
             const float okf = (!MASKED || ok) ? 1.f : 0.f;
             float xj = 0.f, yj = 0.f;
@@ -1574,7 +1648,7 @@
         auto epilogue_sym = [&](auto) {
 #pragma unroll
         for (int r = 0; r < 4; ++r) {
-            const int j = j0 + 4 * g + r;
+            const int j = jc0 + r;
             const bool ok = iv && (j < JH);
             const float okf = ok ? 1.f : 0.f;
             float xj = 0.f, yj = 0.f;
@@ -1660,7 +1734,7 @@
         if constexpr (SYM) {
             if (j0 >= a.mir) epilogue_sym(0); else epilogue(std::true_type{});
         } else {
-            if (j0 + 16 <= A && i0 + RB <= a.i_hi) epilogue(std::false_type{}); else epilogue(std::true_type{});
+            if (j0 + jspan <= A && i0 + RB <= a.i_hi) epilogue(std::false_type{}); else epilogue(std::true_type{});
         }
 #endif
         if ((++tiles_done & (SYM ? 15 : 31)) == 0) flush();
@@ -2104,12 +2178,16 @@
 }
 
 static int fill_anchor_multi(AnchorMultiArgs& a, const float* const* Z, int M, const float* beta, int A, const double* sums,
-                             float alpha, float tau_icl, float tau_ial, int a_lo, int a_hi) {
+                             float alpha, float tau_icl, float tau_ial, int a_lo, int a_hi, const void* const* Zb = nullptr) {
     if (M < 2 || M > 4) { sga_set_error("sga_loss_anchor_multi: M=%d not in {2,3,4} (use the per-table kernels)", M); return SGA_ERR_ARG; }
     if (a_lo < 0 || a_hi > A || a_lo > a_hi) { sga_set_error("sga_loss_anchor_multi: anchor shard [%d,%d) outside [0,%d]", a_lo, a_hi, A); return SGA_ERR_ARG; }
     a.M = M; a.A = A; a.i_lo = a_lo; a.i_hi = a_hi; a.beta = beta; a.sums = sums; a.alpha = alpha;
     a.kc = LOG2E / tau_icl; a.ki = LOG2E / tau_ial; a.itc = 1.f / tau_icl; a.iti = 1.f / tau_ial;
-    for (int m = 0; m < M; ++m) { if (!Z[m]) { sga_set_error("sga_loss_anchor_multi: null table"); return SGA_ERR_ARG; } a.Z[m] = Z[m]; }
+    for (int m = 0; m < M; ++m) {
+        if (Zb ? !Zb[m] : !Z[m]) { sga_set_error("sga_loss_anchor_multi: null table"); return SGA_ERR_ARG; }
+        if (Zb) a.Zb[m] = static_cast<const unsigned char*>(Zb[m]); else a.Z[m] = Z[m];
+    }
+    a.nbA = (A + 31) / 32;
     const int nib = (a_hi - a_lo + 31) / 32, ntile = (A + 31) / 32;
     int ns = (4 * sga_num_cus() + nib - 1) / (nib > 0 ? nib : 1);
     if (ns > (ntile + 3) / 4) ns = (ntile + 3) / 4;
@@ -2145,24 +2223,44 @@
     return SGA_OK;
 }
 
-extern "C" int sga_loss_anchor_multi_bwd(const float* const* Z, int M, const float* beta, int A, const double* sums,
-                                         float alpha, float tau_icl, float tau_ial, const float* coef, float* const* M1,
-                                         double* gs, double* gamma, int a_lo, int a_hi, double* out_terms, void* stream) {
-    SGA_CHECK_ARG(Z && beta && sums && coef && M1 && gs && gamma && A >= 0, "sga_loss_anchor_multi_bwd: bad argument");
+static void launch_aa_planes(AnchorMultiArgs& a, int M, bool sym, bool terms, int ncols, hipStream_t s) {
+    const size_t lds = (size_t)M * 2 * S3_BLOCK;
+    const int threads = M <= 3 ? aa_planes_threads<3>() : aa_planes_threads<4>();
+    const int nib = (a.i_hi - a.i_lo + 31) / 32, ntile16 = 2 * ((ncols + 31) / 32), TW = threads / 128;
+    int nsp = (3 * sga_num_cus() + nib - 1) / (nib > 0 ? nib : 1);
+    if (nsp > (ntile16 + TW - 1) / TW) nsp = (ntile16 + TW - 1) / TW;
+    if (nsp < 1) nsp = 1;
+    a.nsplit = nsp;
+    auto go = [&](auto k) {
+        hipFuncSetAttribute(reinterpret_cast<const void*>(k), hipFuncAttributeMaxDynamicSharedMemorySize, (int)lds);
+        hipLaunchKernelGGL(k, dim3(nib * nsp), dim3(threads), lds, s, a);
+    };
+    if (sym) { if (M == 2) go(anchor_multi_bwd16_kernel<2, true, 32, true, true>); else if (M == 3) go(anchor_multi_bwd16_kernel<3, true, 32, true, true>); else go(anchor_multi_bwd16_kernel<4, true, 32, true, true>); }
+    else if (terms) { if (M == 2) go(anchor_multi_bwd16_kernel<2, true, 32, false, true>); else if (M == 3) go(anchor_multi_bwd16_kernel<3, true, 32, false, true>); else go(anchor_multi_bwd16_kernel<4, true, 32, false, true>); }
+    else { if (M == 2) go(anchor_multi_bwd16_kernel<2, false, 32, false, true>); else if (M == 3) go(anchor_multi_bwd16_kernel<3, false, 32, false, true>); else go(anchor_multi_bwd16_kernel<4, false, 32, false, true>); }
+}
+
+static int anchor_multi_bwd_impl(const float* const* Z, const void* const* Zb, int M, const float* beta, int A, const double* sums,
+                                 float alpha, float tau_icl, float tau_ial, const float* coef, float* const* M1,
+                                 double* gs, double* gamma, int a_lo, int a_hi, double* out_terms, void* stream) {
+    SGA_CHECK_ARG((Z || Zb) && beta && sums && coef && M1 && gs && gamma && A >= 0, "sga_loss_anchor_multi_bwd: bad argument");
     hipStream_t s = static_cast<hipStream_t>(stream);
     if (int rc0 = zero_slots(gs, (M + 1) * 8, s, "sga_loss_anchor_multi_bwd")) return rc0;
     if (int rc1 = zero_slots(gamma, M, s, "sga_loss_anchor_multi_bwd")) return rc1;
     if (out_terms) { if (int rc2 = zero_slots(out_terms, (M + 1) + 2 * M, s, "sga_loss_anchor_multi_bwd")) return rc2; }
     if (A == 0 || a_hi <= a_lo) return SGA_OK;
     AnchorMultiArgs a{};
-    int rc = fill_anchor_multi(a, Z, M, beta, A, sums, alpha, tau_icl, tau_ial, a_lo, a_hi);
+    int rc = fill_anchor_multi(a, Z, M, beta, A, sums, alpha, tau_icl, tau_ial, a_lo, a_hi, Zb);
     if (rc) return rc;
     a.coef = coef; a.gs = gs; a.gamma = gamma;
     float* inv = reinterpret_cast<float*>(gs + (size_t)(1 + SGA_SLOTS) * (M + 1) * 8);
     hipLaunchKernelGGL(inv_sums_kernel, dim3(1), dim3(64), 0, s, sums, inv, (M + 1) * 8);
     a.inv = inv;
     for (int m = 0; m < M; ++m) { SGA_CHECK_ARG(M1[m], "sga_loss_anchor_multi_bwd: null stash"); a.M1[m] = M1[m]; }
-    {
+    if (Zb) {
+        a.out = out_terms;
+        launch_aa_planes(a, M, false, out_terms != nullptr, A, s);
+    } else {
         const int RB = M <= 3 ? 32 : 16, TW = M <= 3 ? 2 : 4;
         const size_t lds = (size_t)(M * 2 * RB * 104 + (M + 1) * 8) * sizeof(float);
         const int nib = (a.i_hi - a.i_lo + RB - 1) / RB, ntile16 = (A + 15) / 16;
@@ -2185,7 +2283,21 @@
     return SGA_OK;
 }
 
-static int symx_impl(const float* const* Z, int M, const float* beta, int A, const double* sums, float alpha,
+extern "C" int sga_loss_anchor_multi_bwd(const float* const* Z, int M, const float* beta, int A, const double* sums,
+                                         float alpha, float tau_icl, float tau_ial, const float* coef, float* const* M1,
+                                         double* gs, double* gamma, int a_lo, int a_hi, double* out_terms, void* stream) {
+    SGA_CHECK_ARG(Z, "sga_loss_anchor_multi_bwd: bad argument");
+    return anchor_multi_bwd_impl(Z, nullptr, M, beta, A, sums, alpha, tau_icl, tau_ial, coef, M1, gs, gamma, a_lo, a_hi, out_terms, stream);
+}
+
+extern "C" int sga_loss_anchor_multi_bwd_bf16x6(const void* const* Zb, int M, const float* beta, int A, const double* sums,
+                                                float alpha, float tau_icl, float tau_ial, const float* coef, float* const* M1,
+                                                double* gs, double* gamma, int a_lo, int a_hi, double* out_terms, void* stream) {
+    SGA_CHECK_ARG(Zb, "sga_loss_anchor_multi_bwd_bf16x6: bad argument");
+    return anchor_multi_bwd_impl(nullptr, Zb, M, beta, A, sums, alpha, tau_icl, tau_ial, coef, M1, gs, gamma, a_lo, a_hi, out_terms, stream);
+}
+
+static int symx_impl(const float* const* Z, const void* const* Zb, int M, const float* beta, int A, const double* sums, float alpha,
                      float tau_icl, float tau_ial, const float* coef, float* const* M1, float* const* M2,
                      double* gs, double* gamma, int a_lo, int a_hi, int j_lo, int j_hi, int mir, double* out_terms,
                      void* stream);
@@ -2194,14 +2306,25 @@
                                               float tau_icl, float tau_ial, const float* coef, float* const* M1, float* const* M2,
                                               double* gs, double* gamma, int a_lo, int a_hi, int j_lo, int j_hi, int mir, double* out_terms,
                                               void* stream) {
-    return symx_impl(Z, M, beta, A, sums, alpha, tau_icl, tau_ial, coef, M1, M2, gs, gamma, a_lo, a_hi, j_lo, j_hi, mir, out_terms, stream);
-}
-
-static int symx_impl(const float* const* Z, int M, const float* beta, int A, const double* sums, float alpha,
+    SGA_CHECK_ARG(Z, "sga_loss_anchor_multi_bwd_symx: bad argument");
+    return symx_impl(Z, nullptr, M, beta, A, sums, alpha, tau_icl, tau_ial, coef, M1, M2, gs, gamma, a_lo, a_hi, j_lo, j_hi, mir, out_terms, stream);
+}
+
+extern "C" int sga_loss_anchor_multi_bwd_symx_bf16x6(const void* const* Zb, int M, const float* beta, int A, const double* sums, float alpha,
+                                                     float tau_icl, float tau_ial, const float* coef, float* const* M1, float* const* M2,
+                                                     double* gs, double* gamma, int a_lo, int a_hi, int j_lo, int j_hi, int mir, double* out_terms,
+                                                     void* stream) {
+    SGA_CHECK_ARG(Zb, "sga_loss_anchor_multi_bwd_symx_bf16x6: bad argument");
+    SGA_CHECK_ARG(j_lo % 32 == 0 && (j_hi % 32 == 0 || j_hi == A) && (mir % 32 == 0 || mir >= j_hi),
+                  "sga_loss_anchor_multi_bwd_symx_bf16x6: columns [%d,%d) / mirror start %d not on 32-column boundaries", j_lo, j_hi, mir);
+    return symx_impl(nullptr, Zb, M, beta, A, sums, alpha, tau_icl, tau_ial, coef, M1, M2, gs, gamma, a_lo, a_hi, j_lo, j_hi, mir, out_terms, stream);
+}
+
+static int symx_impl(const float* const* Z, const void* const* Zb, int M, const float* beta, int A, const double* sums, float alpha,
                      float tau_icl, float tau_ial, const float* coef, float* const* M1, float* const* M2,
                      double* gs, double* gamma, int a_lo, int a_hi, int j_lo, int j_hi, int mir, double* out_terms,
                      void* stream) {
-    SGA_CHECK_ARG(Z && beta && sums && coef && M1 && M2 && gs && gamma && out_terms && A >= 0, "sga_loss_anchor_multi_bwd_symx: bad argument");
+    SGA_CHECK_ARG((Z || Zb) && beta && sums && coef && M1 && M2 && gs && gamma && out_terms && A >= 0, "sga_loss_anchor_multi_bwd_symx: bad argument");
     SGA_CHECK_ARG(M >= 2 && M <= 4, "sga_loss_anchor_multi_bwd_symx: M=%d (2, 3 or 4)", M);
     SGA_CHECK_ARG(a_lo % 32 == 0 && (a_hi % 32 == 0 || a_hi == A), "sga_loss_anchor_multi_bwd_symx: block [%d,%d) not on 32-row boundaries", a_lo, a_hi);
     SGA_CHECK_ARG(j_lo >= 0 && j_lo % 16 == 0 && j_hi <= A && j_lo <= j_hi && (j_hi % 16 == 0 || j_hi == A) && mir >= j_lo && (mir % 16 == 0 || mir >= j_hi),
@@ -2214,7 +2337,7 @@
     if (int rc2 = zero_slots(out_terms, (M + 1) + 2 * M, s, "sga_loss_anchor_multi_bwd_symx")) return rc2;
     if (A == 0 || a_hi <= a_lo || j_hi <= j_lo) return SGA_OK;
     AnchorMultiArgs a{};
-    int rc = fill_anchor_multi(a, Z, M, beta, A, sums, alpha, tau_icl, tau_ial, a_lo, a_hi);
+    int rc = fill_anchor_multi(a, Z, M, beta, A, sums, alpha, tau_icl, tau_ial, a_lo, a_hi, Zb);
     if (rc) return rc;
     a.coef = coef; a.gs = gs; a.gamma = gamma; a.out = out_terms; a.j_lo = j_lo; a.j_hi = j_hi; a.mir = mir;
     float* inv = reinterpret_cast<float*>(gs + (size_t)(1 + SGA_SLOTS) * (M + 1) * 8);
@@ -2223,6 +2346,14 @@
     for (int m = 0; m < M; ++m) {
         SGA_CHECK_ARG(M1[m] && (M2[m] || mir >= j_hi), "sga_loss_anchor_multi_bwd_symx: null stash");
         a.M1[m] = M1[m]; a.M2[m] = M2[m];
+    }
+    if (Zb) {
+        launch_aa_planes(a, M, true, true, j_hi - j_lo, s);
+        fold_slots(out_terms, (M + 1) + 2 * M, s);
+        fold_slots(gs, (M + 1) * 8, s);
+        fold_slots(gamma, M, s);
+        SGA_CHECK_LAUNCH("sga_loss_anchor_multi_bwd_symx_bf16x6");
+        return SGA_OK;
     }
     const int RB = M <= 3 ? 32 : 16, TW = M <= 3 ? 2 : 4;
     const size_t lds = (size_t)(M * 2 * RB * 104 + (M + 1) * 8) * sizeof(float);
diff --git a/sgaligner_amd/csrc/split3_layout.h b/sgaligner_amd/csrc/split3_layout.h
--- /dev/null
+++ b/sgaligner_amd/csrc/split3_layout.h
@@ -0,0 +1,10 @@
+#pragma once
+
+constexpr int S3_DP = 104;
+constexpr int S3_PLANE = 3 * 2 * 1024;
+constexpr int S3_TAIL = 3 * S3_PLANE;
+constexpr int S3_BLOCK = S3_TAIL + 2048;
+constexpr int S3_NCH = S3_BLOCK / 1024;
+constexpr int S3_ROWSLOTS = 3 * 12 + 4;
+
+__host__ __device__ constexpr int s3_slot(int g, int i) { return 16 * g + (i ^ (12 * (g & 1))); }
diff --git a/sgaligner_amd/csrc/sweep3.hip b/sgaligner_amd/csrc/sweep3.hip
--- a/sgaligner_amd/csrc/sweep3.hip
+++ b/sgaligner_amd/csrc/sweep3.hip
@@ -2,6 +2,7 @@
 #include <type_traits>
 
 #include "loss_math.h"
+#include "split3_layout.h"
 
 namespace {
 
@@ -11,13 +12,6 @@
 typedef unsigned int u32x4 __attribute__((ext_vector_type(4)));
 typedef unsigned int u32x2 __attribute__((ext_vector_type(2)));
 typedef short s16x4 __attribute__((ext_vector_type(4)));
-
-constexpr int S3_DP = 104;
-constexpr int S3_PLANE = 3 * 2 * 1024;
-constexpr int S3_TAIL = 3 * S3_PLANE;
-constexpr int S3_BLOCK = S3_TAIL + 2048;
-constexpr int S3_NCH = S3_BLOCK / 1024;
-constexpr int S3_ROWSLOTS = 3 * 12 + 4;
 
 __device__ __forceinline__ void split3_pair(float v0, float v1, unsigned& h, unsigned& m, unsigned& l) {
     const bf16x2 H = __builtin_convertvector(f32x2{v0, v1}, bf16x2);
@@ -62,7 +56,6 @@
         sgb_seq<X + 1, END, NR, VALU_ALL>();
     }
 }
-__host__ __device__ constexpr int s3_slot(int g, int i) { return 16 * g + (i ^ (12 * (g & 1))); }
 
 struct TLayout { int nbA, nb1, nb2; };
 __host__ __device__ inline TLayout make_tlayout(int A, int J1, int J2) { return TLayout{(A + 31) / 32, (J1 + 31) / 32, (J2 + 31) / 32}; }
diff --git a/sgaligner_amd/loss_ops.py b/sgaligner_amd/loss_ops.py
--- a/sgaligner_amd/loss_ops.py
+++ b/sgaligner_amd/loss_ops.py
@@ -506,6 +506,8 @@
                 ev[1].record()
                 _o.KERNEL_EVENTS.setdefault('loss_multi_sums', []).append(ev + ((a_hi - a_lo, s.A, s.J1, s.J2, M),))
         sums = _allreduce_sum(sums[0].contiguous(), reduce)
+        aa3 = split3 and get_mfma_mode() == 'bf16x6'
+        zarr3 = _ptr_array(zbs) if aa3 else None
         zj = torch.empty((2 * s.A, M * dp), device=dev, dtype=torch.float32)
         _lib.check(L.sga_loss_build_joint(zarr, M, _p(beta), 2 * s.A, _p(zj), st), 'sga_loss_build_joint')
         out = torch.empty((slots * (nt + 2 * M),), device=dev, dtype=torch.float64)
@@ -536,9 +538,10 @@
                     m1 = [b[:n1] for b in buf]
                     m2 = [b[n1:] for b in buf]
                     has2 = mir < jh
-                    _lib.check(L.sga_loss_anchor_multi_bwd_symx(zarr, M, _p(beta), s.A, _p(sums), float(alpha), TAU_ICL, TAU_IAL, _p(coef),
-                                     _ptr_array(m1), _ptr_array(m2) if has2 else (_ct.c_void_p * M)(), _p(gsc), _p(gam2),
-                                     lo, hi, jl, jh, mir, _p(out), st), 'sga_loss_anchor_multi_bwd_symx')
+                    symx = L.sga_loss_anchor_multi_bwd_symx_bf16x6 if aa3 else L.sga_loss_anchor_multi_bwd_symx
+                    _lib.check(symx(zarr3 if aa3 else zarr, M, _p(beta), s.A, _p(sums), float(alpha), TAU_ICL, TAU_IAL, _p(coef),
+                                    _ptr_array(m1), _ptr_array(m2) if has2 else (_ct.c_void_p * M)(), _p(gsc), _p(gam2),
+                                    lo, hi, jl, jh, mir, _p(out), st), 'sga_loss_anchor_multi_bwd_symx')
                     out_acc += out[:n_terms]
                     gs_aa += gsc[0]
                     gam_aa += gam2[0]
@@ -553,9 +556,10 @@
             elif chunks:
                 cmax = max(hi - lo for lo, hi in chunks)
                 m1 = [torch.empty((s.A * cmax,), device=dev, dtype=torch.float32) for _ in range(M)]
+                bwd = L.sga_loss_anchor_multi_bwd_bf16x6 if aa3 else L.sga_loss_anchor_multi_bwd
                 for lo, hi in chunks:
-                    _lib.check(L.sga_loss_anchor_multi_bwd(zarr, M, _p(beta), s.A, _p(sums), float(alpha), TAU_ICL, TAU_IAL, _p(coef),
-                                                           _ptr_array(m1), _p(gsc), _p(gam2), lo, hi, _p(out), st), 'sga_loss_anchor_multi_bwd')
+                    _lib.check(bwd(zarr3 if aa3 else zarr, M, _p(beta), s.A, _p(sums), float(alpha), TAU_ICL, TAU_IAL, _p(coef),
+                                   _ptr_array(m1), _p(gsc), _p(gam2), lo, hi, _p(out), st), 'sga_loss_anchor_multi_bwd')
                     out_acc += out[:n_terms]
                     gs_aa += gsc[0]
                     gam_aa += gam2[0]
@@ -580,6 +584,7 @@
         ctx.shapes = [tuple(t.shape) for t in tables]
         ctx.n_zb = len(zbs)
         ctx.split3 = split3
+        ctx.aa3 = aa3
         ctx.centred32 = centred32
         ctx.onepass = onepass
         ctx.n_zc = len(zcs)
@@ -647,8 +652,9 @@
             m1 = [torch.empty((A * cmax,), device=dev, dtype=torch.float32) for _ in range(ntab)]
         for lo, hi in chunks:
             if fused:
-                _lib.check(L.sga_loss_anchor_multi_bwd(_ptr_array(zs), M, _p(beta), A, _p(sums), ctx.alpha, TAU_ICL, TAU_IAL, _p(coef),
-                                                       _ptr_array(m1), _p(gsc), _p(gam2), lo, hi, None, st), 'sga_loss_anchor_multi_bwd')
+                bwd = L.sga_loss_anchor_multi_bwd_bf16x6 if ctx.aa3 else L.sga_loss_anchor_multi_bwd
+                _lib.check(bwd(_ptr_array(zbs) if ctx.aa3 else _ptr_array(zs), M, _p(beta), A, _p(sums), ctx.alpha, TAU_ICL, TAU_IAL, _p(coef),
+                               _ptr_array(m1), _p(gsc), _p(gam2), lo, hi, None, st), 'sga_loss_anchor_multi_bwd')
                 gam_acc += gam2[0]
             else:
                 _lib.check(L.sga_loss_anchor_bwd(_ptr_array(list(zs) + [zj]), (_ct.c_int * nt)(*dps), nt, A, _p(sums), ctx.alpha,
```
